# ScottHCL/recommend

Hardware: AMD Instinct MI355X
Metric: ranked samples/sec (fwd+bwd) at B=4096 seq=128; AUC parity vs ref (higher is better)
Workload: dtype f32-emulated (fp16-pair / split-bf16); 1 GPU; C2: OneTrans 4L d128 H4 f512 L_NS12 L_S128 (seq 3x42), Criteo-shape 13 dense + 26 ids, replicated tables, fwd+bwd+optimizer; global_batch=4096, per_gpu_batch=4096, seq_len=128, parallelism=dp1

## Files before the change

### include/onetrans_hip.h

```cpp
#ifndef ONETRANS_HIP_H
#define ONETRANS_HIP_H

#include <stddef.h>
#include <stdint.h>

#ifdef __cplusplus
extern "C" {
#endif

#define OT_OK 0
#define OT_ERR_INVALID_ARG 1
#define OT_ERR_UNSUPPORTED 2
#define OT_ERR_HIP 3

#define OT_GEMM_NN 0
#define OT_GEMM_NT 1

#define OT_AX_NONE 0
#define OT_AX_RMSNORM 1
#define OT_AX_GELU 2
#define OT_AX_BF16 4
#define OT_AX_BF16_RMSNORM 5

#define OT_EPI_BIAS 1
#define OT_EPI_GELU_BWD 2
#define OT_EPI_GELU 4
#define OT_EPI_DROPOUT 8
#define OT_EPI_RESIDUAL 16
#define OT_EPI_ACCUMULATE 32
#define OT_EPI_ROW_RSTD 64
#define OT_EPI_ROWDOT 256
#define OT_EPI_RMSNORM_BWD 128
#define OT_EPI_C_BF16 512
#define OT_EPI_AUX_BF16 1024
#define OT_WG_D_BF16 8

int ot_version(void);
const char* ot_get_last_error_string(void);

int ot_gemm_tile_rows(void);
#define OT_MATMUL_F32 0
#define OT_MATMUL_SPLIT_BF16 1
#define OT_MATMUL_BF16 2
int ot_mixed_gemm(int mode, const float* A, int64_t lda, int K, const int32_t* in_rows,
                  int a_xform, const float* a_rstd, const float* a_gamma,
                  const float* W, int64_t w_gstride, int64_t ldw, int N,
                  const int32_t* tile_group, int ntiles,
                  const float* bias, int64_t bias_gstride,
                  float* C, int64_t ldc, const int32_t* out_rows, int epi,
                  const float* res, int64_t ldres, int res_tok,
                  const float* aux, int64_t ldaux,
                  uint32_t seed, uint32_t site, float drop_rate, int tail_K, int tail_I,
                  const int32_t* tail_pos, int precision, void* stream);
typedef struct ot_rms_epilogue {
  size_t struct_size;
  float* rstd_out; float eps;
  const float* x; int64_t ldx;
  const float* gamma; const float* rstd;
  const float* dres; int64_t lddres;
  int dres_tail_K, dres_tail_I;
  const int32_t* dres_tail_inv;
  float* dx_masked; int64_t lddxm;
  float* dgamma; int accumulate_dgamma;
  void* workspace; size_t ws_bytes;
  float* rowdot; int rowdot_n;
  uint16_t* gelu_out; int64_t ldgelu;
  uint16_t* xn_out; int64_t ldxn;
  uint16_t* c16_out; int64_t ldc16;
  float* rowmax_out; int rowmax_n;
  const float* a_rowmax; int a_rowmax_n;
  float* amax_out;
  float* rowabs_out; int rowabs_n;
} ot_rms_epilogue;
size_t ot_mixed_gemm_rms_workspace_size(int ntiles, int N);
int ot_mixed_gemm_rms(int mode, const float* A, int64_t lda, int K, const int32_t* in_rows,
                      int a_xform, const float* a_rstd, const float* a_gamma,
                      const float* W, int64_t w_gstride, int64_t ldw, int N,
                      const int32_t* tile_group, int ntiles,
                      const float* bias, int64_t bias_gstride,
                      float* C, int64_t ldc, const int32_t* out_rows, int epi,
                      const float* res, int64_t ldres, int res_tok,
                      const float* aux, int64_t ldaux,
                      uint32_t seed, uint32_t site, float drop_rate, int tail_K, int tail_I,
                      const int32_t* tail_pos, const ot_rms_epilogue* rms, int precision, void* stream);

size_t ot_wgrad_workspace_size(int nchunks, int K, int N);
int ot_mixed_gemm_wgrad(const float* A, int64_t lda, const int32_t* a_rows, int a_xform,
                        const float* a_rstd, const float* a_gamma,
                        const float* D, int64_t ldd, const int32_t* d_rows, int K, int N,
                        const int32_t* chunks, int nchunks, const int32_t* gchunk, int ngroups,
                        float* dW, int64_t dw_gstride, float* db, int64_t db_gstride,
                        int accumulate, void* workspace, size_t ws_bytes, int precision, void* stream);

int ot_mixed_gemm_wgrad_ex(const float* A, int64_t lda, const int32_t* a_rows, int a_xform,
                           const float* a_rstd, const float* a_gamma,
                           const float* D, int64_t ldd, const int32_t* d_rows, int K, int N,
                           const int32_t* chunks, int nchunks, const int32_t* gchunk, int ngroups,
                           float* dW, int64_t dw_gstride, float* db, int64_t db_gstride,
                           int accumulate, void* workspace, size_t ws_bytes, const float* a_bound,
                           const float* d_bound, int precision, void* stream);

int ot_transpose_banks(const float* src, float* dst, const int64_t* banks_dev, int nbanks, int64_t total_tiles,
                       void* stream);

size_t ot_split_image_elems(int G, int N, int K);
int ot_split_images(const float* base, const int64_t* desc_dev, int ndesc, int64_t total_units, uint16_t* img,
                    int precision, void* stream);
int ot_mixed_gemm_img(int mode, const float* A, int64_t lda, int K, const int32_t* in_rows,
                      int a_xform, const float* a_rstd, const float* a_gamma,
                      const float* W, int64_t w_gstride, int64_t ldw, int N,
                      const int32_t* tile_group, int ntiles,
                      const float* bias, int64_t bias_gstride,
                      float* C, int64_t ldc, const int32_t* out_rows, int epi,
                      const float* res, int64_t ldres, int res_tok,
                      const float* aux, int64_t ldaux,
                      uint32_t seed, uint32_t site, float drop_rate, int tail_K, int tail_I,
                      const int32_t* tail_pos, const uint16_t* b_image, int image_ntn, int image_tn0,
                      int precision, void* stream);
int ot_plane_wide(int on);
int ot_wgrad_wide(int on);
int ot_plane_rowmeta(int on);
int ot_plane_panel(int on);
int ot_plane_panel_launches(void);
int ot_mixed_gemm_rms_img(int mode, const float* A, int64_t lda, int K, const int32_t* in_rows,
                          int a_xform, const float* a_rstd, const float* a_gamma,
                          const float* W, int64_t w_gstride, int64_t ldw, int N,
                          const int32_t* tile_group, int ntiles,
                          const float* bias, int64_t bias_gstride,
                          float* C, int64_t ldc, const int32_t* out_rows, int epi,
                          const float* res, int64_t ldres, int res_tok,
                          const float* aux, int64_t ldaux,
                          uint32_t seed, uint32_t site, float drop_rate, int tail_K, int tail_I,
                          const int32_t* tail_pos, const ot_rms_epilogue* rms, const uint16_t* b_image,
                          int image_ntn, int image_tn0, int precision, void* stream);

typedef struct ot_ffn_fused_args {
  size_t struct_size;
  const float* x1; int64_t ldx1;
  const int32_t* rows;
  const int32_t* tile_group; int ntiles;
  const float* rstd;
  const uint16_t* w1_image; int w1_groups;
  const uint16_t* w2_image; int w2_groups;
  const float* b1; int64_t b1_gstride;
  const float* b2; int64_t b2_gstride;
  int f;
  float* u_out; int64_t ldu;
  float* u_amax;
  float* x2; int64_t ldx2;
  float* rstd_out; float eps;
  uint32_t seed, site; float drop_rate;
  int tail_K, tail_I; const int32_t* tail_pos;
} ot_ffn_fused_args;
int ot_ffn_fused_fwd(const ot_ffn_fused_args* args, void* stream);
int ot_ffn_fused(int on);

typedef struct ot_ffn_fused_bwd_args {
  size_t struct_size;
  const float* dy2; int64_t lddy2;
  const float* dy2_rowmax; int dy2_rowmax_n;
  const int32_t* rows;
  const int32_t* tile_group; int ntiles;
  const uint16_t* w2_image; int w2_groups;
  const uint16_t* w1_image; int w1_groups;
  int f;
  const float* u; int64_t ldu;
  float* du; int64_t lddu;
  float* du_amax;
  const float* x1; int64_t ldx1;
  const float* gamma; const float* rstd;
  const float* dres; int64_t lddres;
  float* dx1; int64_t lddx1;
  float* dx_masked; int64_t lddxm;
  float* dgamma; int accumulate_dgamma;
  void* workspace; size_t ws_bytes;
  float* amax_out; float* rowabs_out; int rowabs_n;
  uint32_t seed, site; float drop_rate;
  int tail_K, tail_I; const int32_t* tail_pos;
} ot_ffn_fused_bwd_args;
int ot_ffn_fused_bwd(const ot_ffn_fused_bwd_args* args, void* stream);
int ot_ffn_fused_bwd_on(int on);

int ot_attn_fwd(const float* qkv, int64_t ld, int B, int H, int I, int K, const int32_t* qpos,
                int head_dim, float* out, float* lse, int precision, void* stream);
size_t ot_attn_fwd_fp8_workspace_size(int B, int H, int I, int head_dim);
int ot_attn_fwd_fp8(const float* qkv, int64_t ld, int B, int H, int I, int K, const int32_t* qpos,
                    int head_dim, float* out, float* lse, void* workspace, size_t ws_bytes, void* stream);
#define OT_FP8_DEQUANT 1
#define OT_FP8_TWO_TERM 2
int ot_attn_fwd_fp8_ex(float* qkv, int64_t ld, int B, int H, int I, int K, const int32_t* qpos, int head_dim,
                       float* out, float* lse, void* workspace, size_t ws_bytes, int flags, void* stream);
int ot_attn_fwd_fp8_deq16(const float* qkv, int64_t ld, int B, int H, int I, int K, const int32_t* qpos,
                          int head_dim, float* out, float* lse, void* workspace, size_t ws_bytes, int flags,
                          uint16_t* deq16, void* stream);
size_t ot_attn_bwd_workspace_size(int B, int H, int K);
int ot_attn_bwd(const float* qkv, int64_t ld, const float* out, const float* dout, const float* lse,
                int B, int H, int I, int K, const int32_t* qpos, int head_dim, float* dqkv, float* delta_ws,
                int precision, void* stream);
size_t ot_attn_bwd_ex_workspace_size(int B, int H, int I, int K, int head_dim, int selected, int precision);
int ot_attn_bwd_ex(const float* qkv, int64_t ld, const float* out, const float* dout, const float* lse,
                   int B, int H, int I, int K, const int32_t* qpos, int head_dim, float* dqkv, void* workspace,
                   size_t ws_bytes, int precision, void* stream);
#define OT_ATTN_DQKV_BF16 1
#define OT_ATTN_QKV_BF16 2
#define OT_ATTN_DQ_PART_BF16 4
int ot_attn_bwd_dqkv_bf16_supported(int I, int K, int head_dim, int selected, int precision);
int ot_attn_bwd_bf16_forms(int I, int K, int head_dim, int selected, int precision);
size_t ot_attn_bwd_flags_workspace_size(int B, int H, int I, int K, int head_dim, int selected, int flags, int precision);
int ot_attn_slice_supported(int I, int K, int head_dim, int selected);
int ot_attn_bwd_flags(const float* qkv, int64_t ld, const float* out, const float* dout, const float* lse,
                      int B, int H, int I, int K, const int32_t* qpos, int head_dim, void* dqkv, int flags,
                      void* workspace, size_t ws_bytes, int precision, void* stream);
int ot_attn_amax_supported(int I, int K, int head_dim, int selected, int precision);
int ot_attn_fwd_amax(const float* qkv, int64_t ld, int B, int H, int I, int K, const int32_t* qpos,
                     int head_dim, float* out, float* lse, float* amax, float* rowmax, int precision, void* stream);
int ot_attn_bwd_amax(const float* qkv, int64_t ld, const float* out, const float* dout, const float* lse,
                     int B, int H, int I, int K, const int32_t* qpos, int head_dim, float* dqkv,
                     void* workspace, size_t ws_bytes, float* amax, float* rowmax, int precision, void* stream);

int ot_attn_fwd_cached(const float* qkv, int64_t ld, const float* kv_cache, int64_t ldc, const int32_t* req,
                       int C, int H, int Ic, int n, int Kq, int head_dim, float* out, void* stream);

int ot_attn_fwd_cached_lse(const float* qkv, int64_t ld, const float* kv_cache, int64_t ldc, const int32_t* req,
                           int C, int H, int Ic, int n, int Kq, int head_dim, float* out, float* lse, void* stream);
size_t ot_attn_bwd_cached_workspace_size(int R, int C, int H, int Ic, int n, int Kq, int head_dim);
int ot_attn_bwd_cached(const float* qkv, int64_t ld, const float* kv_cache, int64_t ldc, const int32_t* req_start,
                       int R, int C, int H, int Ic, int n, int Kq, int head_dim, const float* out, const float* dout,
                       const float* lse, float* dqkv, float* dkv_cache, int accumulate, void* workspace,
                       size_t ws_bytes, void* stream);

int ot_attn_fold_supported(int d, int H);
int ot_attn_fold_rows(int I, int ded0, int ded1);
int ot_attn_fold_fwd(const float* x, int64_t ldx, const float* rstd, const float* gamma, const float* w, int64_t ldw,
                     const float* wT, int64_t ldwT, const float* qkv, int64_t ldqkv, int B, int H, int I,
                     int head_dim, int ded0, int ded1, float* o, float* lse, float* y, void* stream);
int ot_attn_fold_bwd(const float* x, int64_t ldx, const float* rstd, const float* gamma, const float* w, int64_t ldw,
                     const float* wT, int64_t ldwT, const float* qkv, int64_t ldqkv, int B, int H, int I,
                     int head_dim, int ded0, int ded1, const float* o, const float* dout, const float* lse,
                     const float* y, const float* dx1, float* dx, int64_t lddx, float* dqkv, int64_t lddqkv, float* z,
                     float* dgpart, void* stream);
size_t ot_attn_fold_workspace_size(int B, int d);
int ot_attn_fold_dw(const float* z, const float* y, const float* qkv, int64_t ldqkv, const float* dout,
                    const float* gamma, int B, int H, int I, int head_dim, float* dW, int64_t lddw, int accumulate,
                    void* workspace, size_t ws_bytes, void* stream);
int ot_attn_fold_dgamma(const float* dgpart, int B, int d, float* dgamma, int accumulate, void* workspace,
                        size_t ws_bytes, void* stream);
int ot_last_fold(int on);

int ot_attn_fwd_masked(const float* qkv, int64_t ld, int B, int H, int I, int K, const int32_t* qpos, int head_dim,
                       const uint8_t* key_valid, int64_t ldv, float* out, float* lse, int precision, void* stream);
int ot_attn_bwd_masked(const float* qkv, int64_t ld, const float* out, const float* dout, const float* lse, int B,
                       int H, int I, int K, const int32_t* qpos, int head_dim, const uint8_t* key_valid, int64_t ldv,
                       float* dqkv, float* delta_ws, int precision, void* stream);
int ot_attn_fwd_cached_masked(const float* qkv, int64_t ld, const float* kv_cache, int64_t ldc, const int32_t* req,
                              int C, int H, int Ic, int n, int Kq, int head_dim, const uint8_t* cache_valid,
                              int64_t ldcv, float* out, float* lse_or_null, void* stream);
int ot_seq_key_valid(const int32_t* lens, const int32_t* seq_len, const int32_t* seq_off, int nseq, int B, int L0,
                     const int32_t* rank, int64_t ldr, uint8_t* valid0, void* stream);

int ot_kv_pack_bf16(const float* qkv, int64_t ld, int R, int64_t rows_per_req, int d, uint16_t* kv16, int64_t ldc16,
                    int64_t req_stride, int64_t row0, void* stream);
int ot_attn_fwd_cached_kv16(const float* qkv, int64_t ld, const uint16_t* kv16, int64_t ldc16, int64_t req_stride,
                            const int32_t* req, int C, int H, int Ic, int n, int Kq, int head_dim,
                            const uint8_t* cache_valid, int64_t ldcv, float* out, float* lse_or_null, void* stream);
// ... 171 lines not shown
```

### recommend_amd/_lib.py

```python

from __future__ import annotations

import ctypes
import os
from ctypes import c_float, c_int, c_int64, c_size_t, c_uint32, c_void_p, c_char_p

_HERE = os.path.dirname(os.path.abspath(__file__))
LIB_PATH = os.environ.get('ONETRANS_HIP_LIB') or os.path.join(_HERE, 'libonetrans_hip.so')
HEADER = os.path.join(os.path.dirname(_HERE), 'include', 'onetrans_hip.h')

OT_GEMM_NN, OT_GEMM_NT = 0, 1
OT_AX_NONE, OT_AX_RMSNORM, OT_AX_GELU, OT_AX_BF16, OT_AX_BF16_RMSNORM = 0, 1, 2, 4, 5
OT_EPI_BIAS, OT_EPI_GELU_BWD, OT_EPI_GELU = 1, 2, 4
OT_EPI_DROPOUT, OT_EPI_RESIDUAL, OT_EPI_ACCUMULATE = 8, 16, 32
OT_EPI_ROW_RSTD, OT_EPI_RMSNORM_BWD, OT_EPI_ROWDOT = 64, 128, 256
OT_EPI_C_BF16 = 512
OT_EPI_AUX_BF16 = 1024
OT_ATTN_DQKV_BF16 = 1
OT_ATTN_QKV_BF16 = 2
OT_ATTN_DQ_PART_BF16 = 4
OT_WG_D_BF16 = 8
OT_MATMUL_F32, OT_MATMUL_SPLIT_BF16, OT_MATMUL_BF16 = 0, 1, 2
OT_FP8_DEQUANT, OT_FP8_TWO_TERM = 1, 2
OT_RANK_SUM, OT_RANK_PRODUCT = 0, 1
RANK_MODES = {'sum': OT_RANK_SUM, 'product': OT_RANK_PRODUCT}
RANK_MAX_K = 1024
MATMUL_MODES = {'f32': OT_MATMUL_F32, 'split': OT_MATMUL_SPLIT_BF16, 'bf16': OT_MATMUL_BF16}


class RmsEpilogue(ctypes.Structure):
    _fields_ = [('struct_size', c_size_t), ('rstd_out', c_void_p), ('eps', c_float),
                ('x', c_void_p), ('ldx', c_int64), ('gamma', c_void_p), ('rstd', c_void_p),
                ('dres', c_void_p), ('lddres', c_int64), ('dres_tail_K', c_int), ('dres_tail_I', c_int),
                ('dres_tail_inv', c_void_p),
                ('dx_masked', c_void_p), ('lddxm', c_int64),
                ('dgamma', c_void_p), ('accumulate_dgamma', c_int),
                ('workspace', c_void_p), ('ws_bytes', c_size_t),
                ('rowdot', c_void_p), ('rowdot_n', c_int),
                ('gelu_out', c_void_p), ('ldgelu', c_int64),
                ('xn_out', c_void_p), ('ldxn', c_int64),
                ('c16_out', c_void_p), ('ldc16', c_int64),
                ('rowmax_out', c_void_p), ('rowmax_n', c_int),
                ('a_rowmax', c_void_p), ('a_rowmax_n', c_int),
                ('amax_out', c_void_p), ('rowabs_out', c_void_p), ('rowabs_n', c_int)]

class FfnFusedArgs(ctypes.Structure):
    _fields_ = [('struct_size', c_size_t), ('x1', c_void_p), ('ldx1', c_int64), ('rows', c_void_p),
                ('tile_group', c_void_p), ('ntiles', c_int), ('rstd', c_void_p),
                ('w1_image', c_void_p), ('w1_groups', c_int), ('w2_image', c_void_p), ('w2_groups', c_int),
                ('b1', c_void_p), ('b1_gstride', c_int64), ('b2', c_void_p), ('b2_gstride', c_int64),
                ('f', c_int), ('u_out', c_void_p), ('ldu', c_int64), ('u_amax', c_void_p),
                ('x2', c_void_p), ('ldx2', c_int64), ('rstd_out', c_void_p), ('eps', c_float),
                ('seed', c_uint32), ('site', c_uint32), ('drop_rate', c_float),
                ('tail_K', c_int), ('tail_I', c_int), ('tail_pos', c_void_p)]


class FfnFusedBwdArgs(ctypes.Structure):
    _fields_ = [('struct_size', c_size_t), ('dy2', c_void_p), ('lddy2', c_int64),
                ('dy2_rowmax', c_void_p), ('dy2_rowmax_n', c_int), ('rows', c_void_p),
                ('tile_group', c_void_p), ('ntiles', c_int),
                ('w2_image', c_void_p), ('w2_groups', c_int), ('w1_image', c_void_p), ('w1_groups', c_int),
                ('f', c_int), ('u', c_void_p), ('ldu', c_int64), ('du', c_void_p), ('lddu', c_int64),
                ('du_amax', c_void_p), ('x1', c_void_p), ('ldx1', c_int64), ('gamma', c_void_p), ('rstd', c_void_p),
                ('dres', c_void_p), ('lddres', c_int64), ('dx1', c_void_p), ('lddx1', c_int64),
                ('dx_masked', c_void_p), ('lddxm', c_int64), ('dgamma', c_void_p), ('accumulate_dgamma', c_int),
                ('workspace', c_void_p), ('ws_bytes', c_size_t),
                ('amax_out', c_void_p), ('rowabs_out', c_void_p), ('rowabs_n', c_int),
                ('seed', c_uint32), ('site', c_uint32), ('drop_rate', c_float),
                ('tail_K', c_int), ('tail_I', c_int), ('tail_pos', c_void_p)]


class SeqTime(ctypes.Structure):
    _fields_ = [('times', c_void_p), ('stride_b', c_int64), ('L', ctypes.c_int32), ('map_off', ctypes.c_int32)]


class NsBag(ctypes.Structure):
    _fields_ = [('table', c_void_p), ('ids', c_void_p), ('weights', c_void_p), ('row_offset', c_int64),
                ('num_rows', c_int64), ('ids_stride', c_int64), ('weights_stride', c_int64),
                ('width', ctypes.c_int32), ('cap', ctypes.c_int32), ('col', ctypes.c_int32),
                ('pooling', ctypes.c_int32)]


OT_BAG_SUM, OT_BAG_MEAN = 0, 1
BAG_POOLINGS = {'sum': OT_BAG_SUM, 'mean': OT_BAG_MEAN}
NS_BAG_MAX = 32
NS_BAG_MAX_WIDTH = 256
SEQ_TIME_MAX_L = 4096
SEQ_TIME_MAX_SEQ = 32

P = c_void_p
I64 = c_int64

SIGNATURES = {
    'ot_version': (c_int, []),
    'ot_get_last_error_string': (c_char_p, []),
    'ot_gemm_tile_rows': (c_int, []),
    'ot_mixed_gemm': (c_int, [c_int, P, I64, c_int, P, c_int, P, P, P, I64, I64, c_int, P, c_int, P, I64,
                              P, I64, P, c_int, P, I64, c_int, P, I64, c_uint32, c_uint32, c_float, c_int,
                              c_int, P, c_int, P]),
    'ot_mixed_gemm_rms_workspace_size': (c_size_t, [c_int, c_int]),
    'ot_mixed_gemm_rms': (c_int, [c_int, P, I64, c_int, P, c_int, P, P, P, I64, I64, c_int, P, c_int, P, I64,
                                  P, I64, P, c_int, P, I64, c_int, P, I64, c_uint32, c_uint32, c_float, c_int,
                                  c_int, P, P, c_int, P]),
    'ot_wgrad_workspace_size': (c_size_t, [c_int, c_int, c_int]),
    'ot_mixed_gemm_wgrad': (c_int, [P, I64, P, c_int, P, P, P, I64, P, c_int, c_int, P, c_int, P, c_int, P,
                                    I64, P, I64, c_int, P, c_size_t, c_int, P]),
    'ot_mixed_gemm_wgrad_ex': (c_int, [P, I64, P, c_int, P, P, P, I64, P, c_int, c_int, P, c_int, P, c_int, P,
                                       I64, P, I64, c_int, P, c_size_t, P, P, c_int, P]),
    'ot_transpose_banks': (c_int, [P, P, P, c_int, I64, P]),
    'ot_mixed_gemm_img': (c_int, [c_int, P, I64, c_int, P, c_int, P, P, P, I64, I64, c_int, P, c_int, P, I64,
                                  P, I64, P, c_int, P, I64, c_int, P, I64, c_uint32, c_uint32, c_float, c_int,
                                  c_int, P, P, c_int, c_int, c_int, P]),
    'ot_mixed_gemm_rms_img': (c_int, [c_int, P, I64, c_int, P, c_int, P, P, P, I64, I64, c_int, P, c_int, P, I64,
                                      P, I64, P, c_int, P, I64, c_int, P, I64, c_uint32, c_uint32, c_float, c_int,
                                      c_int, P, P, P, c_int, c_int, c_int, P]),
    'ot_split_image_elems': (c_size_t, [c_int, c_int, c_int]),
    'ot_plane_wide': (c_int, [c_int]),
    'ot_wgrad_wide': (c_int, [c_int]),
    'ot_plane_rowmeta': (c_int, [c_int]),
    'ot_plane_panel': (c_int, [c_int]),
    'ot_plane_panel_launches': (c_int, []),
    'ot_ffn_fused_fwd': (c_int, [P, P]),
    'ot_ffn_fused': (c_int, [c_int]),
    'ot_ffn_fused_bwd': (c_int, [P, P]),
    'ot_ffn_fused_bwd_on': (c_int, [c_int]),
    'ot_split_images': (c_int, [P, P, c_int, I64, P, c_int, P]),
    'ot_attn_fwd': (c_int, [P, I64, c_int, c_int, c_int, c_int, P, c_int, P, P, c_int, P]),
    'ot_attn_fwd_fp8_workspace_size': (c_size_t, [c_int, c_int, c_int, c_int]),
    'ot_attn_fwd_fp8': (c_int, [P, I64, c_int, c_int, c_int, c_int, P, c_int, P, P, P, c_size_t, P]),
    'ot_attn_fwd_fp8_ex': (c_int, [P, I64, c_int, c_int, c_int, c_int, P, c_int, P, P, P, c_size_t, c_int, P]),
    'ot_attn_fwd_fp8_deq16': (c_int, [P, I64, c_int, c_int, c_int, c_int, P, c_int, P, P, P, c_size_t, c_int, P, P]),
    'ot_attn_bwd_workspace_size': (c_size_t, [c_int, c_int, c_int]),
    'ot_attn_bwd': (c_int, [P, I64, P, P, P, c_int, c_int, c_int, c_int, P, c_int, P, P, c_int, P]),
    'ot_attn_bwd_ex_workspace_size': (c_size_t, [c_int, c_int, c_int, c_int, c_int, c_int, c_int]),
    'ot_attn_bwd_ex': (c_int, [P, I64, P, P, P, c_int, c_int, c_int, c_int, P, c_int, P, P, c_size_t, c_int, P]),
    'ot_attn_bwd_dqkv_bf16_supported': (c_int, [c_int, c_int, c_int, c_int, c_int]),
    'ot_attn_bwd_bf16_forms': (c_int, [c_int, c_int, c_int, c_int, c_int]),
    'ot_attn_slice_supported': (c_int, [c_int, c_int, c_int, c_int]),
    'ot_attn_bwd_flags_workspace_size': (c_size_t, [c_int, c_int, c_int, c_int, c_int, c_int, c_int, c_int]),
    'ot_attn_bwd_flags': (c_int, [P, I64, P, P, P, c_int, c_int, c_int, c_int, P, c_int, P, c_int, P, c_size_t, c_int, P]),
    'ot_attn_fwd_cached': (c_int, [P, I64, P, I64, P, c_int, c_int, c_int, c_int, c_int, c_int, P, P]),
    'ot_attn_fwd_cached_lse': (c_int, [P, I64, P, I64, P, c_int, c_int, c_int, c_int, c_int, c_int, P, P, P]),
    'ot_attn_bwd_cached_workspace_size': (c_size_t, [c_int, c_int, c_int, c_int, c_int, c_int, c_int]),
    'ot_attn_bwd_cached': (c_int, [P, I64, P, I64, P, c_int, c_int, c_int, c_int, c_int, c_int, c_int, P, P, P, P, P,
                                   c_int, P, c_size_t, P]),
    'ot_attn_amax_supported': (c_int, [c_int, c_int, c_int, c_int, c_int]),
    'ot_attn_fwd_amax': (c_int, [P, I64, c_int, c_int, c_int, c_int, P, c_int, P, P, P, P, c_int, P]),
    'ot_attn_bwd_amax': (c_int, [P, I64, P, P, P, c_int, c_int, c_int, c_int, P, c_int, P, P, c_size_t, P, P, c_int,
                                 P]),
    'ot_pyramid_select': (c_int, [P, c_float, c_int, c_int, c_int, c_int, P, P, P, c_int, P]),
    'ot_rmsnorm_fwd': (c_int, [P, I64, P, P, I64, P, I64, c_int, c_float, P]),
    'ot_rmsnorm_bwd_workspace_size': (c_size_t, [I64, c_int]),
    'ot_rmsnorm_bwd': (c_int, [P, I64, P, I64, P, P, P, I64, c_int, c_int, P, P, I64, P, I64, c_uint32,
                               c_uint32, c_float, c_int, c_int, P, P, c_int, I64, c_int, P, c_size_t, P]),
    'ot_dropout_apply': (c_int, [P, I64, P, I64, I64, c_int, c_uint32, c_uint32, c_float, c_int, c_int, P, P]),
    'ot_dropout_apply_bf16': (c_int, [P, I64, P, I64, I64, c_int, c_uint32, c_uint32, c_float, c_int, c_int, P, P]),
    'ot_rows_absmax': (c_int, [P, I64, I64, c_int, P, c_int, P]),
    'ot_dropout_rowmax_supported': (c_int, [c_int]),
    'ot_dropout_apply_ex': (c_int, [P, I64, P, I64, I64, c_int, c_uint32, c_uint32, c_float, c_int, c_int, P, P, P,
                                    c_int, P]),
    'ot_rows_colsum_workspace_size': (c_size_t, [I64, c_int]),
    'ot_rows_colsum': (c_int, [P, I64, P, I64, c_int, P, c_int, P, c_size_t, P]),
    'ot_ns_assemble': (c_int, [P, c_int, P, c_int, P, I64, P]),
    'ot_ns_grad_pack': (c_int, [P, c_int, c_int, P, I64, c_int, P, P, P]),
    'ot_fill_rows': (c_int, [P, I64, P, I64, P, c_int, P]),
    'ot_seq_rows': (c_int, [P, I64, c_int, c_int, I64, P, P]),
    'ot_head_fwd': (c_int, [P, P, P, c_int, c_int, c_int, P, P, P]),
    'ot_head_bwd_workspace_size': (c_size_t, [c_int, c_int, c_int]),
    'ot_head_bwd': (c_int, [P, P, P, P, c_int, c_int, c_int, P, P, P, I64, I64, c_int, P, c_size_t, P]),
    'ot_bce_workspace_size': (c_size_t, [c_int, c_int]),
    'ot_bce_fwd': (c_int, [P, P, c_int, c_int, P, P, c_size_t, P]),
    'ot_bce_bwd': (c_int, [P, P, P, c_int, c_int, P, P]),
    'ot_task_loss_fwd': (c_int, [P, P, c_int, c_int, c_uint32, P, P, c_size_t, P]),
    'ot_task_loss_bwd': (c_int, [P, P, P, c_int, c_int, c_uint32, P, P]),
    'ot_task_loss_logits_fwd': (c_int, [P, P, P, c_int, c_int, c_uint32, P, P, c_size_t, P]),
    'ot_task_loss_logits_bwd': (c_int, [P, P, P, c_int, c_int, c_uint32, P, P]),
    'ot_head_bwd_ex': (c_int, [P, P, P, P, P, c_int, c_int, c_int, P, P, P, I64, I64, c_int, P, c_size_t, P]),
    'ot_sparse_adagrad_workspace_size': (c_size_t, [I64, c_int]),
    'ot_sparse_adagrad': (c_int, [P, P, c_int, I64, P, P, I64, c_float, c_float, c_float, P, c_size_t, P]),
    'ot_sparse_grad_dense': (c_int, [c_int, I64, P, P, I64, P, P, c_size_t, P]),
    'ot_dense_adagrad_workspace_size': (c_size_t, []),
    'ot_dense_adagrad': (c_int, [P, P, P, I64, c_int, c_float, c_float, c_float, P, c_size_t, P]),
    'ot_sparse_prepare': (c_int, [c_int, I64, P, P, I64, P, P, c_size_t, P]),
    'ot_sparse_finish': (c_int, [P, P, c_int, I64, c_float, c_float, c_float, P, P, c_size_t, P]),
    'ot_shard_route_workspace_size': (c_size_t, [I64]),
    'ot_shard_route': (c_int, [P, I64, I64, c_int, P, P, P, P, c_size_t, P]),
    'ot_shard_route_unique_workspace_size': (c_size_t, [I64]),
    'ot_shard_route_unique': (c_int, [P, I64, I64, c_int, P, P, P, P, P, P, c_size_t, P]),
    'ot_segment_rows_sum': (c_int, [P, P, P, I64, c_int, P, P]),
    'ot_segment_rows_sum_workspace_size': (c_size_t, [I64, I64, c_int]),
    'ot_segment_rows_sum_ex': (c_int, [P, P, P, I64, I64, c_int, P, P, c_size_t, P]),
    'ot_gather_rows': (c_int, [P, c_int, P, I64, P, P]),
    'ot_permute_rows': (c_int, [P, P, I64, c_int, c_int, P, P]),
    'ot_hash_uniform_rows': (c_int, [P, I64, c_int, c_int, c_int, c_uint32, c_float, c_float, P]),
    'ot_clip_rmsprop_workspace_size': (c_size_t, [c_int, I64]),
    'ot_clip_rmsprop': (c_int, [P, P, P, P, P, c_int, I64, c_float, c_float, c_float, c_float, c_float, P,
                                c_size_t, P]),
    'ot_clip_adam_workspace_size': (c_size_t, [c_int, I64]),
    'ot_clip_adam': (c_int, [P, P, P, P, P, c_int, I64, c_float, c_float, c_float, c_float, I64, c_float, P,
                             c_size_t, P]),
    'ot_metrics_workspace_size': (c_size_t, [c_int, c_int]),
    'ot_metrics_update': (c_int, [P, P, c_int, c_int, I64, P, c_int, P, P, P, c_size_t, P]),
    'ot_grouped_auc_workspace_size': (c_size_t, [c_int, I64, c_int]),
    'ot_grouped_auc': (c_int, [P, P, P, c_int, I64, I64, c_int, c_uint32, P, P, P, P, P, c_size_t, P]),
    'ot_rank_topk_workspace_size': (c_size_t, [c_int, I64, c_int]),
    'ot_rank_topk': (c_int, [P, I64, c_int, P, c_int, P, I64, c_int, c_int, P, P, P, P, P, c_size_t, P]),
    'ot_seq_time_rows_workspace_size': (c_size_t, [c_int, c_int, c_int]),
    'ot_seq_time_rows': (c_int, [P, c_int, c_int, c_int, I64, P, P, P, P, c_size_t, P]),
# ... 70 lines not shown
```

### recommend_amd/csrc/gemm_ffn.hip

```cpp
#include <atomic>
#include <cstdlib>
#include <mutex>

#include "gemm.h"

namespace ot {

#ifndef OT_FFN_NSTG
#define OT_FFN_NSTG 3
#endif
constexpr int FF_NST = OT_FFN_NSTG;
static_assert(FF_NST == 2 || FF_NST == 3, "fused FFN stage buffers");
constexpr int PG_A_BYTES = GT * 16 * 4;
constexpr int FF_STG = PG_A_BYTES + 2 * GT * 16 * 2;
constexpr int FF_TR_LD = 36;
constexpr int FF_TR_WAVE = 32 * FF_TR_LD * 4;
constexpr int FF_TR_OFF = FF_NST * FF_STG;
constexpr int FF_META_OFF = FF_TR_OFF + 4 * FF_TR_WAVE;
constexpr int FF_TAB_OFF = FF_META_OFF + GT * 4;
constexpr int FF_MAX_F = 1024;
static_assert(FF_META_OFF >= (64 * (GT + 4) + 8 * GT) * 4, "fused FFN: the epilogue tile overlays the row metadata");
static_assert(FF_TAB_OFF + (2 * FF_MAX_F + GT) * 4 <= 80 * 1024, "fused FFN LDS");
constexpr int ffn_lds(int f) { return FF_TAB_OFF + (2 * f + GT) * 4; }

// ... 161 lines not shown
    if (mrow >= 0) am = fmaxf(am, ua);
    {
      const float s = pow2_scale14(fmaxf(mx, 0.17f));
      if (c > 0) {
        const float ratio = s * hinv;
#pragma unroll
        for (int a = 0; a < 4; ++a)
#pragma unroll
          for (int r = 0; r < 16; ++r) acc2[a][r] *= ratio;
      }
      hsc = s;
      hinv = 1.f / s;
    }
    if (q.u_out) {
#pragma unroll
      for (int nb = 0; nb < 4; ++nb) {
#pragma unroll
        for (int qd = 0; qd < 4; ++qd)
          *reinterpret_cast<f32x4*>(trw + li * FF_TR_LD + 8 * qd + 4 * h) =
              f32x4{acc1[nb][4 * qd], acc1[nb][4 * qd + 1], acc1[nb][4 * qd + 2], acc1[nb][4 * qd + 3]};
        asm volatile("s_waitcnt lgkmcnt(0)" ::: "memory");
#pragma unroll
        for (int ps = 0; ps < 4; ++ps) {
          const f32x4 v = *reinterpret_cast<const f32x4*>(trw + ((lane >> 3) + 8 * ps) * FF_TR_LD + 4 * (lane & 7));
          const int ur = rmeta[32 * wave + (lane >> 3) + 8 * ps];
          if (ur >= 0) store_out4(q.u_out + (int64_t)ur * q.ldu + 128 * c + 32 * nb + 4 * (lane & 7), v);
        }
        asm volatile("s_waitcnt lgkmcnt(0)" ::: "memory");
      }
    }
    auto stage2 = [&](int j, const f32x16& u) {
      top(8 + j);
      const char* sb = lds + ((8 + j) % FF_NST) * FF_STG;
#pragma unroll
      for (int s = 0; s < 2; ++s) {
        const f32x4 g0 = gelu_erf4(f32x4{u[8 * s], u[8 * s + 1], u[8 * s + 2], u[8 * s + 3]});
        const f32x4 g1 = gelu_erf4(f32x4{u[8 * s + 4], u[8 * s + 5], u[8 * s + 6], u[8 * s + 7]});
        const float hv[8] = {g0.x, g0.y, g0.z, g0.w, g1.x, g1.y, g1.z, g1.w};
        u32x4 fh[3];
        pair8(hv, hsc, fh);
        u32x4 fw[4][2];
#pragma unroll
        for (int nb = 0; nb < 4; ++nb)
#pragma unroll
          for (int pl = 0; pl < 2; ++pl) {
            const char* wb = sb + s * 8192 + pl * 4096 + nb * 1024;
            const u32x2 lo = *reinterpret_cast<const u32x2*>(wb + woff0);
            const u32x2 hi = *reinterpret_cast<const u32x2*>(wb + woff1);
            fw[nb][pl] = u32x4{lo.x, lo.y, hi.x, hi.y};
          }
#pragma unroll
        for (int nb = 0; nb < 4; ++nb) acc2[nb] = mfma_pair_t(fw[nb], fh, acc2[nb]);
      }
    };
    stage2(0, acc1[0]);
    stage2(1, acc1[1]);
    stage2(2, acc1[2]);
    stage2(3, acc1[3]);
  }
#pragma unroll
  for (int nb = 0; nb < 4; ++nb)
#pragma unroll
    for (int qd = 0; qd < 4; ++qd) {
      const f32x4 cs = *reinterpret_cast<const f32x4*>(tab + 2 * q.f + 32 * nb + 8 * qd + 4 * h);
#pragma unroll
      for (int i = 0; i < 4; ++i) acc2[nb][4 * qd + i] *= hinv * cs[i];
    }
  asm volatile("s_waitcnt vmcnt(0) lgkmcnt(0)" ::: "memory");
  __syncthreads();
  gemm_vec_epilogue<EPIT, 5, false, 8, false>(p, acc2, smem, tm, 0, g, 0, -1, rmeta);
  if (q.u_amax) amax_flush(q.u_amax, am);
}

#ifndef OT_FFN_FUSED
#define OT_FFN_FUSED 1
#endif
static int ffn_fused_initial() {
  const char* e = getenv("ONETRANS_FFN_FUSED");
  return e && *e ? (atoi(e) != 0) : OT_FFN_FUSED;
}
static std::atomic<int> g_ffn_fused{ffn_fused_initial()};

constexpr int FB_TAB_OFF = FF_TAB_OFF;
static_assert(FB_TAB_OFF + (FF_MAX_F + GT) * 4 <= 80 * 1024, "fused FFN backward LDS");
constexpr int ffn_bwd_lds(int f) { return FB_TAB_OFF + (f + GT) * 4; }

struct FfnBwdArgs {
  GemmArgs e;
  const uint16_t* img2; int g2;
  const uint16_t* img1; int g1;
  const float* u; int64_t ldu;
  float* du; int64_t lddu;
  float* du_amax;
  int f;
};

template <int EPIT>
__global__ __launch_bounds__(256, 2) void ffn_fused_bwd_kernel(FfnBwdArgs q) {
  const GemmArgs& p = q.e;
  extern __shared__ __attribute__((aligned(16))) float smem[];
  char* lds = reinterpret_cast<char*>(smem);
  const int tm = xcd_remap(blockIdx.x, p.ntm);
  const int g = p.tile_group ? p.tile_group[tm] : 0;
  const int t = threadIdx.x, lane = t & 63, wave = t >> 6;
  const int h = lane >> 5, li = lane & 31;
  const int nch = q.f >> 7;

  int arow[2];
#pragma unroll
  for (int i = 0; i < 2; ++i) {
    const int64_t gr = (int64_t)tm * GT + (2 * wave + i) * 16 + (lane >> 2);
    const int ir = p.in_rows ? p.in_rows[gr] : (int)gr;
    arow[i] = ir < 0 ? 0 : ir;
  }
  int urow[4];
#pragma unroll
  for (int i = 0; i < 4; ++i) {
    const int64_t gr = (int64_t)tm * GT + 32 * wave + 8 * i + (lane >> 3);
    const int ur = p.out_rows ? p.out_rows[gr] : (int)gr;
    urow[i] = ur < 0 ? 0 : ur;
  }
  constexpr int64_t T1 = 8 * (int64_t)PG_B_BYTES;
  const char* img2 = reinterpret_cast<const char*>(q.img2) + (int64_t)(q.g2 ? g : 0) * nch * T1;
  const char* img1 = reinterpret_cast<const char*>(q.img1) + (int64_t)(q.g1 ? g : 0) * (q.f >> 4) * PG_B_BYTES;
  const int blane = 2 * wave * 1024 + 16 * lane;
  auto issue = [&](int c, int sidx, int buf) {
    char* sb = lds + buf * FF_STG;
    if (sidx < 8) {
      const char* bs = img2 + c * T1 + (int64_t)sidx * PG_B_BYTES + blane;
#pragma unroll
      for (int i = 0; i < 2; ++i)
        __builtin_amdgcn_global_load_lds(
            (const void*)(p.A + (int64_t)arow[i] * p.lda + 16 * sidx + 4 * ((lane & 3) ^ ((lane >> 4) & 3))),
            (lds_void_t*)(sb + (2 * wave + i) * 1024), 16, 0, 0);
#pragma unroll
      for (int i = 0; i < 2; ++i)
        __builtin_amdgcn_global_load_lds((const void*)(bs + i * 1024),
                                         (lds_void_t*)(sb + PG_A_BYTES + (2 * wave + i) * 1024), 16, 0, 0);
    } else if (sidx < 12) {
#pragma unroll
      for (int i = 0; i < 4; ++i)
        __builtin_amdgcn_global_load_lds(
            (const void*)(q.u + (int64_t)urow[i] * q.ldu + 128 * c + 32 * (sidx - 8) +
                          4 * ((lane & 7) ^ ((4 * i + (lane >> 4)) & 7))),
            (lds_void_t*)(sb + (4 * wave + i) * 1024), 16, 0, 0);
    } else {
      const char* bs = img1 + (int64_t)(8 * c + 2 * (sidx - 12)) * PG_B_BYTES + blane;
#pragma unroll
      for (int u = 0; u < 2; ++u)
#pragma unroll
        for (int i = 0; i < 2; ++i)
          __builtin_amdgcn_global_load_lds((const void*)(bs + u * PG_B_BYTES + i * 1024),
                                           (lds_void_t*)(sb + u * 8192 + (2 * wave + i) * 1024), 16, 0, 0);
    }
  };

  const int ra = 32 * wave + li;
  const int aoff0 = ra * 64 + 16 * ((2 * h) ^ ((li >> 2) & 3));
  const int sw = (li >> 3) & 1;
  const int boff = PG_A_BYTES + li * 32 + 16 * (h ^ sw);
  const int woff0 = li * 32 + 16 * sw + 8 * h;
  const int usw = (li >> 1) & 7;

  float abound = 0.f;
  int mrow;
  {
    const int64_t gr = (int64_t)tm * GT + ra;
    int ir = p.in_rows ? p.in_rows[gr] : (int)gr;
    mrow = p.out_rows ? p.out_rows[gr] : (int)gr;
    ir = ir < 0 ? 0 : ir;
    for (int j = 0; j < p.a_rowmax_n; ++j) abound = fmaxf(abound, p.a_rowmax[(int64_t)ir * p.a_rowmax_n + j]);
  }
  float* tab = reinterpret_cast<float*>(lds + FB_TAB_OFF);
  int tt = t;
  asm volatile("" : "+v"(tt));
  for (int idx = tt; idx < q.f; idx += 256) {
    const float* cs = reinterpret_cast<const float*>(img2 + (idx >> 7) * T1 + 2 * GT * 16 * 2);
    const float bad = reinterpret_cast<const uint32_t*>(cs)[GT] == PAIR_IMAGE_TAG ? 1.f : __builtin_nanf("");
    tab[idx] = bad / cs[idx & 127];
  }
  if (tt < GT) {
    const float* cs = reinterpret_cast<const float*>(img1 + 2 * GT * 16 * 2);
    const float bad = reinterpret_cast<const uint32_t*>(cs)[GT] == PAIR_IMAGE_TAG ? 1.f : __builtin_nanf("");
    tab[q.f + tt] = bad / cs[tt];
  }
  int* rmeta = reinterpret_cast<int*>(lds + FF_META_OFF);
  if (h == 0) rmeta[ra] = mrow;
  const float asc = pow2_scale14(abound);
  const float ainv = 1.f / asc;
  float* trw = reinterpret_cast<float*>(lds + FF_TR_OFF + wave * FF_TR_WAVE);
  asm volatile("" : "+v"(abound), "+v"(mrow), "+v"(arow[0]), "+v"(arow[1]), "+v"(urow[0]), "+v"(urow[1]),
               "+v"(urow[2]), "+v"(urow[3]));

  int rb = 0;
  issue(0, 0, 0);
  if (FF_NST == 3) issue(0, 1, 1);
  f32x16 acc2[4];
#pragma unroll
  for (int a = 0; a < 4; ++a)
#pragma unroll
    for (int r = 0; r < 16; ++r) acc2[a][r] = 0.f;
  float am = 0.f, bound = 0.f, hsc = 1.f, hinv = 1.f;

  for (int c = 0; c < nch; ++c) {
    auto top = [&](int sidx) -> const char* {
      if (FF_NST == 2 || sidx == 12 || (sidx == 15 && c + 1 == nch)) asm volatile("s_waitcnt vmcnt(0)" ::: "memory");
      else asm volatile("s_waitcnt vmcnt(4)" ::: "memory");
      asm volatile("s_waitcnt lgkmcnt(0)" ::: "memory");
      __builtin_amdgcn_s_barrier();
      asm volatile("" ::: "memory");
      constexpr int AH = FF_NST - 1;
      const int nb_ = rb == 0 ? FF_NST - 1 : rb - 1;
      if (sidx + AH < 16) issue(c, sidx + AH, nb_);
      else if (c + 1 < nch) issue(c + 1, sidx + AH - 16, nb_);
      const char* sb = lds + rb * FF_STG;
      rb = rb + 1 == FF_NST ? 0 : rb + 1;
      return sb;
    };
    f32x16 acc1[4];
#pragma unroll
    for (int a = 0; a < 4; ++a)
#pragma unroll
      for (int r = 0; r < 16; ++r) acc1[a][r] = 0.f;
#pragma unroll
    for (int kt = 0; kt < 8; ++kt) {
      const char* sb = top(kt);
      u32x4 fb[4][2];
#pragma unroll
      for (int nb = 0; nb < 4; ++nb)
#pragma unroll
        for (int pl = 0; pl < 2; ++pl) fb[nb][pl] = *reinterpret_cast<const u32x4*>(sb + boff + pl * 4096 + nb * 1024);
      const f32x4 a0 = *reinterpret_cast<const f32x4*>(sb + aoff0);
      const f32x4 a1 = *reinterpret_cast<const f32x4*>(sb + (aoff0 ^ 16));
      const float av[8] = {a0.x, a0.y, a0.z, a0.w, a1.x, a1.y, a1.z, a1.w};
      u32x4 fa[3];
      pair8(av, asc, fa);
#pragma unroll
      for (int nb = 0; nb < 4; ++nb) acc1[nb] = mfma_pair_t(fb[nb], fa, acc1[nb]);
    }
    float ua = 0.f;
    auto finish = [&](int nb, f32x16& a) {
      const char* sb = top(8 + nb);
#pragma unroll
      for (int qd = 0; qd < 4; ++qd) {
        const f32x4 u4 = *reinterpret_cast<const f32x4*>(sb + ra * 128 + 16 * ((2 * qd + h) ^ usw));
        const f32x4 ci = *reinterpret_cast<const f32x4*>(tab + 128 * c + 32 * nb + 8 * qd + 4 * h);
        f32x4 v = {a[4 * qd], a[4 * qd + 1], a[4 * qd + 2], a[4 * qd + 3]};
        v = v * (ainv * ci);
        v *= gelu_erf_grad4(u4);
        ua = amax4(ua, v);
        a[4 * qd] = v.x; a[4 * qd + 1] = v.y; a[4 * qd + 2] = v.z; a[4 * qd + 3] = v.w;
      }
    };
    finish(0, acc1[0]);
    finish(1, acc1[1]);
    finish(2, acc1[2]);
    finish(3, acc1[3]);
    if (mrow >= 0) am = fmaxf(am, ua);
    bound = fmaxf(bound, fmaxf(ua, __shfl_xor(ua, 32, 64)));
    {
      const float s = pow2_scale14(bound);
      if (c > 0) {
        const float ratio = s * hinv;
#pragma unroll
        for (int a = 0; a < 4; ++a)
#pragma unroll
          for (int r = 0; r < 16; ++r) acc2[a][r] *= ratio;
      }
      hsc = s;
      hinv = 1.f / s;
    }
#pragma unroll
    for (int nb = 0; nb < 4; ++nb) {
#pragma unroll
      for (int qd = 0; qd < 4; ++qd)
        *reinterpret_cast<f32x4*>(trw + li * FF_TR_LD + 8 * qd + 4 * h) =
            f32x4{acc1[nb][4 * qd], acc1[nb][4 * qd + 1], acc1[nb][4 * qd + 2], acc1[nb][4 * qd + 3]};
      asm volatile("s_waitcnt lgkmcnt(0)" ::: "memory");
#pragma unroll
      for (int ps = 0; ps < 4; ++ps) {
        const f32x4 v = *reinterpret_cast<const f32x4*>(trw + ((lane >> 3) + 8 * ps) * FF_TR_LD + 4 * (lane & 7));
        const int ur = rmeta[32 * wave + (lane >> 3) + 8 * ps];
        if (ur >= 0) store_out4(q.du + (int64_t)ur * q.lddu + 128 * c + 32 * nb + 4 * (lane & 7), v);
      }
      asm volatile("s_waitcnt lgkmcnt(0)" ::: "memory");
    }
    auto stage2 = [&](int j, const f32x16& u) {
      const char* sb = top(12 + j);
#pragma unroll
      for (int s = 0; s < 2; ++s) {
        const float hv[8] = {u[8 * s], u[8 * s + 1], u[8 * s + 2], u[8 * s + 3],
                             u[8 * s + 4], u[8 * s + 5], u[8 * s + 6], u[8 * s + 7]};
        u32x4 fh[3];
        pair8(hv, hsc, fh);
        u32x4 fw[4][2];
#pragma unroll
        for (int nb = 0; nb < 4; ++nb)
#pragma unroll
          for (int pl = 0; pl < 2; ++pl) {
            const char* wb = sb + s * 8192 + pl * 4096 + nb * 1024;
            const u32x2 lo = *reinterpret_cast<const u32x2*>(wb + woff0);
            const u32x2 hi = *reinterpret_cast<const u32x2*>(wb + (woff0 ^ 16));
            fw[nb][pl] = u32x4{lo.x, lo.y, hi.x, hi.y};
          }
#pragma unroll
        for (int nb = 0; nb < 4; ++nb) acc2[nb] = mfma_pair_t(fw[nb], fh, acc2[nb]);
      }
    };
    stage2(0, acc1[0]);
    stage2(1, acc1[1]);
    stage2(2, acc1[2]);
    stage2(3, acc1[3]);
  }
#pragma unroll
  for (int nb = 0; nb < 4; ++nb)
#pragma unroll
    for (int qd = 0; qd < 4; ++qd) {
      const f32x4 cs = *reinterpret_cast<const f32x4*>(tab + q.f + 32 * nb + 8 * qd + 4 * h);
#pragma unroll
      for (int i = 0; i < 4; ++i) acc2[nb][4 * qd + i] *= hinv * cs[i];
    }
  asm volatile("s_waitcnt vmcnt(0) lgkmcnt(0)" ::: "memory");
  __syncthreads();
  gemm_vec_epilogue<EPIT, 5, false, OT_PLANE_EPI_RBN, false>(p, acc2, smem, tm, 0, g, 0, -1, rmeta);
  if (q.du_amax) amax_flush(q.du_amax, am);
}

#ifndef OT_FFN_FUSED_BWD
#define OT_FFN_FUSED_BWD 1
#endif
static int ffn_fused_bwd_initial() {
  const char* e = getenv("ONETRANS_FFN_FUSED_BWD");
  return e && *e ? (atoi(e) != 0) : OT_FFN_FUSED_BWD;
}
static std::atomic<int> g_ffn_fused_bwd{ffn_fused_bwd_initial()};

}

using namespace ot;

extern "C" int ot_ffn_fused_bwd_on(int on) {
  const int old = g_ffn_fused_bwd.load(std::memory_order_relaxed);
  if (on >= 0) g_ffn_fused_bwd.store(on ? 1 : 0, std::memory_order_relaxed);
  return old;
}

extern "C" int ot_ffn_fused_bwd(const ot_ffn_fused_bwd_args* a, void* stream) {
  OT_REQUIRE(a, "ot_ffn_fused_bwd: null arguments");
  OT_REQUIRE(a->struct_size == sizeof(ot_ffn_fused_bwd_args),
             "ot_ffn_fused_bwd: ot_ffn_fused_bwd_args.struct_size %zu != %zu (header of another ot_version)",
             a->struct_size, sizeof(ot_ffn_fused_bwd_args));
  OT_REQUIRE(a->dy2 && a->dy2_rowmax && a->u && a->du && a->w2_image && a->w1_image && a->x1 && a->gamma && a->rstd &&
                 a->dx1 && a->dgamma && a->workspace,
             "ot_ffn_fused_bwd: null operand");
  OT_REQUIRE(a->ntiles >= 0 && a->f >= GT && a->f % GT == 0 && a->f <= FF_MAX_F,
             "ot_ffn_fused_bwd: bad sizes ntiles=%d f=%d (f a multiple of %d up to %d)", a->ntiles, a->f, GT, FF_MAX_F);
  auto a16 = [](const void* q) { return ((uintptr_t)q & 15) == 0; };
  OT_REQUIRE(a->lddy2 >= GT && a->ldx1 >= GT && a->lddx1 >= GT && a->lddy2 % 4 == 0 && a->ldx1 % 4 == 0 &&
                 a->lddx1 % 4 == 0 && a16(a->dy2) && a16(a->x1) && a16(a->dx1) && a16(a->gamma) && a16(a->w2_image) &&
                 a16(a->w1_image),
             "ot_ffn_fused_bwd: rows of %d floats, leading dimensions multiples of 4, 16-B aligned operands", GT);
  OT_REQUIRE(a->ldu >= a->f && a->lddu >= a->f && a->ldu % 4 == 0 && a->lddu % 4 == 0 && a16(a->u) && a16(a->du),
             "ot_ffn_fused_bwd: u / du need ld >= f, ld %% 4 == 0 and 16-B alignment");
  OT_REQUIRE(a->dy2_rowmax_n >= 1, "ot_ffn_fused_bwd: dy2_rowmax_n must be >= 1");
  OT_REQUIRE(!a->dres || (a->lddres >= GT && a->lddres % 4 == 0 && a16(a->dres)),
             "ot_ffn_fused_bwd: dres needs lddres >= %d, lddres %% 4 == 0 and 16-B alignment", GT);
  OT_REQUIRE(a->w1_groups >= 1 && a->w2_groups >= 1, "ot_ffn_fused_bwd: image group counts must be >= 1");
  OT_REQUIRE(a->w1_groups == 1 && a->w2_groups == 1 ? true : a->tile_group != nullptr,
             "ot_ffn_fused_bwd: grouped weight images need tile_group");
  OT_REQUIRE(a->drop_rate >= 0.f && a->drop_rate < 1.f, "ot_ffn_fused_bwd: drop_rate out of range");
  OT_REQUIRE(a->drop_rate == 0.f || (a->tail_K > 0 && a->tail_I >= a->tail_K), "ot_ffn_fused_bwd: bad tail map");
  OT_REQUIRE(a->drop_rate == 0.f || (a->dx_masked && a->lddxm >= GT && a->lddxm % 4 == 0 && a16(a->dx_masked)),
             "ot_ffn_fused_bwd: dropout needs dx_masked (lddxm >= %d, lddxm %% 4 == 0, 16-B aligned)", GT);
  OT_REQUIRE(a->ws_bytes >= ot_mixed_gemm_rms_workspace_size(a->ntiles, GT), "ot_ffn_fused_bwd: workspace too small");
  OT_REQUIRE(!a->rowabs_out || a->rowabs_n == 1, "ot_ffn_fused_bwd: rowabs_out needs rowabs_n == 1");
  if (a->ntiles == 0) return OT_OK;
  FfnBwdArgs q{};
  GemmArgs& p = q.e;
  p.A = a->dy2; p.lda = a->lddy2; p.K = a->f; p.in_rows = a->rows;
  p.a_rowmax = a->dy2_rowmax; p.a_rowmax_n = a->dy2_rowmax_n;
  p.N = GT; p.tile_group = a->tile_group;
  p.C = a->dx1; p.ldc = a->lddx1; p.out_rows = a->rows;
  p.seed = a->seed; p.site = a->site; p.drop_thr = 0u; p.drop_scale = 1.f;
  p.tail_K = a->tail_K > 0 ? a->tail_K : 1; p.tail_I = a->tail_I > 0 ? a->tail_I : 1; p.tail_pos = a->tail_pos;
  p.drop_width = GT; p.ntm = a->ntiles; p.ntn = 1;
  p.nx = a->x1; p.ldnx = a->ldx1; p.ngamma = a->gamma; p.nrstd = a->rstd;
  p.dres = a->dres; p.lddres = a->lddres;
  p.dxm = a->dx_masked; p.lddxm = a->lddxm;
  p.dgpart = (float*)a->workspace;
  p.amax_out = a->amax_out; p.rowabs_out = a->rowabs_out; p.rowabs_n = a->rowabs_n;
  int epi = OT_EPI_RMSNORM_BWD;
  if (a->drop_rate > 0.f) {
    epi |= OT_EPI_DROPOUT;
    p.drop_thr = drop_threshold(a->drop_rate);
    p.drop_scale = 1.f / (1.f - a->drop_rate);
  }
  p.epi = epi;
  q.img2 = a->w2_image; q.g2 = a->w2_groups > 1;
  q.img1 = a->w1_image; q.g1 = a->w1_groups > 1;
  q.u = a->u; q.ldu = a->ldu; q.du = a->du; q.lddu = a->lddu; q.du_amax = a->du_amax; q.f = a->f;
  void (*kern)(FfnBwdArgs) = a->drop_rate > 0.f ? ffn_fused_bwd_kernel<OT_EPI_RMSNORM_BWD | OT_EPI_DROPOUT>
                                                : ffn_fused_bwd_kernel<OT_EPI_RMSNORM_BWD>;
  static std::once_flag once;
  std::call_once(once, [] {
    (void)hipFuncSetAttribute((const void*)ffn_fused_bwd_kernel<OT_EPI_RMSNORM_BWD>,
                              hipFuncAttributeMaxDynamicSharedMemorySize, ffn_bwd_lds(FF_MAX_F));
    (void)hipFuncSetAttribute((const void*)ffn_fused_bwd_kernel<OT_EPI_RMSNORM_BWD | OT_EPI_DROPOUT>,
                              hipFuncAttributeMaxDynamicSharedMemorySize, ffn_bwd_lds(FF_MAX_F));
    (void)hipGetLastError();
  });
  hipStream_t s = (hipStream_t)stream;
  hipLaunchKernelGGL(kern, dim3((unsigned)a->ntiles), dim3(256), (size_t)ffn_bwd_lds(a->f), s, q);
  OT_LAUNCH_CHECK("ot_ffn_fused_bwd");
  float* dgpart = (float*)a->workspace;
  launch_colsum_reduce(dgpart, a->ntiles, GT, a->dgamma, a->accumulate_dgamma, s, dgpart + (int64_t)a->ntiles * GT);
  OT_LAUNCH_CHECK("ot_ffn_fused_bwd(dgamma)");
  return OT_OK;
}

extern "C" int ot_ffn_fused(int on) {
  const int old = g_ffn_fused.load(std::memory_order_relaxed);
  if (on >= 0) g_ffn_fused.store(on ? 1 : 0, std::memory_order_relaxed);
  return old;
}

extern "C" int ot_ffn_fused_fwd(const ot_ffn_fused_args* a, void* stream) {
  OT_REQUIRE(a, "ot_ffn_fused_fwd: null arguments");
  OT_REQUIRE(a->struct_size == sizeof(ot_ffn_fused_args),
             "ot_ffn_fused_fwd: ot_ffn_fused_args.struct_size %zu != %zu (header of another ot_version)",
             a->struct_size, sizeof(ot_ffn_fused_args));
  OT_REQUIRE(a->x1 && a->x2 && a->rstd && a->w1_image && a->w2_image && a->b1 && a->b2,
             "ot_ffn_fused_fwd: null operand");
  OT_REQUIRE(a->ntiles >= 0 && a->f >= GT && a->f % GT == 0 && a->f <= FF_MAX_F,
             "ot_ffn_fused_fwd: bad sizes ntiles=%d f=%d (f a multiple of %d up to %d)", a->ntiles, a->f, GT, FF_MAX_F);
  auto a16 = [](const void* q) { return ((uintptr_t)q & 15) == 0; };
  OT_REQUIRE(a->ldx1 >= GT && a->ldx2 >= GT && a->ldx1 % 4 == 0 && a->ldx2 % 4 == 0 && a16(a->x1) && a16(a->x2) &&
                 a16(a->b1) && a16(a->b2) && a->b1_gstride % 4 == 0 && a->b2_gstride % 4 == 0 && a16(a->w1_image) &&
                 a16(a->w2_image),
             "ot_ffn_fused_fwd: rows of %d floats, leading dimensions and bias strides multiples of 4, 16-B aligned "
             "operands", GT);
  OT_REQUIRE(!a->u_out || (a->ldu >= a->f && a->ldu % 4 == 0 && a16(a->u_out)),
             "ot_ffn_fused_fwd: u_out needs ldu >= f, ldu %% 4 == 0 and 16-B alignment");
  OT_REQUIRE(a->w1_groups >= 1 && a->w2_groups >= 1, "ot_ffn_fused_fwd: image group counts must be >= 1");
  OT_REQUIRE(a->w1_groups == 1 && a->w2_groups == 1 ? true : a->tile_group != nullptr,
             "ot_ffn_fused_fwd: grouped weight images need tile_group");
  OT_REQUIRE(a->drop_rate >= 0.f && a->drop_rate < 1.f, "ot_ffn_fused_fwd: drop_rate out of range");
  OT_REQUIRE(a->drop_rate == 0.f || (a->tail_K > 0 && a->tail_I >= a->tail_K), "ot_ffn_fused_fwd: bad tail map");
  if (a->ntiles == 0) return OT_OK;
  FfnArgs q{};
  GemmArgs& p = q.e;
  p.A = a->x1; p.lda = a->ldx1; p.K = GT; p.in_rows = a->rows; p.a_xform = OT_AX_RMSNORM; p.a_rstd = a->rstd;
  p.N = GT; p.tile_group = a->tile_group; p.bias = a->b2; p.bias_gstride = a->b2_gstride;
  p.C = a->x2; p.ldc = a->ldx2; p.out_rows = a->rows;
  p.res = a->x1; p.ldres = a->ldx1; p.res_tok = 0;
  p.seed = a->seed; p.site = a->site; p.drop_thr = 0u; p.drop_scale = 1.f;
  p.tail_K = a->tail_K > 0 ? a->tail_K : 1; p.tail_I = a->tail_I > 0 ? a->tail_I : 1; p.tail_pos = a->tail_pos;
  p.drop_width = GT; p.ntm = a->ntiles; p.ntn = 1;
  p.rstd_out = a->rstd_out; p.eps = a->eps;
  int epi = OT_EPI_BIAS | OT_EPI_RESIDUAL;
  if (a->drop_rate > 0.f) {
    epi |= OT_EPI_DROPOUT;
    p.drop_thr = drop_threshold(a->drop_rate);
    p.drop_scale = 1.f / (1.f - a->drop_rate);
  }
  if (a->rstd_out) epi |= OT_EPI_ROW_RSTD;
  p.epi = epi;
  q.img1 = a->w1_image; q.g1 = a->w1_groups > 1;
  q.img2 = a->w2_image; q.g2 = a->w2_groups > 1;
  q.b1 = a->b1; q.b1_gstride = a->b1_gstride;
  q.u_out = a->u_out; q.ldu = a->ldu; q.u_amax = a->u_amax; q.f = a->f;
  void (*kern)(FfnArgs) = nullptr;
#define OT_FFN_PICK(EP_) if (epi == (EP_)) kern = ffn_fused_kernel<EP_>;
  OT_FFN_PICK(OT_EPI_BIAS | OT_EPI_RESIDUAL)
  OT_FFN_PICK(OT_EPI_BIAS | OT_EPI_RESIDUAL | OT_EPI_DROPOUT)
  OT_FFN_PICK(OT_EPI_BIAS | OT_EPI_RESIDUAL | OT_EPI_ROW_RSTD)
  OT_FFN_PICK(OT_EPI_BIAS | OT_EPI_RESIDUAL | OT_EPI_DROPOUT | OT_EPI_ROW_RSTD)
#undef OT_FFN_PICK
  static std::once_flag once;
  std::call_once(once, [] {
#define OT_FFN_ATTR(EP_)                                                                                            \
  (void)hipFuncSetAttribute((const void*)ffn_fused_kernel<EP_>, hipFuncAttributeMaxDynamicSharedMemorySize,         \
                            ffn_lds(FF_MAX_F));
    OT_FFN_ATTR(OT_EPI_BIAS | OT_EPI_RESIDUAL)
    OT_FFN_ATTR(OT_EPI_BIAS | OT_EPI_RESIDUAL | OT_EPI_DROPOUT)
    OT_FFN_ATTR(OT_EPI_BIAS | OT_EPI_RESIDUAL | OT_EPI_ROW_RSTD)
    OT_FFN_ATTR(OT_EPI_BIAS | OT_EPI_RESIDUAL | OT_EPI_DROPOUT | OT_EPI_ROW_RSTD)
#undef OT_FFN_ATTR
    (void)hipGetLastError();
  });
  hipLaunchKernelGGL(kern, dim3((unsigned)a->ntiles), dim3(256), (size_t)ffn_lds(a->f), (hipStream_t)stream, q);
  OT_LAUNCH_CHECK("ot_ffn_fused_fwd");
  return OT_OK;
}
```

### recommend_amd/csrc/gemm_wgrad.hip

```cpp
#include <atomic>
#include <mutex>

#include "gemm.h"

namespace ot {

#ifndef OT_WGRAD_BF16_RS
#define OT_WGRAD_BF16_RS 2
#endif
constexpr int WGRAD_BF16_RS = OT_WGRAD_BF16_RS;
#ifndef OT_WGRAD_DBUF
#define OT_WGRAD_DBUF 0
#endif

__host__ __device__ inline unsigned wgrad_grid(int nchunks, int per_chunk) {
  return (unsigned)(nchunks < 8 ? nchunks : (nchunks + 7) / 8 * 8) * per_chunk;
}
__device__ __forceinline__ bool wgrad_tile(int b, int per_chunk, int nchunks, int& c, int& rem) {
  if (nchunks < 8) {
    c = b / per_chunk;
    rem = b % per_chunk;
    return true;
  }
  const int x = b & 7, j = b >> 3;
  c = x + 8 * (j / per_chunk);
  rem = j % per_chunk;
  return c < nchunks;
}

constexpr int WBR = 32;
constexpr int WLD = GT;

struct WgradArgs {
  const float* A; int64_t lda; const int32_t* a_rows; int a_xform; const float* a_rstd; const float* a_gamma;
  const float* D; int64_t ldd; const int32_t* d_rows;
  int K, N;
  const int32_t* chunks;
  int nchunks;
  float* slab;
  float* bslab;
  int ntk, ntn;
  const float* a_bound; const float* d_bound;
};

template <int AXT>
__global__ __launch_bounds__(256, 2) void wgrad_kernel(WgradArgs p) {
  extern __shared__ __attribute__((aligned(16))) float smem[];
  const int ax = AXT >= 0 ? AXT : p.a_xform;
  const int per_chunk = p.ntk * p.ntn;
  int c, rem;
  if (!wgrad_tile(blockIdx.x, per_chunk, p.nchunks, c, rem)) return;
  const int tk = rem / p.ntn, tn = rem % p.ntn;
  const int k0 = tk * GT, n0 = tn * GT;
  const int row_begin = p.chunks[3 * c + 1], row_count = p.chunks[3 * c + 2];
  const int t = threadIdx.x, lane = t & 63, wave = t >> 6;
  const int h = lane >> 5, li = lane & 31;
  const int wm = (wave >> 1) * 64, wn = (wave & 1) * 64;
  const int sr = t >> 3, sc = t & 7;
  const f32x4 zero4 = {0.f, 0.f, 0.f, 0.f};

  f32x16 acc[2][2];
#pragma unroll
  for (int a = 0; a < 2; ++a)
#pragma unroll
    for (int b = 0; b < 2; ++b)
#pragma unroll
      for (int r = 0; r < 16; ++r) acc[a][b][r] = 0.f;
  float bsum = 0.f;
  const bool do_bias = p.bslab && tk == 0 && t < GT;

  auto rows_of = [&](int rs, int& ar, int& dr) {
    const int lr = rs + sr;
    const int64_t mi = (int64_t)row_begin + (lr < row_count ? lr : 0);
    ar = p.a_rows ? p.a_rows[mi] : (int)mi;
    dr = p.d_rows ? p.d_rows[mi] : (int)mi;
  };
  f32x4 va[4], vd[4], gv[4];
  float rsd = 1.f;
  bool aok = false, dok = false;
  auto load_stage = [&](int st, int ar, int dr) {
    const bool in = st * WBR + sr < row_count && ar >= 0 && dr >= 0;
    aok = in; dok = in;
    const float* pa = p.A + (int64_t)(aok ? ar : 0) * p.lda;
    const float* pd = p.D + (int64_t)(dok ? dr : 0) * p.ldd;
    if (ax == OT_AX_RMSNORM) rsd = p.a_rstd[aok ? ar : 0];
#pragma unroll
    for (int i = 0; i < 4; ++i) {
      const int k = k0 + 4 * (sc + 8 * i), n = n0 + 4 * (sc + 8 * i);
      const int kc = k < p.K ? k : 0, nc = n < p.N ? n : 0;
      va[i] = *reinterpret_cast<const f32x4*>(pa + kc);
      vd[i] = *reinterpret_cast<const f32x4*>(pd + nc);
      if (ax == OT_AX_RMSNORM) gv[i] = *reinterpret_cast<const f32x4*>(p.a_gamma + kc);
    }
  };
  constexpr int NBUF = OT_WGRAD_DBUF ? 2 : 1;
  auto store_stage = [&](int buf) {
    float* As = smem + buf * WBR * WLD;
    float* Ds = smem + (NBUF + buf) * WBR * WLD;
#pragma unroll
    for (int i = 0; i < 4; ++i) {
      const int kk = 4 * (sc + 8 * i);
      f32x4 a = va[i], dv = vd[i];
      if (ax == OT_AX_RMSNORM) {
        a = a * gv[i] * rsd;
      } else if (ax == OT_AX_GELU) {
        a = gelu_erf4(a);
      }
      if (!(aok && k0 + kk < p.K)) a = zero4;
      if (!(dok && n0 + kk < p.N)) dv = zero4;
      *reinterpret_cast<f32x4*>(As + sr * WLD + kk) = a;
      *reinterpret_cast<f32x4*>(Ds + sr * WLD + kk) = dv;
    }
  };

  const int nst = (row_count + WBR - 1) / WBR;
  int ar, dr, ar2 = -1, dr2 = -1;
  rows_of(0, ar, dr);
  if (nst > 1) rows_of(WBR, ar2, dr2);
  load_stage(0, ar, dr);
  store_stage(0);
  __syncthreads();
  for (int st = 0; st < nst; ++st) {
    const int cur = NBUF == 2 ? (st & 1) : 0;
    const bool more = st + 1 < nst;
    int ar3 = -1, dr3 = -1;
    if (more) {
      load_stage(st + 1, ar2, dr2);
      if (st + 2 < nst) rows_of((st + 2) * WBR, ar3, dr3);
    }
    const float* As = smem + cur * WBR * WLD;
    const float* Ds = smem + (NBUF + cur) * WBR * WLD;
    if (do_bias) {
#pragma unroll
      for (int r = 0; r < WBR; r += 4)
        bsum += (Ds[r * WLD + t] + Ds[(r + 1) * WLD + t]) + (Ds[(r + 2) * WLD + t] + Ds[(r + 3) * WLD + t]);
    }
    float fa[16][2], fb[16][2];
#pragma unroll
    for (int s2 = 0; s2 < 16; ++s2)
#pragma unroll
      for (int m = 0; m < 2; ++m) {
        fa[s2][m] = As[(2 * s2 + h) * WLD + wm + 32 * m + li];
        fb[s2][m] = Ds[(2 * s2 + h) * WLD + wn + 32 * m + li];
      }
#pragma unroll
    for (int s2 = 0; s2 < 16; ++s2)
#pragma unroll
      for (int m = 0; m < 2; ++m)
#pragma unroll
        for (int n = 0; n < 2; ++n)
          acc[m][n] = __builtin_amdgcn_mfma_f32_32x32x2f32(fa[s2][m], fb[s2][n], acc[m][n], 0, 0, 0);
    if (NBUF == 2) {
      if (more) store_stage(cur ^ 1);
      __syncthreads();
    } else {
      __syncthreads();
      if (more) store_stage(0);
      __syncthreads();
    }
    ar2 = ar3; dr2 = dr3;
  }
  float* slab = p.slab + (int64_t)c * p.K * p.N;
#pragma unroll
  for (int m = 0; m < 2; ++m)
#pragma unroll
    for (int r = 0; r < 16; ++r) {
      const int k = k0 + wm + 32 * m + (r & 3) + 8 * (r >> 2) + 4 * h;
      if (k >= p.K) continue;
#pragma unroll
      for (int n = 0; n < 2; ++n) {
        const int col = n0 + wn + 32 * n + li;
        if (col < p.N) slab[(int64_t)k * p.N + col] = acc[m][n][r];
      }
    }
  if (do_bias && n0 + t < p.N) p.bslab[(int64_t)c * p.N + n0 + t] = bsum;
}

typedef short v4i16 __attribute__((ext_vector_type(4)));
constexpr int WSPLANE = WBR * 256;
constexpr int WSOP = 3 * WSPLANE;

__device__ __forceinline__ int wsw_off(int r, int ch) { return 256 * r + 16 * (ch ^ (((r & 3) << 2) | ((r >> 2) & 3))); }

__device__ __forceinline__ v4i16 ds_tr16(const char* base, int off) {
  typedef __attribute__((address_space(3))) v4i16 lds_v4i16;
  return __builtin_amdgcn_ds_read_tr16_b64_v4i16((lds_v4i16*)(base + off));
}

template <int TERMS>
constexpr int wgrad_rs() { return WGRAD_BF16_RS > 0 && TERMS == 1 ? WGRAD_BF16_RS : 1; }

template <int AXT, int TERMS, bool DBF = false>
__global__ __launch_bounds__(256, 2) void wgrad_split_kernel(WgradArgs p) {
  constexpr int RS = wgrad_rs<TERMS>();
  static_assert(RS * WSPLANE <= WSOP && (TERMS == 1 || RS == 1), "wgrad stage LDS");
  static_assert(TERMS != 2 || (!DBF && (AXT == OT_AX_NONE || AXT == OT_AX_RMSNORM || AXT == OT_AX_GELU)),
                "pair wgrad forms");
  constexpr bool PAIR = TERMS == 2;
  constexpr int BR = WBR * RS;
  constexpr int NPL = TERMS == 1 ? 1 : PAIR ? 2 : 3;
  extern __shared__ __attribute__((aligned(16))) char smem_c[];
  const int ax = AXT >= 0 ? AXT : p.a_xform;
  const int per_chunk = p.ntk * p.ntn;
  int c, rem;
  if (!wgrad_tile(blockIdx.x, per_chunk, p.nchunks, c, rem)) return;
  const int tk = rem / p.ntn, tn = rem % p.ntn;
  const int k0 = tk * GT, n0 = tn * GT;
  const int row_begin = p.chunks[3 * c + 1], row_count = p.chunks[3 * c + 2];
  const int t = threadIdx.x, lane = t & 63, wave = t >> 6;
  const int h = lane >> 5, li = lane & 31;
  const int wm = (wave >> 1) * 64, wn = (wave & 1) * 64;
  const int sr = t >> 3, sc = t & 7;
  const f32x4 zero4 = {0.f, 0.f, 0.f, 0.f};
  char* As = smem_c;
  char* Ds = smem_c + WSOP;

  f32x16 acc[2][2];
#pragma unroll
  for (int a = 0; a < 2; ++a)
#pragma unroll
    for (int b = 0; b < 2; ++b)
#pragma unroll
      for (int r = 0; r < 16; ++r) acc[a][b][r] = 0.f;
  const bool do_bias = p.bslab && tk == 0;
  f32x4 bsum[4] = {zero4, zero4, zero4, zero4};
  f32x4 gv[4];
  if (ax == OT_AX_RMSNORM) {
#pragma unroll
    for (int i = 0; i < 4; ++i) {
      const int k = k0 + 4 * (sc + 8 * i);
      gv[i] = *reinterpret_cast<const f32x4*>(p.a_gamma + (k < p.K ? k : 0));
    }
  }
  f32x4 sa[4];
  float sdv = 1.f;
  if constexpr (PAIR) {
    sdv = pow2_scale14(p.d_bound[0]);
    const float sqk = sqrtf((float)p.K);
    const float s1 = AXT == OT_AX_RMSNORM ? 1.f : pow2_scale14(p.a_bound[0]);
#pragma unroll
    for (int i = 0; i < 4; ++i)
      sa[i] = AXT == OT_AX_RMSNORM
                  ? f32x4{pow2_scale14(sqk * fabsf(gv[i].x)), pow2_scale14(sqk * fabsf(gv[i].y)),
                          pow2_scale14(sqk * fabsf(gv[i].z)), pow2_scale14(sqk * fabsf(gv[i].w))}
                  : f32x4{s1, s1, s1, s1};
  }

  auto rows_of = [&](int rs, int (&ar)[RS], int (&dr)[RS]) {
#pragma unroll
    for (int j = 0; j < RS; ++j) {
      const int lr = rs + sr + WBR * j;
      const int64_t mi = (int64_t)row_begin + (lr < row_count ? lr : 0);
      ar[j] = p.a_rows ? p.a_rows[mi] : (int)mi;
      dr[j] = p.d_rows ? p.d_rows[mi] : (int)mi;
    }
  };
  f32x4 va[RS][4], vd[RS][4];
  float rsd[RS];
  bool inr[RS];
  auto load_stage = [&](int st, const int (&ar)[RS], const int (&dr)[RS]) {
#pragma unroll
    for (int j = 0; j < RS; ++j) {
      inr[j] = st * BR + sr + WBR * j < row_count && ar[j] >= 0 && dr[j] >= 0;
      const float* pa = p.A + (int64_t)(inr[j] ? ar[j] : 0) * p.lda;
      const uint16_t* pa16 = reinterpret_cast<const uint16_t*>(p.A) + (int64_t)(inr[j] ? ar[j] : 0) * p.lda;
      const float* pd = p.D + (int64_t)(inr[j] ? dr[j] : 0) * p.ldd;
      rsd[j] = ax == OT_AX_RMSNORM ? p.a_rstd[inr[j] ? ar[j] : 0] : 1.f;
#pragma unroll
      for (int i = 0; i < 4; ++i) {
        const int k = k0 + 4 * (sc + 8 * i), n = n0 + 4 * (sc + 8 * i);
        const int kc = k < p.K ? k : 0, nc = n < p.N ? n : 0;
        if (AXT == OT_AX_BF16) {
          const u32x2 w = *reinterpret_cast<const u32x2*>(pa16 + kc);
          va[j][i] = f32x4{__uint_as_float(w.x << 16), __uint_as_float(w.x & 0xffff0000u),
                           __uint_as_float(w.y << 16), __uint_as_float(w.y & 0xffff0000u)};
        } else {
          va[j][i] = *reinterpret_cast<const f32x4*>(pa + kc);
        }
        if (DBF) {
          const u32x2 w = *reinterpret_cast<const u32x2*>(reinterpret_cast<const uint16_t*>(p.D) +
                                                          (int64_t)(inr[j] ? dr[j] : 0) * p.ldd + nc);
          vd[j][i] = f32x4{__uint_as_float(w.x << 16), __uint_as_float(w.x & 0xffff0000u),
                           __uint_as_float(w.y << 16), __uint_as_float(w.y & 0xffff0000u)};
        } else {
          vd[j][i] = *reinterpret_cast<const f32x4*>(pd + nc);
        }
      }
    }
  };
  auto store_stage = [&]() {
#pragma unroll
    for (int j = 0; j < RS; ++j)
#pragma unroll
      for (int i = 0; i < 4; ++i) {
        const int cc = sc + 8 * i;
        f32x4 a = va[j][i], dv = vd[j][i];
        if (ax == OT_AX_RMSNORM) {
          a = a * gv[i] * rsd[j];
        } else if (ax == OT_AX_GELU) {
          a = gelu_erf4(a);
        }
        dv = dv * (inr[j] ? 1.f : 0.f);
        bsum[i] += dv;
        const int off = wsw_off(sr + WBR * j, cc >> 1) + 8 * (cc & 1);
        if constexpr (TERMS == 1) {
          *reinterpret_cast<u32x2*>(As + off) = bf16_rne4(a);
          *reinterpret_cast<u32x2*>(Ds + off) = bf16_rne4(dv);
          continue;
        }
        if constexpr (PAIR) {
          u32x2 h0, l0;
          pair4(a * sa[i], h0, l0);
          *reinterpret_cast<u32x2*>(As + off) = h0;
          *reinterpret_cast<u32x2*>(As + WSPLANE + off) = l0;
          pair4(dv * sdv, h0, l0);
          *reinterpret_cast<u32x2*>(Ds + off) = h0;
          *reinterpret_cast<u32x2*>(Ds + WSPLANE + off) = l0;
          continue;
        }
        u32x2 q0, q1, q2;
        split3(a, q0, q1, q2);
        *reinterpret_cast<u32x2*>(As + off) = q0;
        *reinterpret_cast<u32x2*>(As + WSPLANE + off) = q1;
        *reinterpret_cast<u32x2*>(As + 2 * WSPLANE + off) = q2;
        split3(dv, q0, q1, q2);
        *reinterpret_cast<u32x2*>(Ds + off) = q0;
        *reinterpret_cast<u32x2*>(Ds + WSPLANE + off) = q1;
        *reinterpret_cast<u32x2*>(Ds + 2 * WSPLANE + off) = q2;
      }
  };
  const int gi = lane & 15, q = gi >> 2, pp = gi & 3, g1 = (lane >> 4) & 1;
  int aoff[2][2], doff[2][2];
#pragma unroll
  for (int m = 0; m < 2; ++m)
#pragma unroll
    for (int rd = 0; rd < 2; ++rd) {
      const int r = 8 * h + 4 * rd + q;
      aoff[m][rd] = wsw_off(r, (wm + 32 * m + 16 * g1) / 8 + (pp >> 1)) + 8 * (pp & 1);
      doff[m][rd] = wsw_off(r, (wn + 32 * m + 16 * g1) / 8 + (pp >> 1)) + 8 * (pp & 1);
    }

  const int nst = (row_count + BR - 1) / BR;
  int ar[RS], dr[RS], ar2[RS], dr2[RS];
  rows_of(0, ar, dr);
  if (nst > 1) rows_of(BR, ar2, dr2);
  load_stage(0, ar, dr);
  store_stage();
  __syncthreads();
  for (int st = 0; st < nst; ++st) {
    const bool more = st + 1 < nst;
    int ar3[RS], dr3[RS];
    if (more) {
      load_stage(st + 1, ar2, dr2);
      if (st + 2 < nst) rows_of((st + 2) * BR, ar3, dr3);
    }
#pragma unroll
    for (int t2 = 0; t2 < 2 * RS; ++t2) {
      u32x4 fa[2][3], fb[2][3];
#pragma unroll
      for (int m = 0; m < 2; ++m)
#pragma unroll
        for (int pl = 0; pl < NPL; ++pl) {
          const int po = pl * WSPLANE + t2 * 16 * 256;
          const v4i16 a0 = ds_tr16(As + po, aoff[m][0]), a1 = ds_tr16(As + po, aoff[m][1]);
          const v4i16 d0 = ds_tr16(Ds + po, doff[m][0]), d1 = ds_tr16(Ds + po, doff[m][1]);
          const u32x2 a0u = __builtin_bit_cast(u32x2, a0), a1u = __builtin_bit_cast(u32x2, a1);
          const u32x2 d0u = __builtin_bit_cast(u32x2, d0), d1u = __builtin_bit_cast(u32x2, d1);
          fa[m][pl] = u32x4{a0u.x, a0u.y, a1u.x, a1u.y};
          fb[m][pl] = u32x4{d0u.x, d0u.y, d1u.x, d1u.y};
        }
#pragma unroll
      for (int m = 0; m < 2; ++m)
#pragma unroll
        for (int n = 0; n < 2; ++n) {
          if constexpr (TERMS == 1) {
            acc[m][n] = mfma_bf16(fa[m][0], fb[n][0], acc[m][n]);
            continue;
          }
          if constexpr (PAIR) {
            acc[m][n] = mfma_f16(fa[m][0], fb[n][1], acc[m][n]);
            acc[m][n] = mfma_f16(fa[m][1], fb[n][0], acc[m][n]);
            acc[m][n] = mfma_f16(fa[m][0], fb[n][0], acc[m][n]);
            continue;
// ... 593 lines not shown
    }
    for (; c < cb + cn; c += 16) s += *reinterpret_cast<const f32x4*>(src + (int64_t)c * KN + i4);
  }
  red[cl][col] = s;
  __syncthreads();
  if (cl == 0 && i4 < KN) {
    f32x4 t = red[0][col];
#pragma unroll
    for (int q = 1; q < 16; ++q) t += red[q][col];
    float* dst = out + i4;
    if (accumulate) t += *reinterpret_cast<const f32x4*>(dst);
    *reinterpret_cast<f32x4*>(dst) = t;
  }
  if (db && N % 4 != 0 && blockIdx.x == 0) {
    for (int n = threadIdx.x; n < N; n += blockDim.x) {
      float t = 0.f;
      if (bslab)
        for (int c = cb; c < cb + cn; ++c) t += bslab[(int64_t)c * N + n];
      float* dst = db + (int64_t)g * db_gstride + n;
      *dst = accumulate ? *dst + t : t;
    }
  }
}

__global__ __launch_bounds__(256) void transpose_banks_kernel(const float* __restrict__ src, float* dst,
                                                              const int64_t* __restrict__ banks, int nbanks) {
  __shared__ float tile[32][33];
  const int64_t tid = blockIdx.x;
  int b = 0;
  while (b + 1 < nbanks && banks[6 * (b + 1) + 5] <= tid) ++b;
  const int64_t* bk = banks + 6 * b;
  const int64_t G = bk[2], K = bk[3], N = bk[4];
  const int64_t tk = (K + 31) / 32, tnn = (N + 31) / 32;
  int64_t rem = tid - bk[5];
  if (rem >= G * tk * tnn) return;
  const int64_t g = rem / (tk * tnn);
  rem %= tk * tnn;
  const int64_t k0 = (rem / tnn) * 32, n0 = (rem % tnn) * 32;
  const float* s = src + bk[0] + g * K * N;
  float* d = dst + bk[1] + g * K * N;
  const int tx = threadIdx.x & 31, ty = threadIdx.x >> 5;
  for (int i = ty; i < 32; i += 8) {
    const int64_t k = k0 + i, n = n0 + tx;
    tile[i][tx] = (k < K && n < N) ? s[k * N + n] : 0.f;
  }
  __syncthreads();
  for (int i = ty; i < 32; i += 8) {
    const int64_t n = n0 + i, k = k0 + tx;
    if (k < K && n < N) d[n * K + k] = tile[tx][i];
  }
}

}

using namespace ot;

extern "C" int ot_transpose_banks(const float* src, float* dst, const int64_t* banks_dev, int nbanks,
                                  int64_t total_tiles, void* stream) {
  OT_REQUIRE(src && dst && banks_dev && nbanks > 0, "ot_transpose_banks: bad args");
  if (total_tiles == 0) return OT_OK;
  hipLaunchKernelGGL(transpose_banks_kernel, dim3((unsigned)total_tiles), dim3(256), 0, (hipStream_t)stream, src, dst,
                     banks_dev, nbanks);
  OT_LAUNCH_CHECK("ot_transpose_banks");
  return OT_OK;
}

static std::atomic<int> g_wgrad_wide{OT_WGRAD_WIDE};
extern "C" int ot_wgrad_wide(int on) {
  const int prev = g_wgrad_wide.load();
  if (on >= 0) g_wgrad_wide.store(on > 3 ? 3 : on);
  return prev;
}

extern "C" size_t ot_wgrad_workspace_size(int nchunks, int K, int N) {
  return ((size_t)nchunks * K * N + (size_t)nchunks * N) * sizeof(float);
}

static int wgrad_impl(const float* A, int64_t lda, const int32_t* a_rows, int a_xform,
                      const float* a_rstd, const float* a_gamma,
                      const float* D, int64_t ldd, const int32_t* d_rows, int K, int N,
                      const int32_t* chunks, int nchunks, const int32_t* gchunk, int ngroups,
                      float* dW, int64_t dw_gstride, float* db, int64_t db_gstride,
                      int accumulate, void* workspace, size_t ws_bytes, const float* a_bound, const float* d_bound,
                      int precision, void* stream) {
  OT_REQUIRE(precision == OT_MATMUL_F32 || precision == OT_MATMUL_SPLIT_BF16 || precision == OT_MATMUL_BF16,
             "ot_mixed_gemm_wgrad: unknown precision %d", precision);
  OT_REQUIRE(A && D && dW && chunks && gchunk && workspace, "ot_mixed_gemm_wgrad: null operand");
  OT_REQUIRE(K % 4 == 0 && N % 4 == 0 && lda % 4 == 0 && ldd % 4 == 0 && dw_gstride % 4 == 0,
             "ot_mixed_gemm_wgrad: K, N, lda, ldd, dw_gstride must be multiples of 4");
  OT_REQUIRE(ws_bytes >= ot_wgrad_workspace_size(nchunks, K, N), "ot_mixed_gemm_wgrad: workspace too small");
  const bool dbf = (a_xform & OT_WG_D_BF16) != 0;
  a_xform &= ~OT_WG_D_BF16;
  OT_REQUIRE(a_xform != OT_AX_RMSNORM || (a_rstd && a_gamma), "ot_mixed_gemm_wgrad: rmsnorm prologue needs rstd/gamma");
  OT_REQUIRE(!dbf || (precision == OT_MATMUL_BF16 &&
                      (a_xform == OT_AX_NONE || a_xform == OT_AX_RMSNORM || a_xform == OT_AX_BF16) &&
                      ((uintptr_t)D % 8) == 0),
             "ot_mixed_gemm_wgrad: OT_WG_D_BF16 needs the bf16 mode, A form OT_AX_NONE / OT_AX_RMSNORM and 8-B "
             "aligned D rows");
  hipStream_t s = (hipStream_t)stream;
  float* slab = (float*)workspace;
  float* bslab = db ? slab + (size_t)nchunks * K * N : nullptr;
  if (nchunks > 0) {
    WgradArgs p{A, lda, a_rows, a_xform, a_rstd, a_gamma, D, ldd, d_rows, K, N, chunks, nchunks, slab, bslab,
                (int)ceil_div(K, GT), (int)ceil_div(N, GT), a_bound, d_bound};
    const bool pair = precision == OT_MATMUL_SPLIT_BF16 && !dbf && d_bound &&
                      ((a_xform == OT_AX_RMSNORM) || ((a_xform == OT_AX_NONE || a_xform == OT_AX_GELU) && a_bound));
    const size_t shmem = (OT_WGRAD_DBUF ? 4 : 2) * WBR * WLD * sizeof(float);
    const bool split = precision != OT_MATMUL_F32;
    OT_REQUIRE(a_xform != OT_AX_BF16 || (precision != OT_MATMUL_F32 && lda % 4 == 0 && ((uintptr_t)A % 8) == 0),
               "ot_mixed_gemm_wgrad: OT_AX_BF16 needs the split / bf16 mode and 8-B aligned rows");
    const bool copy = dbf && a_xform == OT_AX_BF16 && K % 8 == 0 && N % 8 == 0 && lda % 8 == 0 &&
                      ldd % 8 == 0 && ((uintptr_t)A % 16) == 0 && ((uintptr_t)D % 16) == 0 && a_rows == d_rows;
    void (*kern)(WgradArgs) =
        pair ? (a_xform == OT_AX_NONE      ? wgrad_split_kernel<OT_AX_NONE, 2>
                : a_xform == OT_AX_RMSNORM ? wgrad_split_kernel<OT_AX_RMSNORM, 2>
                                           : wgrad_split_kernel<OT_AX_GELU, 2>)
        : copy ? (a_rows ? wgrad_bf16_kernel<true> : wgrad_bf16_kernel<false>)
        : dbf ? (a_xform == OT_AX_NONE      ? wgrad_split_kernel<OT_AX_NONE, 1, true>
                 : a_xform == OT_AX_BF16    ? wgrad_split_kernel<OT_AX_BF16, 1, true>
                                            : wgrad_split_kernel<OT_AX_RMSNORM, 1, true>)
        : a_xform == OT_AX_BF16 ? (precision == OT_MATMUL_BF16 ? wgrad_split_kernel<OT_AX_BF16, 1>
                                                                : wgrad_split_kernel<OT_AX_BF16, SPLIT_TERMS>)
        : precision == OT_MATMUL_BF16
            ? (a_xform == OT_AX_NONE      ? wgrad_split_kernel<OT_AX_NONE, 1>
               : a_xform == OT_AX_RMSNORM ? wgrad_split_kernel<OT_AX_RMSNORM, 1>
               : a_xform == OT_AX_GELU    ? wgrad_split_kernel<OT_AX_GELU, 1>
                                          : wgrad_split_kernel<-1, 1>)
        : split ? (a_xform == OT_AX_NONE      ? wgrad_split_kernel<OT_AX_NONE, SPLIT_TERMS>
                 : a_xform == OT_AX_RMSNORM ? wgrad_split_kernel<OT_AX_RMSNORM, SPLIT_TERMS>
                 : a_xform == OT_AX_GELU    ? wgrad_split_kernel<OT_AX_GELU, SPLIT_TERMS>
                                            : wgrad_split_kernel<-1, SPLIT_TERMS>)
              : (a_xform == OT_AX_NONE      ? wgrad_kernel<OT_AX_NONE>
                 : a_xform == OT_AX_RMSNORM ? wgrad_kernel<OT_AX_RMSNORM>
                 : a_xform == OT_AX_GELU    ? wgrad_kernel<OT_AX_GELU>
                                            : wgrad_kernel<-1>);
    const size_t split_shmem = 2 * WSOP;
    static std::once_flag lds_once;
    std::call_once(lds_once, [] {
      for (void (*k)(WgradArgs) : {wgrad_kernel<OT_AX_NONE>, wgrad_kernel<OT_AX_RMSNORM>, wgrad_kernel<OT_AX_GELU>,
                                   wgrad_kernel<-1>})
        (void)hipFuncSetAttribute((const void*)k, hipFuncAttributeMaxDynamicSharedMemorySize, 4 * WBR * WLD * 4);
      (void)hipGetLastError();
    });
    const size_t copy_shmem = (size_t)WG_LDS;
    if (copy && copy_shmem > 64 * 1024) {
      static std::once_flag copy_once;
      std::call_once(copy_once, [] {
        for (void (*k)(WgradArgs) : {wgrad_bf16_kernel<true>, wgrad_bf16_kernel<false>})
          (void)hipFuncSetAttribute((const void*)k, hipFuncAttributeMaxDynamicSharedMemorySize, WG_LDS);
        (void)hipGetLastError();
      });
    }
    const int wgw = g_wgrad_wide.load(std::memory_order_relaxed);
    if (copy && N % (2 * GT) == 0 && K % (2 * GT) == 0 && (wgw == 1 || wgw == 3)) {
      static std::once_flag sq_once;
      std::call_once(sq_once, [] {
        for (void (*k)(WgradArgs) : {wgrad_bf16_sq_kernel<true>, wgrad_bf16_sq_kernel<false>})
          (void)hipFuncSetAttribute((const void*)k, hipFuncAttributeMaxDynamicSharedMemorySize, WS_LDS);
        (void)hipGetLastError();
      });
      hipLaunchKernelGGL(a_rows ? wgrad_bf16_sq_kernel<true> : wgrad_bf16_sq_kernel<false>,
                         dim3(wgrad_grid(nchunks, (K / (2 * GT)) * (N / (2 * GT)))), dim3(512), (size_t)WS_LDS, s, p);
    } else if (copy && N % (2 * GT) == 0 && wgw) {
      static std::once_flag wide_once;
      std::call_once(wide_once, [] {
        for (void (*k)(WgradArgs) : {wgrad_bf16_wide_kernel<true>, wgrad_bf16_wide_kernel<false>})
          (void)hipFuncSetAttribute((const void*)k, hipFuncAttributeMaxDynamicSharedMemorySize, WW_LDS);
        (void)hipGetLastError();
      });
      hipLaunchKernelGGL(a_rows ? wgrad_bf16_wide_kernel<true> : wgrad_bf16_wide_kernel<false>,
                         dim3(wgrad_grid(nchunks, p.ntk * (N / (2 * GT)))), dim3(256), (size_t)WW_LDS, s, p);
    } else {
      hipLaunchKernelGGL(kern, dim3(wgrad_grid(nchunks, p.ntk * p.ntn)), dim3(256),
                         copy ? copy_shmem : split ? split_shmem : shmem, s, p);
    }
    OT_LAUNCH_CHECK("ot_mixed_gemm_wgrad");
  }
  const int wblocks = (int)ceil_div((int64_t)K * N / 4, 16);
  const int bblocks = (db && N % 4 == 0) ? (int)ceil_div((int64_t)N / 4, 16) : 0;
  dim3 rg(wblocks + bblocks, ngroups);
  hipLaunchKernelGGL(wgrad_reduce_kernel, rg, dim3(256), 0, s, slab, bslab, gchunk, K, N, dW, dw_gstride, db,
                     db_gstride, accumulate, wblocks);
  OT_LAUNCH_CHECK("ot_mixed_gemm_wgrad(reduce)");
  return OT_OK;
}

extern "C" int ot_mixed_gemm_wgrad(const float* A, int64_t lda, const int32_t* a_rows, int a_xform,
                                   const float* a_rstd, const float* a_gamma,
                                   const float* D, int64_t ldd, const int32_t* d_rows, int K, int N,
                                   const int32_t* chunks, int nchunks, const int32_t* gchunk, int ngroups,
                                   float* dW, int64_t dw_gstride, float* db, int64_t db_gstride,
                                   int accumulate, void* workspace, size_t ws_bytes, int precision,
                                   void* stream) {
  return wgrad_impl(A, lda, a_rows, a_xform, a_rstd, a_gamma, D, ldd, d_rows, K, N, chunks, nchunks, gchunk, ngroups,
                    dW, dw_gstride, db, db_gstride, accumulate, workspace, ws_bytes, nullptr, nullptr, precision,
                    stream);
}

extern "C" int ot_mixed_gemm_wgrad_ex(const float* A, int64_t lda, const int32_t* a_rows, int a_xform,
                                      const float* a_rstd, const float* a_gamma,
                                      const float* D, int64_t ldd, const int32_t* d_rows, int K, int N,
                                      const int32_t* chunks, int nchunks, const int32_t* gchunk, int ngroups,
                                      float* dW, int64_t dw_gstride, float* db, int64_t db_gstride,
                                      int accumulate, void* workspace, size_t ws_bytes, const float* a_bound,
                                      const float* d_bound, int precision, void* stream) {
  return wgrad_impl(A, lda, a_rows, a_xform, a_rstd, a_gamma, D, ldd, d_rows, K, N, chunks, nchunks, gchunk, ngroups,
                    dW, dw_gstride, db, db_gstride, accumulate, workspace, ws_bytes, a_bound, d_bound, precision,
                    stream);
}
```

### recommend_amd/kernels.py

```python

from __future__ import annotations

import contextlib
import ctypes
import functools
import os
import threading
from typing import Optional, Tuple, Union

import torch

from . import _lib
from ._lib import call, size

Ptrish = Union[None, torch.Tensor, Tuple[torch.Tensor, int]]


class Probe:

    def __init__(self):
        self.recs = []

    def begin(self):
        ev = torch.cuda.Event(enable_timing=True)
# ... 148 lines not shown

def pyramid_select(B: int, I: int, K: int, pos: torch.Tensor, inv: Optional[torch.Tensor] = None,
                   score: Optional[torch.Tensor] = None, sign: float = 1.0, nforce: int = 0,
                   map_rows: Optional[torch.Tensor] = None, map_per_sample: int = 0) -> None:
    ev = _probe.begin() if _probe is not None else None
    call('ot_pyramid_select', ptr(score), float(sign), B, I, K, nforce, ptr(pos), ptr(inv), ptr(map_rows),
         map_per_sample, stream())
    if ev is not None:
        _probe.end('pyramid', 0.0, ev)


def stream() -> int:
    return torch.cuda.current_stream().cuda_stream


def workspace(nbytes: int, device) -> torch.Tensor:
    return torch.empty(max(int(nbytes), 16), dtype=torch.uint8, device=device)


def gemm(mode: int, A: Ptrish, lda: int, K: int, in_rows: Ptrish, W: Ptrish, w_gstride: int, ldw: int, N: int,
         tile_group: Ptrish, ntiles: int, C: Ptrish, ldc: int, out_rows: Ptrish, *, a_xform: int = 0,
         rstd: Ptrish = None, gamma: Ptrish = None, bias: Ptrish = None, bias_gstride: int = 0, epi: int = 0,
         res: Ptrish = None, ldres: int = 0, res_tok: int = 0, aux: Ptrish = None, ldaux: int = 0,
         seed: int = 0, site: int = 0, drop: float = 0.0, tail: Tuple[int, int] = (1, 1),
         m_rows: int = 0, bimg=None) -> None:
    ev = _probe.begin() if _probe is not None else None
    args = (mode, ptr(A), lda, K, ptr(in_rows), a_xform, ptr(rstd), ptr(gamma), ptr(W), w_gstride,
            ldw, N, ptr(tile_group), ntiles, ptr(bias), bias_gstride, ptr(C), ldc, ptr(out_rows), epi, ptr(res),
            ldres, res_tok, ptr(aux), ldaux, seed & 0xFFFFFFFF, site, float(drop), tail[0], tail[1], _sel(tail))
    if bimg is not None:
        call('ot_mixed_gemm_img', *args, ptr(bimg[0]), bimg[1], bimg[2], _prec(), stream())
    else:
        call('ot_mixed_gemm', *args, _prec(), stream())
    if ev is not None:
        M = m_rows or ntiles * 128
        _probe.end('mixed_gemm', 2.0 * M * K * N, ev, f'gemm mode{mode} ax{a_xform} epi{epi} M{M} K{K} N{N}',
                   gemm_bytes(M, K, N, a_xform, epi), _terms(bimg, a_xform, None, N))


def gemm_rms(mode: int, A: Ptrish, lda: int, K: int, in_rows: Ptrish, W: Ptrish, w_gstride: int, ldw: int,
             N: int, tile_group: Ptrish, ntiles: int, C: Ptrish, ldc: int, out_rows: Ptrish, *, epi: int,
             a_xform: int = 0, rstd: Ptrish = None, gamma: Ptrish = None, bias: Ptrish = None,
             bias_gstride: int = 0, res: Ptrish = None, ldres: int = 0, res_tok: int = 0, seed: int = 0,
             site: int = 0, drop: float = 0.0, tail: Tuple[int, int] = (1, 1), m_rows: int = 0,
             rstd_out: Ptrish = None, eps: float = 1e-6, nx: Ptrish = None, ldnx: int = 0,
             ngamma: Ptrish = None, nrstd: Ptrish = None, dres: Ptrish = None, lddres: int = 0,
             dres_tail: Tuple[int, int] = (0, 0), dx_masked: Ptrish = None, lddxm: int = 0,
             dgamma: Ptrish = None, accumulate_dgamma: bool = False, device=None, bimg=None,
             aux: Ptrish = None, ldaux: int = 0, rowdot: Ptrish = None, rowdot_n: int = 0,
             gelu_out: Ptrish = None, ldgelu: int = 0, xn_out: Ptrish = None, ldxn: int = 0,
             c16_out: Ptrish = None, ldc16: int = 0, rowmax_out: Ptrish = None, rowmax_n: int = 0,
             a_rowmax: Ptrish = None, a_rowmax_n: int = 0, amax_out: Ptrish = None, rowabs_out: Ptrish = None,
             rowabs_n: int = 0) -> None:
    need_ws = dgamma is not None or (rstd_out is not None and N > 128)
    ws = workspace(size('ot_mixed_gemm_rms_workspace_size', ntiles, N) if need_ws else 16,
                   device if device is not None else (C[0] if isinstance(C, tuple) else C).device)
    e = _lib.RmsEpilogue(ctypes.sizeof(_lib.RmsEpilogue), ptr(rstd_out), float(eps), ptr(nx), ldnx, ptr(ngamma), ptr(nrstd), ptr(dres), lddres,
                         dres_tail[0], dres_tail[1], _sel(dres_tail), ptr(dx_masked), lddxm, ptr(dgamma),
                         int(accumulate_dgamma), ptr(ws), ws.numel(), ptr(rowdot), int(rowdot_n),
                         ptr(gelu_out), int(ldgelu), ptr(xn_out), int(ldxn), ptr(c16_out), int(ldc16),
                         ptr(rowmax_out), int(rowmax_n), ptr(a_rowmax), int(a_rowmax_n), ptr(amax_out),
                         ptr(rowabs_out), int(rowabs_n))
    ev = _probe.begin() if _probe is not None else None
    args = (mode, ptr(A), lda, K, ptr(in_rows), a_xform, ptr(rstd), ptr(gamma), ptr(W),
            w_gstride, ldw, N, ptr(tile_group), ntiles, ptr(bias), bias_gstride, ptr(C), ldc, ptr(out_rows), epi,
            ptr(res), ldres, res_tok, ptr(aux), ldaux, seed & 0xFFFFFFFF, site, float(drop), tail[0], tail[1],
            _sel(tail), ctypes.byref(e))
    if bimg is not None:
        call('ot_mixed_gemm_rms_img', *args, ptr(bimg[0]), bimg[1], bimg[2], _prec(), stream())
    else:
        call('ot_mixed_gemm_rms', *args, _prec(), stream())
    if ev is not None:
        M = m_rows or ntiles * 128
        extra = (nx is not None) + (dres is not None) + (dx_masked is not None)
        _probe.end('mixed_gemm', 2.0 * M * K * N, ev, f'gemm_rms mode{mode} ax{a_xform} epi{epi} M{M} K{K} N{N}',
                   gemm_bytes(M, K, N, a_xform, epi) + 4.0 * M * N * extra + 2.0 * M * N * (gelu_out is not None)
                   + 2.0 * M * K * (xn_out is not None)
                   + 4.0 * M * ((rstd_out is not None) + (nrstd is not None)), _terms(bimg, a_xform, a_rowmax, N))


def wgrad(A: Ptrish, lda: int, a_rows: Ptrish, D: Ptrish, ldd: int, d_rows: Ptrish, K: int, N: int, rmap_dev,
          nchunks: int, ngroups: int, dW: Ptrish, dw_gstride: int, db: Ptrish = None, db_gstride: int = 0, *,
          a_xform: int = 0, rstd: Ptrish = None, gamma: Ptrish = None, accumulate: bool = False,
          device=None, m_rows: int = 0, rowmap=None, a_bound: Ptrish = None, d_bound: Ptrish = None) -> None:
    if rowmap is not None and rowmap.group_rows:
        tiles = ((K + 127) // 128) * ((N + 127) // 128)
        ch, gc, nchunks = rowmap.chunks_for(tiles, device)
        rmap_dev = {'chunks': ch, 'gchunk': gc}
    nbytes = size('ot_wgrad_workspace_size', nchunks, K, N)
    ws = workspace(nbytes, device)
    ev = _probe.begin() if _probe is not None else None
    call('ot_mixed_gemm_wgrad_ex', ptr(A), lda, ptr(a_rows), a_xform, ptr(rstd), ptr(gamma), ptr(D), ldd,
         ptr(d_rows), K, N, ptr(rmap_dev['chunks']), nchunks, ptr(rmap_dev['gchunk']), ngroups, ptr(dW),
         dw_gstride, ptr(db), db_gstride, int(accumulate), ptr(ws), ws.numel(), ptr(a_bound), ptr(d_bound), _prec(),
         stream())
    if ev is not None:
        ax = a_xform & ~_lib.OT_WG_D_BF16
        wterms = {'bf16': 1, 'f32': 0}.get(matmul_mode(), 3 if (
            d_bound is not None and not (a_xform & _lib.OT_WG_D_BF16)
            and (ax == _lib.OT_AX_RMSNORM or (a_bound is not None and ax in (_lib.OT_AX_NONE, _lib.OT_AX_GELU))))
            else 6)
        _probe.end('mixed_gemm', 2.0 * m_rows * K * N, ev, f'wgrad ax{a_xform} M{m_rows} K{K} N{N} ch{nchunks}',
                   (2.0 if (a_xform & ~_lib.OT_WG_D_BF16) == _lib.OT_AX_BF16 else 4.0) * m_rows * K
                   + (2.0 if a_xform & _lib.OT_WG_D_BF16 else 4.0) * m_rows * N
                   + 4.0 * m_rows * ((a_xform & ~_lib.OT_WG_D_BF16) == _lib.OT_AX_RMSNORM) + 4.0 * ngroups * K * N,
                   wterms)


def transpose_banks(src, dst, banks_dev, nbanks, total_tiles) -> None:
    call('ot_transpose_banks', ptr(src), ptr(dst), ptr(banks_dev), nbanks, total_tiles, stream())


def split_image_elems(G: int, N: int, K: int) -> int:
    return int(_lib.load().ot_split_image_elems(G, N, K))


def plane_wide(on: int = -1) -> int:
    return _lib.size('ot_plane_wide', int(on))


def wgrad_wide(on: int = -1) -> int:
    return _lib.size('ot_wgrad_wide', int(on))


def plane_rowmeta(on: int = -1) -> int:
    return _lib.size('ot_plane_rowmeta', int(on))


def plane_panel(on: int = -1) -> int:
    return _lib.size('ot_plane_panel', int(on))


def plane_panel_launches() -> int:
    return _lib.size('ot_plane_panel_launches')


def ffn_fused(on: int = -1) -> int:
    return _lib.size('ot_ffn_fused', int(on))


FFN_FUSED_MAX_F = 1024


def ffn_fused_fwd(x1: Ptrish, ldx1: int, rows: Ptrish, tile_group: Ptrish, ntiles: int, rstd: Ptrish, w1_image,
                  w1_groups: int, w2_image, w2_groups: int, b1: Ptrish, b1_gstride: int, b2: Ptrish, b2_gstride: int,
                  f: int, x2: Ptrish, ldx2: int, *, u_out: Ptrish = None, ldu: int = 0, u_amax: Ptrish = None,
                  rstd_out: Ptrish = None, eps: float = 1e-6, seed: int = 0, site: int = 0, drop: float = 0.0,
                  tail: Tuple[int, int] = (1, 1), m_rows: int = 0) -> None:
    a = _lib.FfnFusedArgs(ctypes.sizeof(_lib.FfnFusedArgs), ptr(x1), ldx1, ptr(rows), ptr(tile_group), ntiles,
                          ptr(rstd), ptr(w1_image), int(w1_groups), ptr(w2_image), int(w2_groups), ptr(b1),
                          b1_gstride, ptr(b2), b2_gstride, f, ptr(u_out), ldu, ptr(u_amax), ptr(x2), ldx2,
                          ptr(rstd_out), float(eps), seed & 0xFFFFFFFF, site, float(drop), tail[0], tail[1],
                          _sel(tail))
    ev = _probe.begin() if _probe is not None else None
    call('ot_ffn_fused_fwd', ctypes.byref(a), stream())
    if ev is not None:
        M = m_rows or ntiles * 128
        _probe.end('mixed_gemm', 2.0 * M * 128 * f * 2, ev, f'ffn_fused M{M} f{f} u{int(u_out is not None)}',
                   4.0 * M * 128 * 3 + 4.0 * M * f * (u_out is not None)
                   + 4.0 * M * (1 + (rstd_out is not None)), 3)


def ffn_fused_bwd_on(on: int = -1) -> int:
    return _lib.size('ot_ffn_fused_bwd_on', int(on))


def ffn_fused_bwd(dy2: Ptrish, lddy2: int, dy2_rowmax: Ptrish, dy2_rowmax_n: int, rows: Ptrish, tile_group: Ptrish,
                  ntiles: int, w2_image, w2_groups: int, w1_image, w1_groups: int, f: int, u: Ptrish, ldu: int,
                  du: Ptrish, lddu: int, x1: Ptrish, ldx1: int, gamma: Ptrish, rstd: Ptrish, dx1: Ptrish, lddx1: int,
                  dgamma: Ptrish, *, du_amax: Ptrish = None, dres: Ptrish = None, lddres: int = 0,
                  dx_masked: Ptrish = None, lddxm: int = 0, accumulate_dgamma: bool = False, amax_out: Ptrish = None,
                  rowabs_out: Ptrish = None, rowabs_n: int = 0, seed: int = 0, site: int = 0, drop: float = 0.0,
                  tail: Tuple[int, int] = (1, 1), m_rows: int = 0, device=None) -> None:
    ws = workspace(size('ot_mixed_gemm_rms_workspace_size', ntiles, 128),
                   device if device is not None else (dx1[0] if isinstance(dx1, tuple) else dx1).device)
    a = _lib.FfnFusedBwdArgs(ctypes.sizeof(_lib.FfnFusedBwdArgs), ptr(dy2), lddy2, ptr(dy2_rowmax), int(dy2_rowmax_n),
                             ptr(rows), ptr(tile_group), ntiles, ptr(w2_image), int(w2_groups), ptr(w1_image),
                             int(w1_groups), f, ptr(u), ldu, ptr(du), lddu, ptr(du_amax), ptr(x1), ldx1, ptr(gamma),
                             ptr(rstd), ptr(dres), lddres, ptr(dx1), lddx1, ptr(dx_masked), lddxm, ptr(dgamma),
                             int(accumulate_dgamma), ptr(ws), ws.numel(), ptr(amax_out), ptr(rowabs_out),
                             int(rowabs_n), seed & 0xFFFFFFFF, site, float(drop), tail[0], tail[1], _sel(tail))
    ev = _probe.begin() if _probe is not None else None
    call('ot_ffn_fused_bwd', ctypes.byref(a), stream())
    if ev is not None:
        M = m_rows or ntiles * 128
        _probe.end('mixed_gemm', 2.0 * M * 128 * f * 2, ev, f'ffn_fused_bwd M{M} f{f} drop{int(drop > 0)}',
                   4.0 * M * 128 * (3 + (dres is not None) + (dx_masked is not None)) + 4.0 * M * f * 2
                   + 4.0 * M * (1 + dy2_rowmax_n), 3)


def split_images(base, desc_dev, ndesc, total_units, img) -> None:
    call('ot_split_images', ptr(base), ptr(desc_dev), ndesc, total_units, ptr(img), _prec(), stream())


def attn_fwd(qkv: torch.Tensor, ld: int, B: int, H: int, I: int, K: int, hd: int, out: torch.Tensor,
             lse: torch.Tensor, qpos: Optional[torch.Tensor] = None, fp8: bool = False,
             dequant: bool = False, fp8_terms: int = 1, deq16: Optional[torch.Tensor] = None,
             amax: Optional[torch.Tensor] = None, rowmax: Optional[torch.Tensor] = None) -> None:
    if fp8 and fp8_terms not in (1, 2):
        raise ValueError(f'fp8_terms {fp8_terms}: 1 or 2')
    ws = None
    if fp8:
        ws = workspace(size('ot_attn_fwd_fp8_workspace_size', B, H, I, hd), qkv.device)
    ev = _probe.begin() if _probe is not None else None
    if fp8 and deq16 is not None:
        call('ot_attn_fwd_fp8_deq16', ptr(qkv), ld, B, H, I, K, ptr(qpos), hd, ptr(out), ptr(lse), ptr(ws),
             ws.numel(), _lib.OT_FP8_TWO_TERM if fp8_terms == 2 else 0, ptr(deq16), stream())
    elif fp8:
        call('ot_attn_fwd_fp8_ex', ptr(qkv), ld, B, H, I, K, ptr(qpos), hd, ptr(out), ptr(lse), ptr(ws),
             ws.numel(), (_lib.OT_FP8_DEQUANT if dequant else 0) | (_lib.OT_FP8_TWO_TERM if fp8_terms == 2 else 0),
             stream())
    elif amax is not None or rowmax is not None:
        call('ot_attn_fwd_amax', ptr(qkv), ld, B, H, I, K, ptr(qpos), hd, ptr(out), ptr(lse), ptr(amax), ptr(rowmax),
             _prec(), stream())
    else:
        call('ot_attn_fwd', ptr(qkv), ld, B, H, I, K, ptr(qpos), hd, ptr(out), ptr(lse), _prec(), stream())
    if ev is not None:
        _probe.end('attention', 4.0 * (K * I - K * (K - 1) / 2) * hd * H * B, ev,
                   f'fwd{"_fp8" if fp8 else ""} I{I} K{K} hd{hd}')


def attn_bwd_bf16_forms(I, K, hd, qpos=None) -> int:
    return int(_lib.load().ot_attn_bwd_bf16_forms(I, K, hd, int(qpos is not None), _prec()))


def attn_bwd_bf16_supported(I, K, hd, qpos=None) -> bool:
    return bool(_lib.load().ot_attn_bwd_dqkv_bf16_supported(I, K, hd, int(qpos is not None), _prec()))


def attn_amax_supported(I, K, hd, qpos=None, backward: bool = False) -> bool:
    return bool(_lib.load().ot_attn_amax_supported(I, K, hd, int(qpos is not None), _prec()) & (2 if backward else 1))


def attn_bwd(qkv, ld, out, dout, lse, B, H, I, K, hd, dqkv, qpos=None, dq_part_bf16: bool = False,
             amax=None, rowmax=None) -> None:
    flags = ((_lib.OT_ATTN_DQKV_BF16 if dqkv.dtype == torch.int16 else 0)
             | (_lib.OT_ATTN_QKV_BF16 if qkv.dtype == torch.int16 else 0)
             | (_lib.OT_ATTN_DQ_PART_BF16 if dq_part_bf16 and dqkv.dtype == torch.int16
                and attn_bwd_bf16_forms(I, K, hd, qpos) & _lib.OT_ATTN_DQ_PART_BF16 else 0))
    ws = workspace(size('ot_attn_bwd_flags_workspace_size', B, H, I, K, hd, int(qpos is not None), flags, _prec()),
                   qkv.device)
    ev = _probe.begin() if _probe is not None else None
    if amax is not None or rowmax is not None:
        call('ot_attn_bwd_amax', ptr(qkv), ld, ptr(out), ptr(dout), ptr(lse), B, H, I, K, ptr(qpos), hd, ptr(dqkv),
             ptr(ws), ws.numel(), ptr(amax), ptr(rowmax), _prec(), stream())
    else:
        call('ot_attn_bwd_flags', ptr(qkv), ld, ptr(out), ptr(dout), ptr(lse), B, H, I, K, ptr(qpos), hd,
             ptr(dqkv), flags, ptr(ws), ws.numel(), _prec(), stream())
    if ev is not None:
        _probe.end('attention', 8.0 * (K * I - K * (K - 1) / 2) * hd * H * B, ev, f'bwd I{I} K{K} hd{hd}')


def last_fold(on: int = -1) -> int:
    return _lib.size('ot_last_fold', int(on))


def attn_fold_supported(d: int, H: int) -> bool:
    return bool(_lib.size('ot_attn_fold_supported', int(d), int(H)))


def attn_fold_rows(I: int, ded0: int, ded1: int) -> int:
    return _lib.size('ot_attn_fold_rows', int(I), int(ded0), int(ded1))


def _fold_common(x, ldx, rstd, gamma, w, ldw, wT, ldwT, qkv, ldqkv, B, H, I, hd, ded):
    return (ptr(x), ldx, ptr(rstd), ptr(gamma), ptr(w), ldw, ptr(wT), ldwT, ptr(qkv), ldqkv, B, H, I, hd, ded[0],
# ... 84 lines not shown


def attn_fwd_cached_kv16(qkv, ld, kv16, ldc16, req_stride, req, C, H, Ic, n, Kq, hd, out, cache_valid=None,
                         lse=None) -> None:
    if kv16 is not None and kv16.dtype != torch.bfloat16:
        raise TypeError(f'attn_fwd_cached_kv16: a bfloat16 cache is expected, got {kv16.dtype}')
    cv, ldcv = _valid_arg(cache_valid) if cache_valid is not None else (None, 0)
    ev = _probe.begin() if _probe is not None else None
    call('ot_attn_fwd_cached_kv16', ptr(qkv), ld, ptr(kv16), ldc16, req_stride, ptr(req), C, H, Ic, n, Kq, hd, cv,
         ldcv, ptr(out), ptr(lse), stream())
    if ev is not None:
        _probe.end('attention', 4.0 * (Kq * (Ic + n) - Kq * (Kq - 1) / 2) * hd * H * C, ev,
                   f'fwd_cached_kv16 Ic{Ic} n{n} K{Kq} hd{hd}')


def seq_key_valid(lens, seq_len, seq_off, B: int, L0: int, valid0, rank=None) -> None:
    n = len(seq_len)
    arr = ctypes.c_int32 * max(1, n)
    sl, so = arr(*seq_len), arr(*seq_off)
    call('ot_seq_key_valid', ptr(lens), ctypes.cast(sl, ctypes.c_void_p), ctypes.cast(so, ctypes.c_void_p), n, B, L0,
         ptr(rank),
         rank.shape[1] if rank is not None else 0, ptr(valid0), stream())


def attn_fwd_cached(qkv, ld, kv_cache, ldc, req, C, H, Ic, n, Kq, hd, out, lse=None) -> None:
    ev = _probe.begin() if _probe is not None else None
    args = (ptr(qkv), ld, ptr(kv_cache), ldc, ptr(req), C, H, Ic, n, Kq, hd, ptr(out))
    if lse is None:
        call('ot_attn_fwd_cached', *args, stream())
    else:
        call('ot_attn_fwd_cached_lse', *args, ptr(lse), stream())
    if ev is not None:
        _probe.end('attention', 4.0 * (Kq * (Ic + n) - Kq * (Kq - 1) / 2) * hd * H * C, ev,
                   f'fwd_cached{"" if lse is None else "_lse"} Ic{Ic} n{n} K{Kq} hd{hd}')


attn_fwd_cached_lse = attn_fwd_cached


def attn_bwd_cached(qkv, ld, kv_cache, ldc, req_start, R, C, H, Ic, n, Kq, hd, out, dout, lse, dqkv, dkv_cache,
                    accumulate: bool = False) -> None:
    ws = workspace(size('ot_attn_bwd_cached_workspace_size', R, C, H, Ic, n, Kq, hd), qkv.device)
    ev = _probe.begin() if _probe is not None else None
    call('ot_attn_bwd_cached', ptr(qkv), ld, ptr(kv_cache), ldc, ptr(req_start), R, C, H, Ic, n, Kq, hd, ptr(out),
         ptr(dout), ptr(lse), ptr(dqkv), ptr(dkv_cache), int(bool(accumulate)), ptr(ws), ws.numel(), stream())
    if ev is not None:
        _probe.end('attention', (8.0 * (Kq * n - Kq * (Kq - 1) / 2) + 14.0 * Kq * Ic) * hd * H * C, ev,
                   f'bwd_cached Ic{Ic} n{n} K{Kq} hd{hd}')


def rmsnorm_fwd(x: Ptrish, ldx: int, rows: int, d: int, rstd: Ptrish, gamma: Ptrish = None, y: Ptrish = None,
                ldy: int = 0, eps: float = 1e-6) -> None:
    ev = _probe.begin() if _probe is not None else None
    call('ot_rmsnorm_fwd', ptr(x), ldx, ptr(gamma), ptr(y), ldy, ptr(rstd), rows, d, eps, stream())
    if ev is not None:
        _probe.end('rowwise', 0.0, ev)


def rmsnorm_bwd(dy: Ptrish, lddy: int, x: Ptrish, ldx: int, gamma: Ptrish, rstd: Ptrish, dx: Ptrish, lddx: int,
                rows: int, d: int, *, dres: Ptrish = None, lddres: int = 0, dres_tail=(0, 0), dx_masked: Ptrish = None,
                lddxm: int = 0, seed: int = 0, site: int = 0, drop: float = 0.0, tail=(1, 1),
                dgamma: Ptrish = None, accumulate: bool = False, device=None) -> None:
    nbytes = size('ot_rmsnorm_bwd_workspace_size', rows, d) if dgamma is not None else 16
    ws = workspace(nbytes, device)
    ev = _probe.begin() if _probe is not None else None
    call('ot_rmsnorm_bwd', ptr(dy), lddy, ptr(x), ldx, ptr(gamma), ptr(rstd), ptr(dres), lddres, dres_tail[0],
         dres_tail[1], _sel(dres_tail), ptr(dx), lddx, ptr(dx_masked), lddxm, seed & 0xFFFFFFFF, site, float(drop),
         tail[0], tail[1], _sel(tail), ptr(dgamma), int(accumulate), rows, d, ptr(ws), ws.numel(), stream())
    if ev is not None:
        _probe.end('rowwise', 0.0, ev)


def dropout_apply(src, lds, dst, ldd, rows, d, seed, site, drop, tail, amax=None, rowmax=None) -> None:
    ev = _probe.begin() if _probe is not None else None
    if amax is not None or rowmax is not None:
        call('ot_dropout_apply_ex', ptr(src), lds, ptr(dst), ldd, rows, d, seed & 0xFFFFFFFF, site, float(drop),
             tail[0], tail[1], _sel(tail), ptr(amax), ptr(rowmax), (d + 255) // 256 if rowmax is not None else 0,
             stream())
    else:
        fn = 'ot_dropout_apply_bf16' if getattr(dst, 'dtype', None) == torch.int16 else 'ot_dropout_apply'
        call(fn, ptr(src), lds, ptr(dst), ldd, rows, d, seed & 0xFFFFFFFF, site, float(drop), tail[0],
             tail[1], _sel(tail), stream())
    if ev is not None:
        _probe.end('rowwise', 0.0, ev)


def dropout_rowmax_supported(d: int) -> bool:
    return bool(_lib.load().ot_dropout_rowmax_supported(d))


def rows_absmax(x, ldx, rows, d, out) -> None:
    ev = _probe.begin() if _probe is not None else None
    call('ot_rows_absmax', ptr(x), ldx, rows, d, ptr(out), (d + 255) // 256, stream())
    if ev is not None:
        _probe.end('rowwise', 0.0, ev)


def rows_colsum(src, ld, rows: Ptrish, nrows: int, ncols: int, out: Ptrish, accumulate=False, device=None) -> None:
    ws = workspace(size('ot_rows_colsum_workspace_size', nrows, ncols), device)
    ev = _probe.begin() if _probe is not None else None
    call('ot_rows_colsum', ptr(src), ld, ptr(rows), nrows, ncols, ptr(out), int(accumulate), ptr(ws), ws.numel(),
         stream())
    if ev is not None:
        _probe.end('rowwise', 0.0, ev)


def ns_assemble(fields_dev, nfields, table, B, out, ld_out) -> None:
    ev = _probe.begin() if _probe is not None else None
    call('ot_ns_assemble', ptr(fields_dev), nfields, ptr(table), B, ptr(out), ld_out, stream())
    if ev is not None:
        _probe.end('embedding', 0.0, ev)


def ns_grad_pack(fields_dev, nsparse, width, dmat, ld, B, keys, grads) -> None:
    ev = _probe.begin() if _probe is not None else None
    call('ot_ns_grad_pack', ptr(fields_dev), nsparse, width, ptr(dmat), ld, B, ptr(keys), ptr(grads), stream())
    if ev is not None:
        _probe.end('embedding', 0.0, ev)


def fill_rows(dst, ld, rows, nrows, vec, d) -> None:
    ev = _probe.begin() if _probe is not None else None
    call('ot_fill_rows', ptr(dst), ld, ptr(rows), nrows, ptr(vec), d, stream())
    if ev is not None:
        _probe.end('embedding', 0.0, ev)


def seq_rows(ids, stride_b, B, L, vocab, in_rows) -> None:
    ev = _probe.begin() if _probe is not None else None
    call('ot_seq_rows', ptr(ids), stride_b, B, L, vocab, ptr(in_rows), stream())
    if ev is not None:
        _probe.end('embedding', 0.0, ev)


def head_fwd(pre1, w2, b2, T, B, dh, logits, probs) -> None:
    ev = _probe.begin() if _probe is not None else None
    call('ot_head_fwd', ptr(pre1), ptr(w2), ptr(b2), T, B, dh, ptr(logits), ptr(probs), stream())
    if ev is not None:
        _probe.end('head_loss', 0.0, ev)


def head_bwd(pre1, w2, probs, dprobs, T, B, dh, dpre1, dw2, db2, sw2, sb2, accumulate=False, device=None,
             dlogits=None) -> None:
    ws = workspace(size('ot_head_bwd_workspace_size', T, B, dh), device)
    ev = _probe.begin() if _probe is not None else None
    call('ot_head_bwd_ex', ptr(pre1), ptr(w2), ptr(probs), ptr(dprobs), ptr(dlogits), T, B, dh, ptr(dpre1), ptr(dw2),
         ptr(db2), sw2, sb2, int(accumulate), ptr(ws), ws.numel(), stream())
    if ev is not None:
        _probe.end('head_loss', 0.0, ev)


def bce_fwd(probs, labels, T, B, loss, device=None, mse_mask: int = 0) -> None:
    ws = workspace(size('ot_bce_workspace_size', T, B), device)
    ev = _probe.begin() if _probe is not None else None
    call('ot_task_loss_fwd', ptr(probs), ptr(labels), T, B, mse_mask, ptr(loss), ptr(ws), ws.numel(), stream())
    if ev is not None:
        _probe.end('head_loss', 0.0, ev)


def bce_bwd(probs, labels, gscale, T, B, dprobs, mse_mask: int = 0) -> None:
    ev = _probe.begin() if _probe is not None else None
    call('ot_task_loss_bwd', ptr(probs), ptr(labels), ptr(gscale), T, B, mse_mask, ptr(dprobs), stream())
    if ev is not None:
        _probe.end('head_loss', 0.0, ev)


def metrics_update(probs, labels, T, B, task_stride, bounds, nb, counts, sums, device=None) -> None:
    ws = workspace(size('ot_metrics_workspace_size', T, B), device)
    ev = _probe.begin() if _probe is not None else None
    call('ot_metrics_update', ptr(probs), ptr(labels), T, B, task_stride, ptr(bounds), nb, ptr(counts), ptr(sums),
         ptr(ws), ws.numel(), stream())
    if ev is not None:
        _probe.end('metrics', 0.0, ev)


def grouped_auc(groups, scores, labels, T, n, task_stride, group_bits, task_mask, agg, num_groups, group_ids=None,
                group_stats=None, device=None) -> None:
    ws = workspace(size('ot_grouped_auc_workspace_size', T, n, group_bits), device)
# ... 201 lines not shown
```

### recommend_amd/model.py

```python

from __future__ import annotations

import json
import os
from typing import Dict, List, Optional, Tuple

import numpy as np
import torch
import torch.nn as nn

from . import _lib
from . import kernels as K
from ._lib import (OT_AX_BF16, OT_AX_BF16_RMSNORM, OT_AX_GELU, OT_AX_RMSNORM, OT_EPI_ACCUMULATE, OT_EPI_AUX_BF16, OT_EPI_BIAS,
                   OT_EPI_C_BF16, OT_EPI_DROPOUT, OT_EPI_GELU_BWD, OT_EPI_RESIDUAL, OT_EPI_RMSNORM_BWD,
                   OT_EPI_ROW_RSTD, OT_EPI_ROWDOT, OT_GEMM_NN, OT_GEMM_NT, OT_WG_D_BF16, NS_FIELD_BYTES)
from .config import (OneTransConfig, check_bag_features, check_ns_tokenizer, check_padding_mask, check_pyramid_select,
                     check_seq_fusion, get_model_config)
from .layout import TILE, FlatLayout, RowMap, build_map, head_map, identity_map, layer_maps, round_up
from .params import init_params, ns_table_offsets

RMS_EPS = 1e-6
NS_GROUPS_KEY = '__ns_token_groups__'


# ... 59 lines not shown
                                      m.layout.f_pad, m.ns_kmax, B, d, m.g('tok.ns.kernel'), m.g('tok.ns.bias'),
                                      accumulate=acc, device=dev)
            else:
                K.wgrad(nsm, m.layout.f_pad, mp['rows'][0], (dx0, L_S * d), L0 * d, mp['rows'][0], m.layout.f_pad,
                        m.cfg_Lnsd, mp, plan['ns_map'].chunks.shape[0], 1, m.g('tok.ns.kernel'), 0,
                        m.g('tok.ns.bias'), 0, accumulate=acc, device=dev, m_rows=B, rowmap=plan['ns_map'])
            if plan['n_sparse'] > 0 or plan['n_bags'] > 0:
                dns = torch.empty(B, m.layout.f_pad, device=dev)
                if grouped:
                    K.ns_group_bwd_input((dx0, L_S * d), L0 * d, m.ns_goff, m.config.num_ns_tokens, m.layout.f_pad,
                                         m.ns_kmax, m.p('tok.ns.kernel'), B, d, dns, m.layout.f_pad)
                else:
                    K.gemm(OT_GEMM_NT, (dx0, L_S * d), L0 * d, m.cfg_Lnsd, mp['rows'][0], m.p('tok.ns.kernel'), 0,
                           m.cfg_Lnsd, m.layout.f_pad, mp['tile_group'], plan['ns_map'].ntiles, dns, m.layout.f_pad,
                           mp['rows'][0], m_rows=B)
                e = m.config.ns_embedding_dim
                n1 = plan['n_sparse'] * B
                n = n1 + plan['bag_ns_slots']
                if n > 0:
                    keys = torch.empty(n, dtype=torch.int64, device=dev)
                    grads = torch.empty(n, e, device=dev)
                    if n1 > 0:
                        K.ns_grad_pack(plan['ns_desc'], plan['n_sparse'], e, dns, m.layout.f_pad, B, keys, grads)
                    if plan['n_bags_ns'] > 0:
                        K.ns_bag_grad_pack(plan['bag_descs'], plan['n_bags_ns'], B, dns, m.layout.f_pad,
                                           plan['bag_coef'], (keys, n1), (grads, n1 * e))
                    m._pending_sparse.append(('emb.ns', keys, grads))
                nq = plan['n_bags'] - plan['n_bags_ns']
                if nq > 0:
                    Eq = m.config.seq_feature_dim
                    nslots = plan['bag_slots'] - plan['bag_ns_slots']
                    keys = torch.empty(nslots, dtype=torch.int64, device=dev)
                    grads = torch.empty(nslots, Eq, device=dev)
                    K.ns_bag_grad_pack(plan['bag_descs'], nq, B, dns, m.layout.f_pad,
                                       (plan['bag_coef'], plan['bag_ns_slots']), keys, grads, first=plan['n_bags_ns'])
                    m._pending_sparse.append(('emb.seq_item', keys, grads))
        elif not acc:
            m.g('tok.ns.kernel').zero_()
            m.g('tok.ns.bias').zero_()
        E = m.config.seq_feature_dim
        if plan['seq_map'] is not None:
            sm = plan['seq_map'].to(dev)
            xrows = _seq_out_rows(plan, sm)
            K.wgrad(plan['seq_A'], E, plan['seq_in'], dx0, d, xrows, E, d, sm,
                    plan['seq_map'].chunks.shape[0], plan['nseq'], m.g('tok.seq.kernel'), E * d,
                    m.g('tok.seq.bias'), d, accumulate=acc, device=dev, m_rows=plan['seq_M'],
                    rowmap=plan['seq_map'])
            if plan['seq_ids'] is not None:
                M = plan['seq_M']
                demb = torch.empty(M, E, device=dev)
                K.gemm(OT_GEMM_NT, dx0, d, d, xrows, m.p('tok.seq.kernel'), E * d, d, E, sm['tile_group'],
                       plan['seq_map'].ntiles, demb, E, sm['rows'][1], m_rows=plan['seq_M'])
                keys = plan['seq_route'] if 'emb.seq_item' in m.sharded else plan['seq_ids']
                m._pending_sparse.append(('emb.seq_item', keys, demb))
        elif not acc:
            m.g('tok.seq.kernel').zero_(); m.g('tok.seq.bias').zero_()
        if plan['n_sep'] > 0:
            K.rows_colsum(dx0, d, plan['sep_rows'], plan['n_sep'], d, m.g('tok.sep'), accumulate=acc, device=dev)
        elif not acc:
            m.g('tok.sep').zero_()
        m.join_side_stream()
        return None, None, None


def _seq_out_rows(plan, sm):
    rows = plan.get('seq_rows_t')
    return rows if rows is not None else sm['rows'][0]


def layer_seed(seed: int, b0: int, I: int, d: int) -> int:
    return (seed + b0 * I * d * 0x9E3779B1) & 0xFFFFFFFF if b0 else seed


def _layer_valid(kvalid, I):
    L0 = kvalid.shape[1]
    return kvalid, L0 - I, L0


def _attn_qpos(cfg, pos):
    return None if getattr(cfg, 'pyramid_select', 'tail') == 'tail' else pos


class PairBounds:
    SLOTS = ('o', 'u', 'dy2', 'du', 'dyo', 'dqkv')

    def __init__(self, layers: int, device):
        self.t, self._taken = torch.zeros(layers, 8, device=device), {}

    @classmethod
    def begin(cls, layers: int, device, mode: str, pair_wgrad: bool) -> Optional['PairBounds']:
        return cls(layers, device) if mode == 'split' and pair_wgrad and torch.is_grad_enabled() else None

    def out(self, l: int, name: str) -> torch.Tensor:
        return self._taken.setdefault((l, name), self.t[l, self.SLOTS.index(name):][:1])

    def get(self, l: int, name: str) -> Optional[torch.Tensor]:
        return self._taken.get((l, name))


def a_row_bounds(on: bool, x, ld: int, rows: int, n: int, reported=None) -> Dict:
    if on and reported is None:
        reported = torch.empty(rows, (n + 255) // 256, device=x.device)
        K.rows_absmax(x, ld, rows, n, reported)
    return dict(a_rowmax=reported, a_rowmax_n=reported.shape[1]) if on else {}


def _block_forward(m, l, x, I, Kq, seed, training, rstd_in=None, select=False, need_out=True, need_u=True,
                   bounds=None, kvalid=None):
    cfg = m.config
    d, f, H = cfg.hidden_dim, cfg.ffn_dim, cfg.num_heads
    hd = d // H
    B = x.shape[0] // I
    dev = x.device
    maps = m.maps(B, I, Kq)
    ma, mt = maps['all'].to(dev), maps['tail'].to(dev)
    na, nt = maps['all'].ntiles, maps['tail'].ntiles
    rate = cfg.dropout_rate if training else 0.0
    dflag = OT_EPI_DROPOUT if rate > 0 else 0
    wqkv, wo = m.pT(f'blk.{l}.wqkv'), m.pT(f'blk.{l}.wo')
    w1, b1, w2, b2 = m.pT(f'blk.{l}.w1'), m.p(f'blk.{l}.b1'), m.pT(f'blk.{l}.w2'), m.p(f'blk.{l}.b2')
    g1, g2 = m.p(f'blk.{l}.norm1'), m.p(f'blk.{l}.norm2')
    fuse = m.fuse_with((f'blk.{l}.wo', 'fwd'), (f'blk.{l}.w2', 'fwd'))
    if rstd_in is not None and rstd_in.numel() == B * I:
        rstd1 = rstd_in
    else:
        rstd1 = torch.empty(B * I, device=dev)
        K.rmsnorm_fwd(x, d, B * I, d, rstd1, eps=RMS_EPS)
    qrows, pos, inv = mt['rows'][0], None, None
    if select:
        pos = torch.empty(B * Kq, dtype=torch.int32, device=dev)
        inv = torch.empty(B * I, dtype=torch.int32, device=dev)
        if cfg.pyramid_select == 'norm':
            nf = min(cfg.num_ns_tokens, Kq)
            qrows = qrows.clone()
            K.pyramid_select(B, I, Kq, pos, inv, score=rstd1, sign=-1.0, nforce=nf, map_rows=qrows,
                             map_per_sample=Kq - nf)
        else:
            K.pyramid_select(B, I, Kq, pos, inv)
    tail = (Kq, I, pos)
    x16 = m.take_x16(l, x) if d % TILE == 0 and need_out else None
    ax1 = OT_AX_BF16_RMSNORM if x16 is not None else OT_AX_RMSNORM
    xa = x16 if x16 is not None else x
    qkv = torch.empty(B * I, 3 * d, device=dev)
    xn_on = (training and K.matmul_mode() == 'bf16' and d % TILE == 0
             and m.bimg(f'blk.{l}.wqkv') is not None)
    xn1 = torch.empty(B * I, d, dtype=torch.int16, device=dev) if xn_on else None
    x1n = torch.empty(B * Kq, d, dtype=torch.int16, device=dev) if xn_on else None
    fold = m.fold_gate(I, Kq, select, kvalid)
    yf = None
    if xn1 is not None:
        full = Kq == I
        K.gemm_rms(OT_GEMM_NT, xa, d, d, ma['rows'][0], wqkv if full else (wqkv, d * d), 3 * d * d, d,
                   3 * d if full else 2 * d, ma['tile_group'], na, qkv if full else (qkv, d), 3 * d, ma['rows'][0],
                   epi=0, a_xform=ax1, rstd=rstd1, gamma=g1, m_rows=maps['all'].nrows, device=dev,
                   bimg=m.bimg(f'blk.{l}.wqkv') if full else m.bimg(f'blk.{l}.wqkv', tn0=d // TILE),
                   xn_out=xn1, ldxn=d)
        if not full:
            K.gemm(OT_GEMM_NT, xa, d, d, qrows, wqkv, 3 * d * d, d, d, mt['tile_group'], nt, qkv,
                   3 * d, qrows, a_xform=ax1, rstd=rstd1, gamma=g1, m_rows=maps['tail'].nrows,
                   bimg=m.bimg(f'blk.{l}.wqkv'))
    elif Kq == I:
        K.gemm(OT_GEMM_NT, xa, d, d, ma['rows'][0], wqkv, 3 * d * d, d, 3 * d, ma['tile_group'], na, qkv,
               3 * d, ma['rows'][0], a_xform=ax1, rstd=rstd1, gamma=g1, m_rows=maps['all'].nrows,
               bimg=m.bimg(f'blk.{l}.wqkv'))
    else:
        mkv, kvm = (maps['fold'].to(dev), maps['fold']) if fold is not None else (ma, maps['all'])
        K.gemm(OT_GEMM_NT, xa, d, d, mkv['rows'][0], (wqkv, d * d), 3 * d * d, d, 2 * d, mkv['tile_group'],
               kvm.ntiles, (qkv, d), 3 * d, mkv['rows'][0], a_xform=ax1, rstd=rstd1, gamma=g1, m_rows=kvm.nrows,
               bimg=m.bimg(f'blk.{l}.wqkv', tn0=d // TILE) if d % TILE == 0 else None)
        K.gemm(OT_GEMM_NT, xa, d, d, qrows, wqkv, 3 * d * d, d, d, mt['tile_group'], nt, qkv,
               3 * d, qrows, a_xform=ax1, rstd=rstd1, gamma=g1, m_rows=maps['tail'].nrows,
               bimg=m.bimg(f'blk.{l}.wqkv'))
    o = torch.empty(B * Kq, d, device=dev)
    lse = torch.empty(B * H * Kq, device=dev)
    qp_f = _attn_qpos(cfg, pos)
    qkv16 = (torch.empty(B * I, 3 * d, dtype=torch.int16, device=dev)
             if m.attn_fp8 and training and K.attn_bwd_bf16_supported(I, Kq, hd, qp_f) else None)
    out = (lambda name: bounds.out(l, name)) if bounds is not None else (lambda name: None)
    pwo_f = m.gemm_pair(f'blk.{l}.wo', 'fwd')
    o_rep = kvalid is None and not m.attn_fp8 and fold is None and K.attn_amax_supported(I, Kq, hd, qp_f)
    rm_o = torch.empty(B * Kq, H, device=dev) if pwo_f and o_rep else None
    if fold is not None:
        yf = torch.empty(B * H, d, device=dev)
        K.attn_fold_fwd(x, d, rstd1, g1, m.p(f'blk.{l}.wqkv'), 3 * d, wqkv, d, qkv, 3 * d, B, H, I, hd, fold, o, lse,
                        yf)
    elif kvalid is not None:
        K.attn_fwd_masked(qkv, 3 * d, B, H, I, Kq, hd, o, lse, _layer_valid(kvalid, I), qpos=qp_f)
# ... 66 lines not shown
        return None, None, saved, pos, inv, rate
    x2 = torch.empty(B * Kq, d, device=dev)
    rstd_out = None
    a2, ax2 = (h, OT_AX_BF16) if h is not None else (u, OT_AX_GELU)
    pa_u = a_row_bounds(pair_w2, u, f, B * Kq, f, umax)
    if fuse:
        rstd_out = torch.empty(B * Kq, device=dev)
        x2_16 = torch.empty(B * Kq, d, dtype=torch.int16, device=dev) if m.x16_on(d) and w2img is not None else None
        K.gemm_rms(OT_GEMM_NT, a2, f, f, mt['rows'][1], w2, f * d, f, d, mt['tile_group'], nt, x2, d,
                   mt['rows'][1], a_xform=ax2, bias=b2, bias_gstride=d,
                   epi=OT_EPI_BIAS | OT_EPI_RESIDUAL | dflag | OT_EPI_ROW_RSTD, res=x1, ldres=d, res_tok=0,
                   seed=seed, site=2 * l + 1, drop=rate, tail=tail, m_rows=maps['tail'].nrows,
                   rstd_out=rstd_out, eps=RMS_EPS, bimg=w2img, c16_out=x2_16, ldc16=d, **pa_u)
        m.put_x16(l + 1, x2, x2_16)
    elif umax is not None:
        K.gemm_rms(OT_GEMM_NT, a2, f, f, mt['rows'][1], w2, f * d, f, d, mt['tile_group'], nt, x2, d, mt['rows'][1],
                   a_xform=ax2, bias=b2, bias_gstride=d, epi=OT_EPI_BIAS | OT_EPI_RESIDUAL | dflag, res=x1,
                   ldres=d, res_tok=0, seed=seed, site=2 * l + 1, drop=rate, tail=tail,
                   m_rows=maps['tail'].nrows, bimg=w2img, **pa_u)
    else:
        K.gemm(OT_GEMM_NT, a2, f, f, mt['rows'][1], w2, f * d, f, d, mt['tile_group'], nt, x2, d, mt['rows'][1],
               a_xform=ax2, bias=b2, bias_gstride=d, epi=OT_EPI_BIAS | OT_EPI_RESIDUAL | dflag, res=x1,
               ldres=d, res_tok=0, seed=seed, site=2 * l + 1, drop=rate, tail=tail,
               m_rows=maps['tail'].nrows, bimg=w2img)
    return x2, rstd_out, saved, pos, inv, rate


class _Block(torch.autograd.Function):

    @staticmethod
    def forward(ctx, flat, x, m, l, I, Kq, seed, training, rstd_in=None, select=False, bounds=None, kvalid=None):
        x2, rstd_out, saved, pos, inv, rate = _block_forward(
            m, l, x, I, Kq, seed, training, rstd_in, select, bounds=bounds,
            need_u=not m.recompute and any(ctx.needs_input_grad), kvalid=kvalid)
        if m.recompute:
            ctx.save_for_backward(saved[0], saved[1])
            ctx.fwd_args = (training, select)
        else:
            ctx.save_for_backward(*saved)
        ctx.m, ctx.l, ctx.I, ctx.Kq, ctx.seed, ctx.rate = m, l, I, Kq, seed, rate
        ctx.pos, ctx.inv, ctx.bounds, ctx.kvalid = pos, inv, bounds, kvalid
        if rstd_out is None:
            rstd_out = x2.new_empty(0)
        ctx.mark_non_differentiable(rstd_out)
        return x2, rstd_out

    @staticmethod
    def backward(ctx, dx2, _drstd=None):
        with K.precision(ctx.m.matmul):
            return _Block._backward(ctx, dx2, _drstd)

    @staticmethod
    def _backward(ctx, dx2, _drstd=None):
        m, l, I, Kq, seed, rate = ctx.m, ctx.l, ctx.I, ctx.Kq, ctx.seed, ctx.rate
        pos, inv, bounds, kvalid = ctx.pos, ctx.inv, ctx.bounds, ctx.kvalid
        if m.recompute:
            xin, rstd_in = ctx.saved_tensors
            training, select = ctx.fwd_args
            _, _, saved, pos, inv, _ = _block_forward(m, l, xin, I, Kq, seed, training, rstd_in, select,
                                                      need_out=False, bounds=bounds, kvalid=kvalid)
            x, rstd1, qkv, o, lse, x1, rstd2, u, h, xn1, x1n, yf = saved
        else:
            x, rstd1, qkv, o, lse, x1, rstd2, u, h, xn1, x1n, yf = ctx.saved_tensors
        tail = (Kq, I, pos)
        cfg = m.config
        d, f, H = cfg.hidden_dim, cfg.ffn_dim, cfg.num_heads
        hd = d // H
        B = x.shape[0] // I
        dev = x.device
        acc = m.accumulate_grads
        maps = m.maps(B, I, Kq)
        ma, mt = maps['all'].to(dev), maps['tail'].to(dev)
        na, nt = maps['all'].ntiles, maps['tail'].ntiles
        nca, nct = maps['all'].chunks.shape[0], maps['tail'].chunks.shape[0]
        G = cfg.num_groups
        dx2 = dx2.contiguous()
        rowdot = None
        fused2 = m.fuse_bwd2 and not m.fuse_bwd and f % TILE == 0
        du_bf = (fused2 and h is not None and m.bimg(f'blk.{l}.w1', 'dgrad') is not None)
        out = (lambda name: bounds.out(l, name)) if bounds is not None else (lambda name: None)
        b_o, b_u = (bounds.get(l, 'o'), bounds.get(l, 'u')) if bounds is not None else (None, None)
        keep = (bounds.t,) if bounds is not None else ()
        pw2, pw1, pwo = (m.dgrad_pair(f'blk.{l}.{w}') for w in ('w2', 'w1', 'wo'))
        dy2_rep = rate > 0 and not du_bf
        b_dy2 = out('dy2') if dy2_rep else None
        rm_dy2 = (torch.empty(B * Kq, (d + 255) // 256, device=dev)
                  if dy2_rep and pw2 and K.dropout_rowmax_supported(d) else None)
        dy2 = dx2
        if rate > 0:
            dy2 = torch.empty(B * Kq, d, device=dev, dtype=torch.int16 if du_bf else torch.float32)
            K.dropout_apply(dx2, d, dy2, d, B * Kq, d, seed, 2 * l + 1, rate, tail, amax=b_dy2, rowmax=rm_dy2)
        pa2 = a_row_bounds(pw2, dy2, d, B * Kq, d, rm_dy2)
        dy_bf = dy2.dtype == torch.int16
        du = torch.empty(B * Kq, f, device=dev, dtype=torch.int16 if du_bf else torch.float32)
        cbf = OT_EPI_C_BF16 if du_bf else 0
        hbf = (torch.empty(B * Kq, f, dtype=torch.int16, device=dev)
               if h is None and fused2 and K.matmul_mode() == 'bf16' else None)
        if hbf is None:
            with m.side(u if h is None else h, dy2, *keep):
                K.wgrad(u if h is None else h, f, mt['rows'][1], dy2, d, mt['rows'][1], f, d, mt, nct, G,
                        m.g(f'blk.{l}.w2'), f * d, m.g(f'blk.{l}.b2'), d,
                        a_xform=(OT_AX_GELU if h is None else OT_AX_BF16) | (OT_WG_D_BF16 if dy_bf else 0),
                        accumulate=acc, device=dev, m_rows=maps['tail'].nrows, rowmap=maps['tail'],
                        a_bound=b_u if h is None else None, d_bound=b_dy2)
        du_rep = fused2 or (((bounds is not None and not du_bf) or pw2 or pw1) and f % TILE == 0)
        b_du = out('du') if du_rep and not du_bf else None
        ffn_bwd = (pw2 and pw1 and m.fuse_bwd and d == TILE and f % TILE == 0 and f <= K.FFN_FUSED_MAX_F
                   and not du_bf and h is None and bool(K.ffn_fused_bwd_on()))
        rm_du = torch.empty(B * Kq, f // TILE, device=dev) if pw1 and du_rep and not ffn_bwd else None
        rep_du = dict(amax_out=b_du, rowabs_out=rm_du, rowabs_n=f // TILE if rm_du is not None else 0)
        if ffn_bwd:
            dx1 = torch.empty(B * Kq, d, device=dev)
            dyo = torch.empty(B * Kq, d, device=dev) if rate > 0 else dx1
            rm_dyo = torch.empty(B * Kq, 1, device=dev) if pwo else None
            b_dyo = out('dyo')
            K.ffn_fused_bwd(dy2, d, pa2['a_rowmax'], pa2['a_rowmax_n'], mt['rows'][1], mt['tile_group'], nt,
                            m.bimg(f'blk.{l}.w2', 'dgrad')[0], m.layout.images[(f'blk.{l}.w2', 'dgrad')][1],
                            m.bimg(f'blk.{l}.w1', 'dgrad')[0], m.layout.images[(f'blk.{l}.w1', 'dgrad')][1], f,
                            u, f, du, f, x1, d, m.p(f'blk.{l}.norm2'), rstd2, dx1, d, m.g(f'blk.{l}.norm2'),
                            du_amax=b_du, dres=dx2, lddres=d, dx_masked=dyo if rate > 0 else None, lddxm=d,
                            accumulate_dgamma=acc, amax_out=b_dyo, rowabs_out=rm_dyo,
                            rowabs_n=1 if rm_dyo is not None else 0, seed=seed, site=2 * l, drop=rate, tail=tail,
                            m_rows=maps['tail'].nrows, device=dev)
        elif fused2:
            rowdot = torch.empty(B * Kq, f // TILE, device=dev)
            K.gemm_rms(OT_GEMM_NT, dy2, d, d, mt['rows'][1], m.p(f'blk.{l}.w2'), f * d, d, f, mt['tile_group'], nt,
                       du, f, mt['rows'][1], aux=u, ldaux=f, a_xform=OT_AX_BF16 if dy_bf else 0,
                       epi=OT_EPI_GELU_BWD | OT_EPI_ROWDOT | cbf | (OT_EPI_AUX_BF16 if u.dtype == torch.int16 else 0),
                       bias=m.p(f'blk.{l}.b1'), bias_gstride=f, rowdot=rowdot, rowdot_n=f // TILE,
                       m_rows=maps['tail'].nrows, device=dev, bimg=m.bimg(f'blk.{l}.w2', 'dgrad'),
                       gelu_out=hbf, ldgelu=f, **rep_du, **pa2)
            if hbf is not None:
                with m.side(hbf, dy2):
                    K.wgrad(hbf, f, mt['rows'][1], dy2, d, mt['rows'][1], f, d, mt, nct, G, m.g(f'blk.{l}.w2'),
                            f * d, m.g(f'blk.{l}.b2'), d, a_xform=OT_AX_BF16, accumulate=acc, device=dev,
                            m_rows=maps['tail'].nrows, rowmap=maps['tail'])
        else:
            K.gemm_rms(OT_GEMM_NT, dy2, d, d, mt['rows'][1], m.p(f'blk.{l}.w2'), f * d, d, f, mt['tile_group'], nt, du,
                       f, mt['rows'][1], epi=OT_EPI_GELU_BWD, aux=u, ldaux=f, m_rows=maps['tail'].nrows, device=dev,
                       bimg=m.bimg(f'blk.{l}.w2', 'dgrad'), **rep_du, **pa2)
        pa1 = a_row_bounds(pw1, du, f, B * Kq, f, rm_du) if not ffn_bwd else {}
        a1n = x1n is not None and du_bf
        with m.side(x1n if a1n else x1, du, rstd2, *keep):
            K.wgrad(x1n if a1n else x1, d, mt['rows'][1], du, f, mt['rows'][1], d, f, mt, nct, G, m.g(f'blk.{l}.w1'),
                    d * f, m.g(f'blk.{l}.b1'), f, rstd=rstd2, gamma=m.p(f'blk.{l}.norm2'),
                    a_xform=(OT_AX_BF16 if a1n else OT_AX_RMSNORM) | (OT_WG_D_BF16 if du_bf else 0),
                    accumulate=acc, device=dev, m_rows=maps['tail'].nrows, rowmap=maps['tail'], d_bound=b_du)
        dx1_ep = m.fuse_bwd or rowdot is not None
        if not ffn_bwd:
            dx1 = torch.empty(B * Kq, d, device=dev)
            dyo = torch.empty(B * Kq, d, device=dev) if rate > 0 else dx1
            rm_dyo = torch.empty(B * Kq, (d + TILE - 1) // TILE, device=dev) if pwo and dx1_ep else None
            b_dyo = out('dyo') if dx1_ep else None
        if ffn_bwd:
            pass
        elif dx1_ep:
            K.gemm_rms(OT_GEMM_NT, du, f, f, mt['rows'][1], m.p(f'blk.{l}.w1'), d * f, f, d, mt['tile_group'], nt,
                       dx1, d, mt['rows'][1], epi=OT_EPI_RMSNORM_BWD | (OT_EPI_DROPOUT if rate > 0 else 0),
                       a_xform=OT_AX_BF16 if du_bf else 0,
                       seed=seed, site=2 * l, drop=rate, tail=tail, m_rows=maps['tail'].nrows, nx=x1, ldnx=d,
                       ngamma=m.p(f'blk.{l}.norm2'), nrstd=rstd2, dres=dx2, lddres=d,
                       dx_masked=dyo if rate > 0 else None, lddxm=d, dgamma=m.g(f'blk.{l}.norm2'),
                       accumulate_dgamma=acc, device=dev, bimg=m.bimg(f'blk.{l}.w1', 'dgrad'),
                       rowdot=rowdot, rowdot_n=f // TILE if rowdot is not None else 0, amax_out=b_dyo,
                       rowabs_out=rm_dyo, rowabs_n=rm_dyo.shape[1] if rm_dyo is not None else 0, **pa1)
        else:
            dxn2 = torch.empty(B * Kq, d, device=dev)
            K.gemm_rms(OT_GEMM_NT, du, f, f, mt['rows'][1], m.p(f'blk.{l}.w1'), d * f, f, d, mt['tile_group'], nt,
                       dxn2, d, mt['rows'][1], epi=0, m_rows=maps['tail'].nrows, device=dev,
                       bimg=m.bimg(f'blk.{l}.w1', 'dgrad'), **pa1)
            K.rmsnorm_bwd(dxn2, d, x1, d, m.p(f'blk.{l}.norm2'), rstd2, dx1, d, B * Kq, d, dres=dx2, lddres=d,
                          dx_masked=dyo if rate > 0 else None, lddxm=d, seed=seed, site=2 * l, drop=rate,
                          tail=tail, dgamma=m.g(f'blk.{l}.norm2'), accumulate=acc, device=dev)
        with m.side(o, dyo, *keep):
            _wgrad_single(m, o, dyo, d, d, mt, m.g(f'blk.{l}.wo'), acc, dev, maps['tail'].nrows, maps['tail'],
                          a_bound=b_o, d_bound=b_dyo)
        do = torch.empty(B * Kq, d, device=dev)
        K.gemm_rms(OT_GEMM_NT, dyo, d, d, mt['rows'][1], m.p(f'blk.{l}.wo'), 0, d, d, mt['tile_group'], nt, do, d,
                   mt['rows'][1], epi=0, m_rows=maps['tail'].nrows, device=dev, bimg=m.bimg(f'blk.{l}.wo', 'dgrad'),
                   **a_row_bounds(pwo, dyo, d, B * Kq, d, rm_dyo))
        if yf is not None:
            dx = _fold_backward(m, l, x, rstd1, qkv, o, lse, yf, do, dx1, B, I, maps['fold'], acc, dev)
            m.side_block_done()
            if m.grad_ready is not None:
                m.grad_ready(l)
            return None, dx, None, None, None, None, None, None, None, None, None, None
        qp = _attn_qpos(cfg, pos)
        dq_bf = (K.matmul_mode() == 'bf16'
                 and K.attn_bwd_bf16_forms(I, Kq, hd, qp) & _lib.OT_ATTN_DQKV_BF16
                 and m.bimg(f'blk.{l}.wqkv', 'dgrad') is not None)
        dqkv = torch.empty(B * I, 3 * d, device=dev, dtype=torch.int16 if dq_bf else torch.float32)
        if Kq < I:
            dqkv[:, :d].zero_()
        bwd_b = kvalid is None and not dq_bf and K.attn_amax_supported(I, Kq, hd, qp, backward=True)
        b_dq = out('dqkv') if bwd_b else None
        pqkv = m.dgrad_pair(f'blk.{l}.wqkv')
        rm_dq = torch.zeros(B * I, 3 * H, device=dev) if pqkv and bwd_b else None
        if kvalid is not None:
            K.attn_bwd_masked(qkv, 3 * d, o, do, lse, B, H, I, Kq, hd, dqkv, _layer_valid(kvalid, I), qpos=qp)
        else:
            K.attn_bwd(qkv, 3 * d, o, do, lse, B, H, I, Kq, hd, dqkv, qpos=qp, dq_part_bf16=True, amax=b_dq,
                       rowmax=rm_dq)
        pa_q = a_row_bounds(pqkv, dqkv, 3 * d, B * I, 3 * d, rm_dq)
        an1 = xn1 is not None and dq_bf
        with m.side(xn1 if an1 else x, dqkv, rstd1, *keep):
            K.wgrad(xn1 if an1 else x, d, ma['rows'][0], dqkv, 3 * d, ma['rows'][0], d, 3 * d, ma, nca, G,
                    m.g(f'blk.{l}.wqkv'), 3 * d * d, None, 0,
                    a_xform=(OT_AX_BF16 if an1 else OT_AX_RMSNORM) | (OT_WG_D_BF16 if dq_bf else 0), rstd=rstd1,
                    gamma=m.p(f'blk.{l}.norm1'), accumulate=acc, device=dev, m_rows=maps['all'].nrows,
                    rowmap=maps['all'], d_bound=b_dq)
        ax_dq = OT_AX_BF16 if dq_bf else 0
        dx = torch.empty(B * I, d, device=dev)
        if m.fuse_bwd:
            K.gemm_rms(OT_GEMM_NT, dqkv, 3 * d, 3 * d, ma['rows'][0], m.p(f'blk.{l}.wqkv'), 3 * d * d, 3 * d, d,
                       ma['tile_group'], na, dx, d, ma['rows'][0], epi=OT_EPI_RMSNORM_BWD, a_xform=ax_dq,
                       m_rows=maps['all'].nrows, nx=x, ldnx=d, ngamma=m.p(f'blk.{l}.norm1'), nrstd=rstd1,
                       dres=dx1, lddres=d, dres_tail=(Kq, I, inv) if Kq < I else (0, 0),
                       dgamma=m.g(f'blk.{l}.norm1'), accumulate_dgamma=acc, device=dev,
                       bimg=m.bimg(f'blk.{l}.wqkv', 'dgrad'), **pa_q)
        else:
            dxn1 = torch.empty(B * I, d, device=dev)
            K.gemm_rms(OT_GEMM_NT, dqkv, 3 * d, 3 * d, ma['rows'][0], m.p(f'blk.{l}.wqkv'), 3 * d * d, 3 * d, d,
                       ma['tile_group'], na, dxn1, d, ma['rows'][0], epi=0, m_rows=maps['all'].nrows, a_xform=ax_dq,
                       bimg=m.bimg(f'blk.{l}.wqkv', 'dgrad'), device=dev, **pa_q)
            K.rmsnorm_bwd(dxn1, d, x, d, m.p(f'blk.{l}.norm1'), rstd1, dx, d, B * I, d, dres=dx1, lddres=d,
                          dres_tail=(Kq, I, inv) if Kq < I else (0, 0), dgamma=m.g(f'blk.{l}.norm1'), accumulate=acc,
                          device=dev)
        m.side_block_done()
        if m.grad_ready is not None:
            m.grad_ready(l)
        return None, dx, None, None, None, None, None, None, None, None, None, None


def _fold_backward(m, l, x, rstd1, qkv, o, lse, yf, do, dx1, B, I, fmap, acc, dev):
    cfg = m.config
    d, H, G = cfg.hidden_dim, cfg.num_heads, cfg.num_groups
    hd = d // H
    ded = m.fold_ded(I)
    mf = fmap.to(dev)
    nf = K.attn_fold_rows(I, *ded)
    g1, w = m.p(f'blk.{l}.norm1'), m.p(f'blk.{l}.wqkv')
    dqkv = torch.empty(B * nf, 3 * d, device=dev)
    dx = torch.empty(B * I, d, device=dev)
    zf = torch.empty(B * H, d, device=dev)
    dgp = torch.empty(B, d, device=dev)
    K.attn_fold_bwd(x, d, rstd1, g1, w, 3 * d, m.pT(f'blk.{l}.wqkv'), d, qkv, 3 * d, B, H, I, hd, ded, o, do, lse, yf,
                    dx1, dx, d, dqkv, 3 * d, zf, dgp)
    pa_q = a_row_bounds(m.dgrad_pair(f'blk.{l}.wqkv'), dqkv, 3 * d, B * nf, 3 * d)
    K.gemm_rms(OT_GEMM_NT, dqkv, 3 * d, 3 * d, mf['rows'][1], w, 3 * d * d, 3 * d, d, mf['tile_group'], fmap.ntiles,
               dx, d, mf['rows'][0], epi=OT_EPI_RMSNORM_BWD, m_rows=fmap.nrows, nx=x, ldnx=d, ngamma=g1, nrstd=rstd1,
               dres=dx, lddres=d, dgamma=m.g(f'blk.{l}.norm1'), accumulate_dgamma=acc, device=dev,
               bimg=m.bimg(f'blk.{l}.wqkv', 'dgrad'), **pa_q)
    K.attn_fold_dgamma(dgp, B, d, m.g(f'blk.{l}.norm1'), accumulate=True)
    with m.side(x, dqkv, rstd1, zf, yf, qkv, do):
        K.wgrad(x, d, mf['rows'][0], dqkv, 3 * d, mf['rows'][1], d, 3 * d, mf, fmap.chunks.shape[0], G,
                m.g(f'blk.{l}.wqkv'), 3 * d * d, None, 0, a_xform=OT_AX_RMSNORM, rstd=rstd1, gamma=g1, accumulate=acc,
                device=dev, m_rows=fmap.nrows, rowmap=fmap)
        K.attn_fold_dw(zf, yf, qkv, 3 * d, do, g1, B, H, I, hd, m.g(f'blk.{l}.wqkv'), 3 * d, accumulate=True)
    return dx


def _wgrad_single(m, A, D, K_, N, mt, dW, acc, dev, mrows=0, rowmap=None, a_bound=None, d_bound=None):
    if rowmap is not None and rowmap.group_rows:
        ch, _, _ = rowmap.chunks_for(((K_ + 127) // 128) * ((N + 127) // 128), dev)
        mp = m.single_group_chunks({'chunks': ch})
    else:
        mp = m.single_group_chunks(mt)
    K.wgrad(A, K_, mt['rows'][1], D, N, mt['rows'][1], K_, N, mp, mp['chunks'].shape[0], 1, dW, 0, None, 0,
            accumulate=acc, device=dev, m_rows=mrows, a_bound=a_bound, d_bound=d_bound)


class _Head(torch.autograd.Function):

    @staticmethod
    def forward(ctx, flat, x, m):
        cfg = m.config
        d, T = cfg.hidden_dim, len(cfg.tasks)
        dh = d // 2
        B = x.shape[0]
        dev = x.device
        y = torch.empty(B, d, device=dev)
        rstd = torch.empty(B, device=dev)
        K.rmsnorm_fwd(x, d, B, d, rstd, gamma=m.p('out_norm'), y=y, ldy=d, eps=RMS_EPS)
        hm = m.head_rows(B)
        hmd = hm.to(dev)
        pre1 = torch.empty(T * B, dh, device=dev)
        K.gemm(OT_GEMM_NT, y, d, d, hmd['rows'][0], m.pT('head.w1'), d * dh, d, dh, hmd['tile_group'], hm.ntiles,
               pre1, dh, hmd['rows'][1], bias=m.p('head.b1'), bias_gstride=dh, epi=OT_EPI_BIAS, m_rows=hm.nrows)
        logits = torch.empty(T, B, device=dev)
        probs = torch.empty(T, B, device=dev)
        K.head_fwd(pre1, m.p('head.w2'), m.p('head.b2'), T, B, dh, logits, probs)
        ctx.save_for_backward(x, rstd, y, pre1, probs)
        ctx.m = m
        ctx.set_materialize_grads(False)
        m._last_logits = logits
        return probs, logits

    @staticmethod
    def backward(ctx, dprobs, dlogits):
        with K.precision(ctx.m.matmul):
            return _Head._backward(ctx, dprobs, dlogits)

# ... 808 lines not shown
```

Before: 207,600 samples/s.

## Fuse backward dropout mask into fused FFN dgrad and W2 wgrad via keep bits

Instead of materialising a dropped-out copy of dx2 with a separate dropout_apply pass, the fused FFN backward kernel regenerates the dropout mask in-kernel, applies it to the A operand, and writes packed keep bits. The W2 weight-gradient kernel then reads those keep bits to mask and scale D on the fly. The row abs-max bounds for dx are produced as an epilogue of the previous layer's QKV dgrad and reused, which avoids an extra rows_absmax pass. This removes a full f32 write/read of the dropped activation and a separate rowwise kernel. In exchange it adds hash work and LDS in the fused kernel, plus a keep-bit load in wgrad.

```diff
diff --git a/include/onetrans_hip.h b/include/onetrans_hip.h
--- a/include/onetrans_hip.h
+++ b/include/onetrans_hip.h
@@ -34,6 +34,7 @@
 #define OT_EPI_C_BF16 512
 #define OT_EPI_AUX_BF16 1024
 #define OT_WG_D_BF16 8
+#define OT_WG_D_KEEPBITS 16
 
 int ot_version(void);
 const char* ot_get_last_error_string(void);
@@ -100,6 +101,14 @@
                            int accumulate, void* workspace, size_t ws_bytes, const float* a_bound,
                            const float* d_bound, int precision, void* stream);
 
+int ot_mixed_gemm_wgrad_keep(const float* A, int64_t lda, const int32_t* a_rows, int a_xform,
+                             const float* D, int64_t ldd, const int32_t* d_rows, int K, int N,
+                             const int32_t* chunks, int nchunks, const int32_t* gchunk, int ngroups,
+                             float* dW, int64_t dw_gstride, float* db, int64_t db_gstride,
+                             int accumulate, void* workspace, size_t ws_bytes, const float* a_bound,
+                             const float* d_bound, const uint32_t* keep, int64_t ldkeep, float d_scale,
+                             int precision, void* stream);
+
 int ot_transpose_banks(const float* src, float* dst, const int64_t* banks_dev, int nbanks, int64_t total_tiles,
                        void* stream);
 
@@ -180,6 +189,9 @@
 } ot_ffn_fused_bwd_args;
 int ot_ffn_fused_bwd(const ot_ffn_fused_bwd_args* args, void* stream);
 int ot_ffn_fused_bwd_on(int on);
+int ot_ffn_fused_bwd_mask(const ot_ffn_fused_bwd_args* args, uint32_t mask_site, uint32_t* keep_out, int64_t ldkeep,
+                          void* stream);
+int ot_bwd_mask_fused(int on);
 
 int ot_attn_fwd(const float* qkv, int64_t ld, int B, int H, int I, int K, const int32_t* qpos,
                 int head_dim, float* out, float* lse, int precision, void* stream);
diff --git a/recommend_amd/_lib.py b/recommend_amd/_lib.py
--- a/recommend_amd/_lib.py
+++ b/recommend_amd/_lib.py
@@ -20,6 +20,7 @@
 OT_ATTN_QKV_BF16 = 2
 OT_ATTN_DQ_PART_BF16 = 4
 OT_WG_D_BF16 = 8
+OT_WG_D_KEEPBITS = 16
 OT_MATMUL_F32, OT_MATMUL_SPLIT_BF16, OT_MATMUL_BF16 = 0, 1, 2
 OT_FP8_DEQUANT, OT_FP8_TWO_TERM = 1, 2
 OT_RANK_SUM, OT_RANK_PRODUCT = 0, 1
@@ -107,6 +108,8 @@
                                     I64, P, I64, c_int, P, c_size_t, c_int, P]),
     'ot_mixed_gemm_wgrad_ex': (c_int, [P, I64, P, c_int, P, P, P, I64, P, c_int, c_int, P, c_int, P, c_int, P,
                                        I64, P, I64, c_int, P, c_size_t, P, P, c_int, P]),
+    'ot_mixed_gemm_wgrad_keep': (c_int, [P, I64, P, c_int, P, I64, P, c_int, c_int, P, c_int, P, c_int, P, I64, P,
+                                         I64, c_int, P, c_size_t, P, P, P, I64, c_float, c_int, P]),
     'ot_transpose_banks': (c_int, [P, P, P, c_int, I64, P]),
     'ot_mixed_gemm_img': (c_int, [c_int, P, I64, c_int, P, c_int, P, P, P, I64, I64, c_int, P, c_int, P, I64,
                                   P, I64, P, c_int, P, I64, c_int, P, I64, c_uint32, c_uint32, c_float, c_int,
@@ -124,6 +127,8 @@
     'ot_ffn_fused': (c_int, [c_int]),
     'ot_ffn_fused_bwd': (c_int, [P, P]),
     'ot_ffn_fused_bwd_on': (c_int, [c_int]),
+    'ot_ffn_fused_bwd_mask': (c_int, [P, c_uint32, P, I64, P]),
+    'ot_bwd_mask_fused': (c_int, [c_int]),
     'ot_split_images': (c_int, [P, P, c_int, I64, P, c_int, P]),
     'ot_attn_fwd': (c_int, [P, I64, c_int, c_int, c_int, c_int, P, c_int, P, P, c_int, P]),
     'ot_attn_fwd_fp8_workspace_size': (c_size_t, [c_int, c_int, c_int, c_int]),
diff --git a/recommend_amd/csrc/gemm_ffn.hip b/recommend_amd/csrc/gemm_ffn.hip
--- a/recommend_amd/csrc/gemm_ffn.hip
+++ b/recommend_amd/csrc/gemm_ffn.hip
@@ -267,8 +267,9 @@
 static std::atomic<int> g_ffn_fused{ffn_fused_initial()};
 
 constexpr int FB_TAB_OFF = FF_TAB_OFF;
-static_assert(FB_TAB_OFF + (FF_MAX_F + GT) * 4 <= 80 * 1024, "fused FFN backward LDS");
-constexpr int ffn_bwd_lds(int f) { return FB_TAB_OFF + (f + GT) * 4; }
+constexpr int FB_KEEP_BYTES = GT * (GT / 8);
+static_assert(FB_TAB_OFF + (FF_MAX_F + GT) * 4 + FB_KEEP_BYTES <= 80 * 1024, "fused FFN backward LDS");
+constexpr int ffn_bwd_lds(int f, bool mask = false) { return FB_TAB_OFF + (f + GT) * 4 + (mask ? FB_KEEP_BYTES : 0); }
 
 struct FfnBwdArgs {
   GemmArgs e;
@@ -278,9 +279,10 @@
   float* du; int64_t lddu;
   float* du_amax;
   int f;
+  uint32_t a_site; uint32_t* keep_out; int64_t ldkeep;
 };
 
-template <int EPIT>
+template <int EPIT, bool MASKA = false>
 __global__ __launch_bounds__(256, 2) void ffn_fused_bwd_kernel(FfnBwdArgs q) {
   const GemmArgs& p = q.e;
   extern __shared__ __attribute__((aligned(16))) float smem[];
@@ -355,6 +357,20 @@
     mrow = p.out_rows ? p.out_rows[gr] : (int)gr;
     ir = ir < 0 ? 0 : ir;
     for (int j = 0; j < p.a_rowmax_n; ++j) abound = fmaxf(abound, p.a_rowmax[(int64_t)ir * p.a_rowmax_n + j]);
+    if constexpr (MASKA) {
+      abound *= p.drop_scale;
+      unsigned char* kb = reinterpret_cast<unsigned char*>(lds + FB_TAB_OFF + (q.f + GT) * 4) + ra * (GT / 8) + h;
+      const uint32_t base = (uint32_t)(tail_token(ir, p.tail_K, p.tail_I, p.tail_pos) * GT) + 8 * h;
+      const uint32_t h0 = base * 0x9E3779B1u + p.seed, sx = q.a_site * 0x85EBCA77u;
+#pragma unroll
+      for (int kt = 0; kt < 8; ++kt) {
+        uint32_t b = 0;
+#pragma unroll
+        for (int e = 0; e < 8; ++e)
+          b |= (uint32_t)(fmix32((h0 + (uint32_t)(16 * kt + e) * 0x9E3779B1u) ^ sx) >= p.drop_thr) << e;
+        kb[2 * kt] = (unsigned char)b;
+      }
+    }
   }
   float* tab = reinterpret_cast<float*>(lds + FB_TAB_OFF);
   int tt = t;
@@ -371,6 +387,15 @@
   }
   int* rmeta = reinterpret_cast<int*>(lds + FF_META_OFF);
   if (h == 0) rmeta[ra] = mrow;
+  if constexpr (MASKA) {
+    __syncthreads();
+    if (tt < GT) {
+      const int kr = rmeta[tt];
+      if (kr >= 0)
+        *reinterpret_cast<u32x4*>(q.keep_out + (int64_t)kr * q.ldkeep) =
+            *reinterpret_cast<const u32x4*>(lds + FB_TAB_OFF + (q.f + GT) * 4 + tt * (GT / 8));
+    }
+  }
   const float asc = pow2_scale14(abound);
   const float ainv = 1.f / asc;
   float* trw = reinterpret_cast<float*>(lds + FF_TR_OFF + wave * FF_TR_WAVE);
@@ -417,7 +442,14 @@
         for (int pl = 0; pl < 2; ++pl) fb[nb][pl] = *reinterpret_cast<const u32x4*>(sb + boff + pl * 4096 + nb * 1024);
       const f32x4 a0 = *reinterpret_cast<const f32x4*>(sb + aoff0);
       const f32x4 a1 = *reinterpret_cast<const f32x4*>(sb + (aoff0 ^ 16));
-      const float av[8] = {a0.x, a0.y, a0.z, a0.w, a1.x, a1.y, a1.z, a1.w};
+      float av[8] = {a0.x, a0.y, a0.z, a0.w, a1.x, a1.y, a1.z, a1.w};
+      if constexpr (MASKA) {
+        const int kb = *reinterpret_cast<const unsigned char*>(lds + FB_TAB_OFF + (q.f + GT) * 4 + ra * (GT / 8) +
+                                                               2 * kt + h);
+#pragma unroll
+        for (int e = 0; e < 8; ++e)
+          av[e] = __uint_as_float(__float_as_uint(av[e]) & (uint32_t)((kb << (31 - e)) >> 31)) * p.drop_scale;
+      }
       u32x4 fa[3];
       pair8(av, asc, fa);
 #pragma unroll
@@ -520,6 +552,15 @@
 }
 static std::atomic<int> g_ffn_fused_bwd{ffn_fused_bwd_initial()};
 
+#ifndef OT_BWD_MASK_FUSED
+#define OT_BWD_MASK_FUSED 1
+#endif
+static int bwd_mask_fused_initial() {
+  const char* e = getenv("ONETRANS_BWD_MASK_FUSED");
+  return e && *e ? (atoi(e) != 0) : OT_BWD_MASK_FUSED;
+}
+static std::atomic<int> g_bwd_mask_fused{bwd_mask_fused_initial()};
+
 }
 
 using namespace ot;
@@ -530,7 +571,8 @@
   return old;
 }
 
-extern "C" int ot_ffn_fused_bwd(const ot_ffn_fused_bwd_args* a, void* stream) {
+static int ffn_fused_bwd_impl(const ot_ffn_fused_bwd_args* a, bool mask, uint32_t mask_site, uint32_t* keep_out,
+                              int64_t ldkeep, void* stream) {
   OT_REQUIRE(a, "ot_ffn_fused_bwd: null arguments");
   OT_REQUIRE(a->struct_size == sizeof(ot_ffn_fused_bwd_args),
              "ot_ffn_fused_bwd: ot_ffn_fused_bwd_args.struct_size %zu != %zu (header of another ot_version)",
@@ -559,6 +601,9 @@
              "ot_ffn_fused_bwd: dropout needs dx_masked (lddxm >= %d, lddxm %% 4 == 0, 16-B aligned)", GT);
   OT_REQUIRE(a->ws_bytes >= ot_mixed_gemm_rms_workspace_size(a->ntiles, GT), "ot_ffn_fused_bwd: workspace too small");
   OT_REQUIRE(!a->rowabs_out || a->rowabs_n == 1, "ot_ffn_fused_bwd: rowabs_out needs rowabs_n == 1");
+  OT_REQUIRE(!mask || (a->drop_rate > 0.f && keep_out && ldkeep >= GT / 32 && ldkeep % 4 == 0 && a16(keep_out)),
+             "ot_ffn_fused_bwd_mask: needs drop_rate > 0 and keep_out (ldkeep >= %d, ldkeep %% 4 == 0, 16-B aligned)",
+             GT / 32);
   if (a->ntiles == 0) return OT_OK;
   FfnBwdArgs q{};
   GemmArgs& p = q.e;
@@ -584,23 +629,42 @@
   q.img2 = a->w2_image; q.g2 = a->w2_groups > 1;
   q.img1 = a->w1_image; q.g1 = a->w1_groups > 1;
   q.u = a->u; q.ldu = a->ldu; q.du = a->du; q.lddu = a->lddu; q.du_amax = a->du_amax; q.f = a->f;
-  void (*kern)(FfnBwdArgs) = a->drop_rate > 0.f ? ffn_fused_bwd_kernel<OT_EPI_RMSNORM_BWD | OT_EPI_DROPOUT>
-                                                : ffn_fused_bwd_kernel<OT_EPI_RMSNORM_BWD>;
+  q.a_site = mask_site; q.keep_out = keep_out; q.ldkeep = ldkeep;
+  void (*kern)(FfnBwdArgs) = mask                 ? ffn_fused_bwd_kernel<OT_EPI_RMSNORM_BWD | OT_EPI_DROPOUT, true>
+                             : a->drop_rate > 0.f ? ffn_fused_bwd_kernel<OT_EPI_RMSNORM_BWD | OT_EPI_DROPOUT>
+                                                  : ffn_fused_bwd_kernel<OT_EPI_RMSNORM_BWD>;
   static std::once_flag once;
   std::call_once(once, [] {
     (void)hipFuncSetAttribute((const void*)ffn_fused_bwd_kernel<OT_EPI_RMSNORM_BWD>,
                               hipFuncAttributeMaxDynamicSharedMemorySize, ffn_bwd_lds(FF_MAX_F));
     (void)hipFuncSetAttribute((const void*)ffn_fused_bwd_kernel<OT_EPI_RMSNORM_BWD | OT_EPI_DROPOUT>,
                               hipFuncAttributeMaxDynamicSharedMemorySize, ffn_bwd_lds(FF_MAX_F));
+    (void)hipFuncSetAttribute((const void*)ffn_fused_bwd_kernel<OT_EPI_RMSNORM_BWD | OT_EPI_DROPOUT, true>,
+                              hipFuncAttributeMaxDynamicSharedMemorySize, ffn_bwd_lds(FF_MAX_F, true));
     (void)hipGetLastError();
   });
   hipStream_t s = (hipStream_t)stream;
-  hipLaunchKernelGGL(kern, dim3((unsigned)a->ntiles), dim3(256), (size_t)ffn_bwd_lds(a->f), s, q);
+  hipLaunchKernelGGL(kern, dim3((unsigned)a->ntiles), dim3(256), (size_t)ffn_bwd_lds(a->f, mask), s, q);
   OT_LAUNCH_CHECK("ot_ffn_fused_bwd");
   float* dgpart = (float*)a->workspace;
   launch_colsum_reduce(dgpart, a->ntiles, GT, a->dgamma, a->accumulate_dgamma, s, dgpart + (int64_t)a->ntiles * GT);
   OT_LAUNCH_CHECK("ot_ffn_fused_bwd(dgamma)");
   return OT_OK;
+}
+
+extern "C" int ot_ffn_fused_bwd(const ot_ffn_fused_bwd_args* a, void* stream) {
+  return ffn_fused_bwd_impl(a, false, 0u, nullptr, 0, stream);
+}
+
+extern "C" int ot_ffn_fused_bwd_mask(const ot_ffn_fused_bwd_args* a, uint32_t mask_site, uint32_t* keep_out,
+                                     int64_t ldkeep, void* stream) {
+  return ffn_fused_bwd_impl(a, true, mask_site, keep_out, ldkeep, stream);
+}
+
+extern "C" int ot_bwd_mask_fused(int on) {
+  const int old = g_bwd_mask_fused.load(std::memory_order_relaxed);
+  if (on >= 0) g_bwd_mask_fused.store(on ? 1 : 0, std::memory_order_relaxed);
+  return old;
 }
 
 extern "C" int ot_ffn_fused(int on) {
diff --git a/recommend_amd/csrc/gemm_wgrad.hip b/recommend_amd/csrc/gemm_wgrad.hip
--- a/recommend_amd/csrc/gemm_wgrad.hip
+++ b/recommend_amd/csrc/gemm_wgrad.hip
@@ -41,6 +41,7 @@
   float* bslab;
   int ntk, ntn;
   const float* a_bound; const float* d_bound;
+  const uint32_t* keep; int64_t ldkeep; float d_scale;
 };
 
 template <int AXT>
@@ -190,9 +191,10 @@
 template <int TERMS>
 constexpr int wgrad_rs() { return WGRAD_BF16_RS > 0 && TERMS == 1 ? WGRAD_BF16_RS : 1; }
 
-template <int AXT, int TERMS, bool DBF = false>
+template <int AXT, int TERMS, bool DBF = false, bool KEEP = false>
 __global__ __launch_bounds__(256, 2) void wgrad_split_kernel(WgradArgs p) {
   constexpr int RS = wgrad_rs<TERMS>();
+  static_assert(!KEEP || (TERMS == 2 && AXT == OT_AX_GELU && !DBF), "keep-bits D: the pair form of the W2 gradient");
   static_assert(RS * WSPLANE <= WSOP && (TERMS == 1 || RS == 1), "wgrad stage LDS");
   static_assert(TERMS != 2 || (!DBF && (AXT == OT_AX_NONE || AXT == OT_AX_RMSNORM || AXT == OT_AX_GELU)),
                 "pair wgrad forms");
@@ -235,7 +237,7 @@
   f32x4 sa[4];
   float sdv = 1.f;
   if constexpr (PAIR) {
-    sdv = pow2_scale14(p.d_bound[0]);
+    sdv = pow2_scale14(KEEP ? p.d_bound[0] * p.d_scale : p.d_bound[0]);
     const float sqk = sqrtf((float)p.K);
     const float s1 = AXT == OT_AX_RMSNORM ? 1.f : pow2_scale14(p.a_bound[0]);
 #pragma unroll
@@ -258,6 +260,7 @@
   f32x4 va[RS][4], vd[RS][4];
   float rsd[RS];
   bool inr[RS];
+  u32x4 kw[RS];
   auto load_stage = [&](int st, const int (&ar)[RS], const int (&dr)[RS]) {
 #pragma unroll
     for (int j = 0; j < RS; ++j) {
@@ -266,6 +269,8 @@
       const uint16_t* pa16 = reinterpret_cast<const uint16_t*>(p.A) + (int64_t)(inr[j] ? ar[j] : 0) * p.lda;
       const float* pd = p.D + (int64_t)(inr[j] ? dr[j] : 0) * p.ldd;
       rsd[j] = ax == OT_AX_RMSNORM ? p.a_rstd[inr[j] ? ar[j] : 0] : 1.f;
+      if constexpr (KEEP)
+        kw[j] = *reinterpret_cast<const u32x4*>(p.keep + (int64_t)(inr[j] ? dr[j] : 0) * p.ldkeep + (n0 >> 5));
 #pragma unroll
       for (int i = 0; i < 4; ++i) {
         const int k = k0 + 4 * (sc + 8 * i), n = n0 + 4 * (sc + 8 * i);
@@ -299,6 +304,13 @@
           a = a * gv[i] * rsd[j];
         } else if (ax == OT_AX_GELU) {
           a = gelu_erf4(a);
+        }
+        if constexpr (KEEP) {
+          const int nb = (int)(kw[j][i] >> (4 * sc));
+          auto kept = [&](float v, int e) {
+            return __uint_as_float(__float_as_uint(v) & (uint32_t)((nb << (31 - e)) >> 31));
+          };
+          dv = f32x4{kept(dv.x, 0), kept(dv.y, 1), kept(dv.z, 2), kept(dv.w, 3)} * p.d_scale;
         }
         dv = dv * (inr[j] ? 1.f : 0.f);
         bsum[i] += dv;
@@ -1058,7 +1070,8 @@
                       const int32_t* chunks, int nchunks, const int32_t* gchunk, int ngroups,
                       float* dW, int64_t dw_gstride, float* db, int64_t db_gstride,
                       int accumulate, void* workspace, size_t ws_bytes, const float* a_bound, const float* d_bound,
-                      int precision, void* stream) {
+                      int precision, void* stream, const uint32_t* keep = nullptr, int64_t ldkeep = 0,
+                      float d_scale = 1.f) {
   OT_REQUIRE(precision == OT_MATMUL_F32 || precision == OT_MATMUL_SPLIT_BF16 || precision == OT_MATMUL_BF16,
              "ot_mixed_gemm_wgrad: unknown precision %d", precision);
   OT_REQUIRE(A && D && dW && chunks && gchunk && workspace, "ot_mixed_gemm_wgrad: null operand");
@@ -1066,7 +1079,13 @@
              "ot_mixed_gemm_wgrad: K, N, lda, ldd, dw_gstride must be multiples of 4");
   OT_REQUIRE(ws_bytes >= ot_wgrad_workspace_size(nchunks, K, N), "ot_mixed_gemm_wgrad: workspace too small");
   const bool dbf = (a_xform & OT_WG_D_BF16) != 0;
-  a_xform &= ~OT_WG_D_BF16;
+  const bool kbits = (a_xform & OT_WG_D_KEEPBITS) != 0;
+  a_xform &= ~(OT_WG_D_BF16 | OT_WG_D_KEEPBITS);
+  OT_REQUIRE(kbits == (keep != nullptr), "ot_mixed_gemm_wgrad: OT_WG_D_KEEPBITS goes with ot_mixed_gemm_wgrad_keep's keep");
+  OT_REQUIRE(!kbits || (precision == OT_MATMUL_SPLIT_BF16 && !dbf && a_xform == OT_AX_GELU && a_bound && d_bound &&
+                        N % GT == 0 && ldkeep >= N / 32 && ldkeep % 4 == 0 && ((uintptr_t)keep % 16) == 0),
+             "ot_mixed_gemm_wgrad: OT_WG_D_KEEPBITS needs the split mode's pair form (f32 D, OT_AX_GELU, both bounds), "
+             "N %% %d == 0, ldkeep >= N / 32, ldkeep %% 4 == 0 and 16-B aligned keep", GT);
   OT_REQUIRE(a_xform != OT_AX_RMSNORM || (a_rstd && a_gamma), "ot_mixed_gemm_wgrad: rmsnorm prologue needs rstd/gamma");
   OT_REQUIRE(!dbf || (precision == OT_MATMUL_BF16 &&
                       (a_xform == OT_AX_NONE || a_xform == OT_AX_RMSNORM || a_xform == OT_AX_BF16) &&
@@ -1078,7 +1097,7 @@
   float* bslab = db ? slab + (size_t)nchunks * K * N : nullptr;
   if (nchunks > 0) {
     WgradArgs p{A, lda, a_rows, a_xform, a_rstd, a_gamma, D, ldd, d_rows, K, N, chunks, nchunks, slab, bslab,
-                (int)ceil_div(K, GT), (int)ceil_div(N, GT), a_bound, d_bound};
+                (int)ceil_div(K, GT), (int)ceil_div(N, GT), a_bound, d_bound, keep, ldkeep, d_scale};
     const bool pair = precision == OT_MATMUL_SPLIT_BF16 && !dbf && d_bound &&
                       ((a_xform == OT_AX_RMSNORM) || ((a_xform == OT_AX_NONE || a_xform == OT_AX_GELU) && a_bound));
     const size_t shmem = (OT_WGRAD_DBUF ? 4 : 2) * WBR * WLD * sizeof(float);
@@ -1088,7 +1107,8 @@
     const bool copy = dbf && a_xform == OT_AX_BF16 && K % 8 == 0 && N % 8 == 0 && lda % 8 == 0 &&
                       ldd % 8 == 0 && ((uintptr_t)A % 16) == 0 && ((uintptr_t)D % 16) == 0 && a_rows == d_rows;
     void (*kern)(WgradArgs) =
-        pair ? (a_xform == OT_AX_NONE      ? wgrad_split_kernel<OT_AX_NONE, 2>
+        kbits  ? wgrad_split_kernel<OT_AX_GELU, 2, false, true>
+        : pair ? (a_xform == OT_AX_NONE      ? wgrad_split_kernel<OT_AX_NONE, 2>
                 : a_xform == OT_AX_RMSNORM ? wgrad_split_kernel<OT_AX_RMSNORM, 2>
                                            : wgrad_split_kernel<OT_AX_GELU, 2>)
         : copy ? (a_rows ? wgrad_bf16_kernel<true> : wgrad_bf16_kernel<false>)
@@ -1184,3 +1204,16 @@
                     dW, dw_gstride, db, db_gstride, accumulate, workspace, ws_bytes, a_bound, d_bound, precision,
                     stream);
 }
+
+extern "C" int ot_mixed_gemm_wgrad_keep(const float* A, int64_t lda, const int32_t* a_rows, int a_xform,
+                                        const float* D, int64_t ldd, const int32_t* d_rows, int K, int N,
+                                        const int32_t* chunks, int nchunks, const int32_t* gchunk, int ngroups,
+                                        float* dW, int64_t dw_gstride, float* db, int64_t db_gstride,
+                                        int accumulate, void* workspace, size_t ws_bytes, const float* a_bound,
+                                        const float* d_bound, const uint32_t* keep, int64_t ldkeep, float d_scale,
+                                        int precision, void* stream) {
+  OT_REQUIRE(keep && (a_xform & OT_WG_D_KEEPBITS), "ot_mixed_gemm_wgrad_keep: needs keep and OT_WG_D_KEEPBITS");
+  return wgrad_impl(A, lda, a_rows, a_xform, nullptr, nullptr, D, ldd, d_rows, K, N, chunks, nchunks, gchunk, ngroups,
+                    dW, dw_gstride, db, db_gstride, accumulate, workspace, ws_bytes, a_bound, d_bound, precision,
+                    stream, keep, ldkeep, d_scale);
+}
diff --git a/recommend_amd/kernels.py b/recommend_amd/kernels.py
--- a/recommend_amd/kernels.py
+++ b/recommend_amd/kernels.py
@@ -254,7 +254,8 @@
 def wgrad(A: Ptrish, lda: int, a_rows: Ptrish, D: Ptrish, ldd: int, d_rows: Ptrish, K: int, N: int, rmap_dev,
           nchunks: int, ngroups: int, dW: Ptrish, dw_gstride: int, db: Ptrish = None, db_gstride: int = 0, *,
           a_xform: int = 0, rstd: Ptrish = None, gamma: Ptrish = None, accumulate: bool = False,
-          device=None, m_rows: int = 0, rowmap=None, a_bound: Ptrish = None, d_bound: Ptrish = None) -> None:
+          device=None, m_rows: int = 0, rowmap=None, a_bound: Ptrish = None, d_bound: Ptrish = None,
+          keep: Ptrish = None, ldkeep: int = 0, d_scale: float = 1.0) -> None:
     if rowmap is not None and rowmap.group_rows:
         tiles = ((K + 127) // 128) * ((N + 127) // 128)
         ch, gc, nchunks = rowmap.chunks_for(tiles, device)
@@ -262,10 +263,18 @@
     nbytes = size('ot_wgrad_workspace_size', nchunks, K, N)
     ws = workspace(nbytes, device)
     ev = _probe.begin() if _probe is not None else None
-    call('ot_mixed_gemm_wgrad_ex', ptr(A), lda, ptr(a_rows), a_xform, ptr(rstd), ptr(gamma), ptr(D), ldd,
-         ptr(d_rows), K, N, ptr(rmap_dev['chunks']), nchunks, ptr(rmap_dev['gchunk']), ngroups, ptr(dW),
-         dw_gstride, ptr(db), db_gstride, int(accumulate), ptr(ws), ws.numel(), ptr(a_bound), ptr(d_bound), _prec(),
-         stream())
+    if keep is not None:
+        assert rstd is None and gamma is None
+        call('ot_mixed_gemm_wgrad_keep', ptr(A), lda, ptr(a_rows), a_xform, ptr(D), ldd, ptr(d_rows), K, N,
+             ptr(rmap_dev['chunks']), nchunks, ptr(rmap_dev['gchunk']), ngroups, ptr(dW), dw_gstride, ptr(db),
+             db_gstride, int(accumulate), ptr(ws), ws.numel(), ptr(a_bound), ptr(d_bound), ptr(keep), ldkeep,
+             float(d_scale), _prec(), stream())
+        a_xform &= ~_lib.OT_WG_D_KEEPBITS
+    else:
+        call('ot_mixed_gemm_wgrad_ex', ptr(A), lda, ptr(a_rows), a_xform, ptr(rstd), ptr(gamma), ptr(D), ldd,
+             ptr(d_rows), K, N, ptr(rmap_dev['chunks']), nchunks, ptr(rmap_dev['gchunk']), ngroups, ptr(dW),
+             dw_gstride, ptr(db), db_gstride, int(accumulate), ptr(ws), ws.numel(), ptr(a_bound), ptr(d_bound),
+             _prec(), stream())
     if ev is not None:
         ax = a_xform & ~_lib.OT_WG_D_BF16
         wterms = {'bf16': 1, 'f32': 0}.get(matmul_mode(), 3 if (
@@ -337,13 +346,18 @@
     return _lib.size('ot_ffn_fused_bwd_on', int(on))
 
 
+def bwd_mask_fused(on: int = -1) -> int:
+    return _lib.size('ot_bwd_mask_fused', int(on))
+
+
 def ffn_fused_bwd(dy2: Ptrish, lddy2: int, dy2_rowmax: Ptrish, dy2_rowmax_n: int, rows: Ptrish, tile_group: Ptrish,
                   ntiles: int, w2_image, w2_groups: int, w1_image, w1_groups: int, f: int, u: Ptrish, ldu: int,
                   du: Ptrish, lddu: int, x1: Ptrish, ldx1: int, gamma: Ptrish, rstd: Ptrish, dx1: Ptrish, lddx1: int,
                   dgamma: Ptrish, *, du_amax: Ptrish = None, dres: Ptrish = None, lddres: int = 0,
                   dx_masked: Ptrish = None, lddxm: int = 0, accumulate_dgamma: bool = False, amax_out: Ptrish = None,
                   rowabs_out: Ptrish = None, rowabs_n: int = 0, seed: int = 0, site: int = 0, drop: float = 0.0,
-                  tail: Tuple[int, int] = (1, 1), m_rows: int = 0, device=None) -> None:
+                  tail: Tuple[int, int] = (1, 1), m_rows: int = 0, device=None, mask_site: Optional[int] = None,
+                  keep_out: Ptrish = None, ldkeep: int = 4) -> None:
     ws = workspace(size('ot_mixed_gemm_rms_workspace_size', ntiles, 128),
                    device if device is not None else (dx1[0] if isinstance(dx1, tuple) else dx1).device)
     a = _lib.FfnFusedBwdArgs(ctypes.sizeof(_lib.FfnFusedBwdArgs), ptr(dy2), lddy2, ptr(dy2_rowmax), int(dy2_rowmax_n),
@@ -353,7 +367,10 @@
                              int(accumulate_dgamma), ptr(ws), ws.numel(), ptr(amax_out), ptr(rowabs_out),
                              int(rowabs_n), seed & 0xFFFFFFFF, site, float(drop), tail[0], tail[1], _sel(tail))
     ev = _probe.begin() if _probe is not None else None
-    call('ot_ffn_fused_bwd', ctypes.byref(a), stream())
+    if mask_site is not None:
+        call('ot_ffn_fused_bwd_mask', ctypes.byref(a), mask_site, ptr(keep_out), ldkeep, stream())
+    else:
+        call('ot_ffn_fused_bwd', ctypes.byref(a), stream())
     if ev is not None:
         M = m_rows or ntiles * 128
         _probe.end('mixed_gemm', 2.0 * M * 128 * f * 2, ev, f'ffn_fused_bwd M{M} f{f} drop{int(drop > 0)}',
@@ -604,7 +621,7 @@
         call(fn, ptr(src), lds, ptr(dst), ldd, rows, d, seed & 0xFFFFFFFF, site, float(drop), tail[0],
              tail[1], _sel(tail), stream())
     if ev is not None:
-        _probe.end('rowwise', 0.0, ev)
+        _probe.end('rowwise', 0.0, ev, 'dropout_apply')
 
 
 def dropout_rowmax_supported(d: int) -> bool:
@@ -615,7 +632,7 @@
     ev = _probe.begin() if _probe is not None else None
     call('ot_rows_absmax', ptr(x), ldx, rows, d, ptr(out), (d + 255) // 256, stream())
     if ev is not None:
-        _probe.end('rowwise', 0.0, ev)
+        _probe.end('rowwise', 0.0, ev, 'rows_absmax')
 
 
 def rows_colsum(src, ld, rows: Ptrish, nrows: int, ncols: int, out: Ptrish, accumulate=False, device=None) -> None:
diff --git a/recommend_amd/model.py b/recommend_amd/model.py
--- a/recommend_amd/model.py
+++ b/recommend_amd/model.py
@@ -165,10 +165,21 @@
 
 
 class PairBounds:
-    SLOTS = ('o', 'u', 'dy2', 'du', 'dyo', 'dqkv')
+    SLOTS = ('o', 'u', 'dy2', 'du', 'dyo', 'dqkv', 'dx')
 
     def __init__(self, layers: int, device):
         self.t, self._taken = torch.zeros(layers, 8, device=device), {}
+        self._dx = {}
+
+    def put_dx(self, l: int, dx: torch.Tensor, rowabs: torch.Tensor) -> None:
+        self._dx[l] = (dx, dx._version, rowabs)
+
+    def take_dx(self, l: int, dx2: torch.Tensor):
+        e = self._dx.pop(l, None)
+        if (e is None or e[0].data_ptr() != dx2.data_ptr() or e[0].shape != dx2.shape or e[1] != dx2._version
+                or not dx2.is_contiguous()):
+            return None
+        return e[2], self.get(l, 'dx')
 
     @classmethod
     def begin(cls, layers: int, device, mode: str, pair_wgrad: bool) -> Optional['PairBounds']:
@@ -186,6 +197,15 @@
         reported = torch.empty(rows, (n + 255) // 256, device=x.device)
         K.rows_absmax(x, ld, rows, n, reported)
     return dict(a_rowmax=reported, a_rowmax_n=reported.shape[1]) if on else {}
+
+
+def bwd_mask_gate(m, l: int, rate: float, bounds, kvalid) -> bool:
+    cfg = m.config
+    d, f = cfg.hidden_dim, cfg.ffn_dim
+    return bool(l >= 0 and rate > 0 and bounds is not None and kvalid is None and K.matmul_mode() == 'split'
+                and m.fuse_bwd and d == TILE and f % TILE == 0 and f <= K.FFN_FUSED_MAX_F
+                and m.dgrad_pair(f'blk.{l}.w2') and m.dgrad_pair(f'blk.{l}.w1')
+                and K.ffn_fused_bwd_on() and K.bwd_mask_fused())
 
 
 def _block_forward(m, l, x, I, Kq, seed, training, rstd_in=None, select=False, need_out=True, need_u=True,
@@ -418,12 +438,24 @@
         b_o, b_u = (bounds.get(l, 'o'), bounds.get(l, 'u')) if bounds is not None else (None, None)
         keep = (bounds.t,) if bounds is not None else ()
         pw2, pw1, pwo = (m.dgrad_pair(f'blk.{l}.{w}') for w in ('w2', 'w1', 'wo'))
+        ffn_bwd = (pw2 and pw1 and m.fuse_bwd and d == TILE and f % TILE == 0 and f <= K.FFN_FUSED_MAX_F
+                   and not du_bf and h is None and bool(K.ffn_fused_bwd_on()))
+        mask_fused = ffn_bwd and b_u is not None and bwd_mask_gate(m, l, rate, bounds, kvalid)
+        dx_rep = bounds.take_dx(l + 1, dx2) if bounds is not None else None
         dy2_rep = rate > 0 and not du_bf
-        b_dy2 = out('dy2') if dy2_rep else None
+        b_dy2 = out('dy2') if dy2_rep and not mask_fused else None
         rm_dy2 = (torch.empty(B * Kq, (d + 255) // 256, device=dev)
-                  if dy2_rep and pw2 and K.dropout_rowmax_supported(d) else None)
+                  if dy2_rep and pw2 and K.dropout_rowmax_supported(d) and not mask_fused else None)
         dy2 = dx2
-        if rate > 0:
+        if mask_fused:
+            if dx_rep is not None:
+                rm_dy2, b_dy2 = dx_rep
+            else:
+                rm_dy2 = torch.empty(B * Kq, 1, device=dev)
+                K.rows_absmax(dx2, d, B * Kq, d, rm_dy2)
+                b_dy2 = rm_dy2.max().reshape(1)
+            keep_bits = torch.empty(B * Kq, d // 32, dtype=torch.int32, device=dev)
+        elif rate > 0:
             dy2 = torch.empty(B * Kq, d, device=dev, dtype=torch.int16 if du_bf else torch.float32)
             K.dropout_apply(dx2, d, dy2, d, B * Kq, d, seed, 2 * l + 1, rate, tail, amax=b_dy2, rowmax=rm_dy2)
         pa2 = a_row_bounds(pw2, dy2, d, B * Kq, d, rm_dy2)
@@ -432,7 +464,7 @@
         cbf = OT_EPI_C_BF16 if du_bf else 0
         hbf = (torch.empty(B * Kq, f, dtype=torch.int16, device=dev)
                if h is None and fused2 and K.matmul_mode() == 'bf16' else None)
-        if hbf is None:
+        if hbf is None and not mask_fused:
             with m.side(u if h is None else h, dy2, *keep):
                 K.wgrad(u if h is None else h, f, mt['rows'][1], dy2, d, mt['rows'][1], f, d, mt, nct, G,
                         m.g(f'blk.{l}.w2'), f * d, m.g(f'blk.{l}.b2'), d,
@@ -441,8 +473,6 @@
                         a_bound=b_u if h is None else None, d_bound=b_dy2)
         du_rep = fused2 or (((bounds is not None and not du_bf) or pw2 or pw1) and f % TILE == 0)
         b_du = out('du') if du_rep and not du_bf else None
-        ffn_bwd = (pw2 and pw1 and m.fuse_bwd and d == TILE and f % TILE == 0 and f <= K.FFN_FUSED_MAX_F
-                   and not du_bf and h is None and bool(K.ffn_fused_bwd_on()))
         rm_du = torch.empty(B * Kq, f // TILE, device=dev) if pw1 and du_rep and not ffn_bwd else None
         rep_du = dict(amax_out=b_du, rowabs_out=rm_du, rowabs_n=f // TILE if rm_du is not None else 0)
         if ffn_bwd:
@@ -457,7 +487,14 @@
                             du_amax=b_du, dres=dx2, lddres=d, dx_masked=dyo if rate > 0 else None, lddxm=d,
                             accumulate_dgamma=acc, amax_out=b_dyo, rowabs_out=rm_dyo,
                             rowabs_n=1 if rm_dyo is not None else 0, seed=seed, site=2 * l, drop=rate, tail=tail,
-                            m_rows=maps['tail'].nrows, device=dev)
+                            m_rows=maps['tail'].nrows, device=dev, mask_site=2 * l + 1 if mask_fused else None,
+                            keep_out=keep_bits if mask_fused else None, ldkeep=d // 32)
+            if mask_fused:
+                with m.side(u, dx2, keep_bits, b_dy2, *keep):
+                    K.wgrad(u, f, mt['rows'][1], dx2, d, mt['rows'][1], f, d, mt, nct, G, m.g(f'blk.{l}.w2'), f * d,
+                            m.g(f'blk.{l}.b2'), d, a_xform=OT_AX_GELU | _lib.OT_WG_D_KEEPBITS, accumulate=acc,
+                            device=dev, m_rows=maps['tail'].nrows, rowmap=maps['tail'], a_bound=b_u, d_bound=b_dy2,
+                            keep=keep_bits, ldkeep=d // 32, d_scale=1.0 / (1.0 - rate))
         elif fused2:
             rowdot = torch.empty(B * Kq, f // TILE, device=dev)
             K.gemm_rms(OT_GEMM_NT, dy2, d, d, mt['rows'][1], m.p(f'blk.{l}.w2'), f * d, d, f, mt['tile_group'], nt,
@@ -547,13 +584,19 @@
                     rowmap=maps['all'], d_bound=b_dq)
         ax_dq = OT_AX_BF16 if dq_bf else 0
         dx = torch.empty(B * I, d, device=dev)
+        rep_dx = {}
+        if pqkv and bwd_mask_gate(m, l - 1, rate, bounds, None):
+            rm_dx = torch.empty(B * I, 1, device=dev)
+            rep_dx = dict(amax_out=out('dx'), rowabs_out=rm_dx, rowabs_n=1)
         if m.fuse_bwd:
             K.gemm_rms(OT_GEMM_NT, dqkv, 3 * d, 3 * d, ma['rows'][0], m.p(f'blk.{l}.wqkv'), 3 * d * d, 3 * d, d,
                        ma['tile_group'], na, dx, d, ma['rows'][0], epi=OT_EPI_RMSNORM_BWD, a_xform=ax_dq,
                        m_rows=maps['all'].nrows, nx=x, ldnx=d, ngamma=m.p(f'blk.{l}.norm1'), nrstd=rstd1,
                        dres=dx1, lddres=d, dres_tail=(Kq, I, inv) if Kq < I else (0, 0),
                        dgamma=m.g(f'blk.{l}.norm1'), accumulate_dgamma=acc, device=dev,
-                       bimg=m.bimg(f'blk.{l}.wqkv', 'dgrad'), **pa_q)
+                       bimg=m.bimg(f'blk.{l}.wqkv', 'dgrad'), **pa_q, **rep_dx)
+            if rep_dx:
+                bounds.put_dx(l, dx, rm_dx)
         else:
             dxn1 = torch.empty(B * I, d, device=dev)
             K.gemm_rms(OT_GEMM_NT, dqkv, 3 * d, 3 * d, ma['rows'][0], m.p(f'blk.{l}.wqkv'), 3 * d * d, 3 * d, d,
```

Result: faster. 210,100 samples/s, median of 6 (+1.2%).
